# PANXIONG-CN/TEC-MoLLM

Measured on AMD Instinct MI355X. Metric: train samples/sec, higher is better.
Workload: dtype f32; 1 GPU; BASELINE configs[1]: B=8/GPU, L_in=48, L_out=12, N=2911, F=10 (d_emb=12), 3 GPT-2 blocks, full fwd+bwd+AdamW, fp32, GATv2 per_timestep, dropout on (p=0.1); global_batch=8, parallelism=dp1, data_feed=fixed, launch=eager

## Files before the change

include/tecmollm.h:

```cpp
#ifndef TECMOLLM_H
#define TECMOLLM_H

#include <stdint.h>

#ifdef __cplusplus
extern "C" {
#endif

#define TECM_OK 0
#define TECM_E_ARG (-1)
#define TECM_E_ALIGN (-2)
#define TECM_E_LAUNCH (-3)
#define TECM_E_LDS (-4)

#define TECM_ABI_VERSION 18
int tecm_abi_version(void);
const char* tecm_last_error(void);

typedef struct TecmWin {
  int32_t enabled;
  int32_t N;
  int32_t Lin, Lout;
  int32_t stride_t;
  int32_t taps;
  int32_t Cw;
  int32_t pad;
} TecmWin;

typedef struct TecmDrop {
  float p;
  int32_t _pad;
  uint64_t seed;
  int64_t ld;
  const uint64_t* seed_dev;
} TecmDrop;

enum { TECM_A_MK = 0, TECM_A_KM = 1 };
enum { TECM_B_NK = 0, TECM_B_KN = 1 };
enum { TECM_ACT_NONE = 0, TECM_ACT_GELU_ERF = 1, TECM_ACT_GELU_TANH = 2 };

#define TECM_IO_A_BF16 1
#define TECM_IO_B_BF16 2
#define TECM_IO_C_BF16 4
#define TECM_IO_PRE_BF16 8
typedef struct TecmGemm {
  int64_t M, N, K;
  const float* A; int64_t lda; int32_t a_layout; int32_t io_bf16; TecmWin a_win; TecmDrop a_drop;
  const float* B; int64_t ldb; int32_t b_layout; int32_t _p1; TecmWin b_win; TecmDrop b_drop;
  float* C; int64_t ldc; TecmWin c_win;
  float alpha; int32_t act;
  const float* bias;
  const float* rowbias; int64_t rb_ld; int32_t rb_div; int32_t rb_mod;
  float* preact; int64_t ldp;
  const float* dact_src; int64_t ldd;
  TecmDrop out_drop;
  const float* residual; int64_t ldr;
  int32_t accumulate;
  int32_t split_k;
  float* workspace;
} TecmGemm;
int tecm_gemm_f32(const TecmGemm* desc, void* stream);
int tecm_gemm_bf16(const TecmGemm* desc, void* stream);
int tecm_gemm_bf16x3(const TecmGemm* g, void* stream);
int tecm_gemm_bf16x6(const TecmGemm* g, void* stream);

int32_t tecm_gemm_tn_splits(int64_t M, int64_t N, int64_t K);
int tecm_p8_rows(int64_t M, int64_t N);

typedef struct TecmSpatial {
  int32_t B, L, N, Cin, Demb, H;
  int32_t graphs_with_edges;
  int32_t num_tiles, tile_nodes, win_max;
  const float* x;
  const float* tf; int64_t tf_sb, tf_sl, tf_sn, tf_sf;
  const float* node_tab; const float* tod_tab; const float* doy_tab; const float* year_tab;
  const float* season_tab;
  int32_t year_rows;
  int32_t tile_edges_max;
  const float* Wl; const float* bl; const float* Wr; const float* br;
  const float* att;
  const float* bias;
  const int32_t* rowptr;
  const int32_t* colidx;
  const int32_t* tile_lo; const int32_t* tile_hi;
  TecmDrop alpha_drop;
  float* out;
  int32_t* err_flag;
  int32_t flags;
  int32_t out_ld;
} TecmSpatial;
#define TECM_SPATIAL_EMBED_ONLY 1
#define TECM_SPATIAL_NO_RESIDUAL 2
#define TECM_BAD_TOD 1
#define TECM_BAD_DOY 2
#define TECM_BAD_YEAR 4
#define TECM_BAD_SEASON 8
int tecm_spatial_fwd(const TecmSpatial* d, void* stream);
int64_t tecm_spatial_fwd2_ws_floats(const TecmSpatial* d);
int tecm_spatial_fwd2(const TecmSpatial* d, float* ws, void* stream);

typedef struct TecmSpatialGrads {
  const float* dout;
  float* d_node_tab;
  float* d_tod_tab; float* d_doy_tab; float* d_year_tab; float* d_season_tab;
  float* partials; int64_t partial_ld;
  int32_t t_chunk; int32_t num_blocks;
  const int32_t* src_ptr; const int32_t* src_col; const int32_t* src_ptr_off;
} TecmSpatialGrads;
int tecm_spatial_bwd(const TecmSpatial* d, const TecmSpatialGrads* g, void* stream);
int tecm_spatial_bwd2_blocks(const TecmSpatial* d);
int tecm_spatial_bwd2(const TecmSpatial* d, const TecmSpatialGrads* g, float* ws, void* stream);
int tecm_spatial_bwd_blocks(const TecmSpatial* d);

#define TECM_GN_OUT_BF16 2
#define TECM_GN_DACT_BF16 4
#define TECM_GN_Y_BF16 1
#define TECM_GN_STATS_GIVEN 8
int tecm_gn_y16_supported(int32_t L, int32_t N, int32_t Cout);
int tecm_groupnorm_gelu_fwd(const void* y, const float* gamma, const float* beta, void* act,
                            float* stats, int32_t B, int32_t L, int32_t N, int32_t Cout, float eps,
                            int32_t io_bf16, int32_t act_stride, void* stream);
int tecm_groupnorm_gelu_bwd(const void* dact, int32_t dstride, const void* y, const float* gamma,
                            const float* beta, const float* stats, void* dy, float* dgb_partials,
                            int32_t* num_blocks, int32_t B, int32_t L, int32_t N, int32_t Cout,
                            int32_t io_bf16,
                            float* seq_sums ,
                            void* stream);

int tecm_layernorm_fwd(const float* x, int64_t ldx, const float* gamma, const float* beta, float* y,
                       int64_t ldy, void* y16, int64_t ldy16,
                       void* y16d ,
                       int64_t ldy16d, const TecmDrop* drop ,
                       int32_t y16d_seq_T, int32_t y16d_seq_N ,
                       float* stats , int64_t M, int32_t D, float eps, void* stream);
typedef struct TecmLnAdd {
  const void* dy2;
  int64_t ld;
  int32_t bf16, _pad;
  TecmDrop drop;
} TecmLnAdd;
typedef struct TecmLnDyMap {
  int32_t T, N;
  TecmDrop drop;
} TecmLnDyMap;
int tecm_layernorm_bwd(const float* dy, int64_t lddy, const float* x, int64_t ldx, const float* gamma,
                       const float* stats, const float* dres, float* dx, void* dx_masked, int32_t masked_bf16,
                       const TecmDrop* mask_drop, float* dgb_partials, int32_t* num_blocks, int64_t M, int32_t D,
                       const TecmLnAdd* add ,
                       int32_t dy_bf16 ,
                       const TecmLnDyMap* dymap , void* stream);

#define TECM_ATT_OUT_BF16 1
#define TECM_ATT_QKV_BF16 2
#define TECM_ATT_DCTX_BF16 4
int tecm_attention_fwd(const float* qkv, void* ctx, int32_t io_bf16, int32_t B, int32_t T, int32_t N, int32_t heads,
                       int32_t D, const TecmDrop* prob_drop, void* stream);
int tecm_attention_bwd(const float* qkv, const float* dctx, void* dqkv, int32_t io_bf16, int32_t B, int32_t T, int32_t N,
                       int32_t heads, int32_t D, const TecmDrop* prob_drop, void* stream);

int tecm_colsum(const float* in, int64_t ld, int64_t outer, int64_t inner, int32_t nseg, int32_t C,
                float* out, int64_t ldo, int32_t accumulate, float scale, const TecmDrop* in_drop,
                float* workspace , void* stream);
int tecm_colsum_twin(const float* in, int64_t ld, int64_t outer, int64_t inner, int32_t nseg, int32_t C,
                     float* out, int64_t ldo, int32_t accumulate, float scale, const TecmDrop* in_drop,
                     float* workspace, void* twin_bf16, int64_t ld_twin, void* stream);

int tecm_huber_fwd_bwd(const float* pred, const float* target, float* dpred, float* loss_out,
                       int64_t n, float delta, float grad_scale, float* workspace ,
                       void* stream);

int tecm_conv_weight_pack(const float* w, float* fwd_pack, float* bwd_pack, int32_t Cout, int32_t Cin,
                          int32_t k, void* stream);
int tecm_conv_weight_unpack(const float* dpack, float* dw, int32_t Cout, int32_t Cin, int32_t k,
                            void* stream);

typedef struct TecmConvDx {
  const void* dy;
  const void* wpack;
  float* dinp;
  int32_t B, Lc, N, Cout, ld_in, _pad;
} TecmConvDx;
int tecm_conv_dx_pack(const float* w3, const float* w5, const float* w7, void* wpack, int32_t Cout, int32_t Cin,
                      int32_t ld_in, void* stream);
int tecm_conv_dx_bf16(const TecmConvDx* p, void* stream);
typedef struct TecmConvFwd {
  const void* inp;
  const void* wpack;
  const float* bias;
  float* y;
  int32_t B, Lc, N, Cout, ld_in, y_bf16;
  float* stats;
  float eps;
  int32_t _pad;
} TecmConvFwd;
int tecm_conv_fwd_pack(const float* w3, const float* w5, const float* w7, void* wpack, int32_t Cout, int32_t Cin,
                       int32_t ld_in, void* stream);
int tecm_conv_fwd_bf16(const TecmConvFwd* p, void* stream);
int tecm_conv_fwd_pack_f32(const float* w3, const float* w5, const float* w7, float* wpack, int32_t Cout, int32_t Cin,
                           int32_t ld_in, void* stream);
int tecm_conv_fwd_f32(const TecmConvFwd* p, void* stream);
int tecm_conv_dx_pack_f32(const float* w3, const float* w5, const float* w7, float* wpack, int32_t Cout, int32_t Cin,
                          int32_t ld_in, void* stream);
int tecm_conv_dx_f32(const TecmConvDx* p, void* stream);
int tecm_conv_fwd_supported(int32_t Lc, int32_t Cout, int32_t ld_in, int32_t f32);
int tecm_conv_dx_supported(int32_t Lc, int32_t Cout, int32_t ld_in, int32_t f32);

typedef struct TecmConvDw {
  const void* inp;
  const void* dy;
  float* workspace;
  float* dw3;
  float* dw5;
  float* dw7;
  int32_t B, Lc, N, Cout, Cin, ld_in, num_blocks, _pad;
} TecmConvDw;
int tecm_huber_fwd_bwd_strided(const float* pred, const int64_t* pred_strides , const float* target,
                               const int64_t* target_strides , float* dpred, float* loss_out, int32_t B, int32_t H,
                               int32_t N, float delta, float grad_scale, float* workspace , void* stream);

int64_t tecm_conv_dw_workspace(int32_t Cout, int32_t ld_in, int32_t num_blocks);
int tecm_conv_dw_bf16(const TecmConvDw* p, void* stream);
int tecm_conv_dw_f32(const TecmConvDw* p, void* stream);

int tecm_cast_bf16(const float* src, int64_t ld_src, void* dst, int64_t ld_dst, int64_t rows, int32_t cols, void* stream);

int tecm_weight_bf16(const float* src, int64_t ld_src, void* same_bf16, int64_t ld_same, void* transposed_bf16, int64_t ld_tr,
                     int32_t rows, int32_t cols, void* stream);

int tecm_dropout_apply(const float* src, int64_t ld_src, void* dst, int64_t ld_dst, int32_t dst_bf16, void* dst2_bf16,
                       int64_t ld_dst2, int64_t rows, int32_t cols, const TecmDrop* drop, void* stream);

int tecm_transpose_scale(const float* src, int64_t lds, float* dst, int64_t ldd, int32_t rows,
                         int32_t cols, float scale, void* stream);

int tecm_lora_fold(const float* lora_B, int32_t n_out, int32_t r, float scale, void* w_kn, int64_t ld_kn, int32_t kn_bf16,
                   void* w_nk, int64_t ld_nk, int32_t nk_bf16, int32_t k_off, void* stream);

int tecm_pack_vectors(const float* const* srcs, const int32_t* lens, int32_t count, float* dst, void* stream);

#define TECM_NORM_BLOCKS 512
typedef struct {
  int64_t n;
  float* param; float* grad; float* exp_avg; float* exp_avg_sq;
  double* partials;
  float* total_norm_out;
  float lr, beta1, beta2, eps, weight_decay, max_norm, grad_scale;
  int32_t step;
  int32_t zero_grad;
  int32_t _pad;
} TecmAdamW;
int tecm_adamw_clip_step(const TecmAdamW* a, void* stream);
int tecm_checksum_tail(const float* param, int64_t n, float* tail, int32_t world, int32_t rank, double* ws, void* stream);
int tecm_checksum_verify(const float* tail, int32_t world, int32_t* err_word, int32_t bit, void* stream);
int tecm_seed_advance(uint64_t* word, uint64_t inc, void* stream);

#define TECM_METRIC_STATS 8
typedef struct {
  const float* pred; int64_t p_stride_s, p_stride_h, p_stride_i;
  const float* target; int64_t t_stride_s, t_stride_h, t_stride_i;
  int64_t S; int32_t H; int32_t _pad; int64_t I;
  double mean, scale;
  float clip_lo, clip_hi; int32_t clip;
  int32_t _pad2;
  double* stats;
} TecmMetrics;
int tecm_metrics_accumulate(const TecmMetrics* m, void* stream);

typedef struct {
  const float* X; const float* TF; const float* Y; const int64_t* starts;
  const int64_t* starts_host_check;
  int64_t T; int64_t row;
  int32_t N, L_in, L_out, F_t, B, _pad;
  float* x_out; float* tf_out; float* y_out;
} TecmWindowBatch;
int tecm_window_batch(const TecmWindowBatch* w, void* stream);

enum { TECM_BASELINE_MEAN = 0, TECM_BASELINE_LAST = 1, TECM_BASELINE_PERIODIC = 2 };
typedef struct {
  const float* X; const int64_t* starts;
  const int64_t* starts_host_check;
  int64_t T;
  int32_t N, C, channel, L_in, L_out, B, mode, period;
  float* out; int64_t o_stride_b, o_stride_h, o_stride_n;
} TecmWindowBaseline;
int tecm_window_baseline(const TecmWindowBaseline* w, void* stream);

typedef struct {
  const float* x; int64_t stride_t, stride_n;
  const int32_t* slot;
  int64_t T; int32_t N, n_slots;
  double* means; double* counts;
} TecmSlotMean;
int tecm_slot_mean(const TecmSlotMean* m, void* stream);

#ifdef __cplusplus
}
#endif
#endif
```

tec-mollm_amd/csrc/common.h:

```cpp
#pragma once
#include <hip/hip_runtime.h>
#include <stdint.h>
#include <stdio.h>
#include <stdarg.h>
#include <math.h>

#include "../../include/tecmollm.h"

#define TECM_WAVE 64

void tecm_set_error(const char* fmt, ...);

#define TECM_REQUIRE(cond, code, ...)            \
  do {                                           \
    if (!(cond)) {                               \
      tecm_set_error(__VA_ARGS__);               \
      return (code);                             \
    }                                            \
  } while (0)

#define TECM_CHECK_LAUNCH(name)                                                     \
  do {                                                                              \
    hipError_t e_ = hipGetLastError();                                              \
    if (e_ != hipSuccess) {                                                         \
      tecm_set_error("%s: launch failed: %s", (name), hipGetErrorString(e_));       \
      return TECM_E_LAUNCH;                                                         \
    }                                                                               \
  } while (0)

static inline bool tecm_aligned(const void* p, size_t a) { return (reinterpret_cast<uintptr_t>(p) % a) == 0; }

__host__ __device__ __forceinline__ uint32_t tecm_hash24(uint64_t seed, uint64_t idx) {
  uint32_t x = (uint32_t)idx + ((uint32_t)(idx >> 32) & 0xffffffu) * 0x9E3779u;
  x += (uint32_t)seed + (uint32_t)(seed >> 32) * 0x9E3779B1u;
  x ^= x >> 16;
  x *= 0x7feb352du;
  x ^= x >> 15;
  x *= 0x846ca68bu;
  x ^= x >> 16;
  return x >> 8;
}
__device__ __forceinline__ uint64_t tecm_seed_now(uint64_t seed, const uint64_t* seed_dev) {
  return seed_dev ? seed + *seed_dev : seed;
}
__host__ __device__ __forceinline__ uint32_t tecm_drop_thresh(float p) { return (uint32_t)(p * 16777216.0f); }
__device__ __forceinline__ float tecm_drop_mult(uint64_t seed, uint64_t idx, uint32_t thresh, float inv_keep) {
  return tecm_hash24(seed, idx) >= thresh ? inv_keep : 0.0f;
}

typedef __bf16 tecm_bf16x4 __attribute__((ext_vector_type(4)));
__device__ __forceinline__ void tecm_store_bf16x4(void* dst, float a, float b, float c, float d) {
  tecm_bf16x4 v;
  v[0] = (__bf16)a; v[1] = (__bf16)b; v[2] = (__bf16)c; v[3] = (__bf16)d;
  *reinterpret_cast<tecm_bf16x4*>(dst) = v;
}

__device__ __forceinline__ float gelu_erf(float x) { return 0.5f * x * (1.0f + erff(x * 0.70710678118654752440f)); }
__device__ __forceinline__ float dgelu_erf(float x) {
  const float cdf = 0.5f * (1.0f + erff(x * 0.70710678118654752440f));
  const float pdf = 0.39894228040143267794f * expf(-0.5f * x * x);
  return cdf + x * pdf;
}
__device__ __forceinline__ void gelu_erf_parts(float x, float& cdf, float& e) {
  const float z = fabsf(x) * 0.70710678118654752440f;
  const float t = __builtin_amdgcn_rcpf(1.0f + 0.3275911f * z);
  e = __builtin_amdgcn_exp2f(-0.72134752044448170368f * x * x);
  const float poly =
      t * (0.254829592f + t * (-0.284496736f + t * (1.421413741f + t * (-1.453152027f + t * 1.061405429f))));
  cdf = 0.5f * (1.0f + copysignf(1.0f - poly * e, x));
}
__device__ __forceinline__ float gelu_erf_fast(float x) {
  float cdf, e;
  gelu_erf_parts(x, cdf, e);
  return x * cdf;
}
__device__ __forceinline__ float dgelu_erf_fast(float x) {
  float cdf, e;
  gelu_erf_parts(x, cdf, e);
  return cdf + x * 0.39894228040143267794f * e;
}
__device__ __forceinline__ float fast_tanh(float u) {
  const float e = __builtin_amdgcn_exp2f(2.88539008177792681472f * u);
  return 1.0f - 2.0f * __builtin_amdgcn_rcpf(1.0f + e);
}
__device__ __forceinline__ void gelu_tanh_parts(float x, float x2, float& s, float& r) {
  float a = x * fmaf(x2, 0.10294324f, 2.3022082f);
  a = fminf(a, 100.0f);
  const float E = __builtin_amdgcn_exp2f(a);
  r = __builtin_amdgcn_rcpf(1.0f + E);
  s = E * r;
}
__device__ __forceinline__ float gelu_tanh(float x) {
  float s, r;
  gelu_tanh_parts(x, x * x, s, r);
  return x * s;
}
__device__ __forceinline__ float dgelu_tanh(float x) {
  const float x2 = x * x;
  float s, r;
  gelu_tanh_parts(x, x2, s, r);
  const float du2 = fmaf(x2, 0.21406445f, 1.5957691f);
  return fmaf(x * du2 * r, s, s);
}
__device__ __forceinline__ float apply_act(int act, float v) {
  return act == TECM_ACT_GELU_ERF ? gelu_erf(v) : (act == TECM_ACT_GELU_TANH ? gelu_tanh(v) : v);
}
__device__ __forceinline__ float apply_dact(int act, float v) {
  return act == TECM_ACT_GELU_ERF ? dgelu_erf(v) : (act == TECM_ACT_GELU_TANH ? dgelu_tanh(v) : 1.0f);
}

__device__ __forceinline__ float wave_sum(float v) {
#pragma unroll
  for (int o = 32; o > 0; o >>= 1) v += __shfl_xor(v, o, 64);
  return v;
}
__device__ __forceinline__ float wave_max(float v) {
#pragma unroll
  for (int o = 32; o > 0; o >>= 1) v = fmaxf(v, __shfl_xor(v, o, 64));
  return v;
}
__device__ __forceinline__ float group16_sum(float v) {
#pragma unroll
  for (int o = 8; o > 0; o >>= 1) v += __shfl_xor(v, o, 64);
  return v;
}

#define TECM_ROW_INVALID INT32_MIN
struct RowRef {
  int64_t srow;
  int32_t t0;
};

__device__ __forceinline__ RowRef make_rowref(const TecmWin& w, bool win, int64_t m, int64_t rows) {
  RowRef r;
  if (m >= rows) {
    r.srow = 0;
    r.t0 = TECM_ROW_INVALID;
    return r;
  }
  if (!win) {
    r.srow = m;
    r.t0 = 0;
    return r;
  }
  const int64_t q = m / w.N;
  const int32_t n = (int32_t)(m - q * w.N);
  const int64_t bq = q / w.Lout;
  const int32_t t_out = (int32_t)(q - bq * w.Lout);
  r.t0 = t_out * w.stride_t - w.pad;
  r.srow = (bq * w.Lin + r.t0) * (int64_t)w.N + n;
  return r;
}
```

tec-mollm_amd/csrc/gemm.hip:

```cpp
#include "gemm_bf16_impl.h"
int tecm_gemm_x3_dispatch(const TecmGemm& g, int products, hipStream_t st);

namespace {

template <int U>
__global__ __launch_bounds__(256) void splitk_reduce_kernel(const TecmGemm g, int splits) {
  __shared__ float red[4][64];
  const int64_t total = g.M * g.N;
  const int lane = threadIdx.x & 63, wave = threadIdx.x >> 6;
  const tecm_gemm::DropCtx odc = tecm_gemm::make_drop(g.out_drop);
  for (int64_t i0 = (int64_t)blockIdx.x * 64; i0 < total; i0 += (int64_t)gridDim.x * 64) {
    const int64_t i = i0 + lane;
    float v16[U];
#pragma unroll
    for (int u = 0; u < U; ++u) v16[u] = 0.f;
    if (i < total) {
      for (int s = wave; s < splits; s += 4 * U) {
#pragma unroll
        for (int u = 0; u < U; ++u) {
          const int sl = s + 4 * u;
          const float v = g.workspace[(int64_t)(sl < splits ? sl : splits - 1) * total + i];
          v16[u] += sl < splits ? v : 0.f;
        }
      }
    }
#pragma unroll
    for (int u = U / 2; u > 0; u >>= 1)
#pragma unroll
      for (int v = 0; v < u; ++v) v16[v] += v16[v + u];
    red[wave][lane] = v16[0];
    __syncthreads();
    if (wave == 0 && i < total) {
      const float v = (red[0][lane] + red[1][lane]) + (red[2][lane] + red[3][lane]);
      const int64_t m = i / g.N;
      tecm_gemm::epilogue_store(g, odc, m, (int32_t)(i - m * g.N), v);
    }
    __syncthreads();
  }
}

__global__ __launch_bounds__(256) void erf_post_kernel(float* __restrict__ C, int64_t ldc, const float* __restrict__ src,
                                                       int64_t lds, int64_t M, int32_t N, tecm_gemm::DropCtx odc) {
  const int64_t total = M * N;
  odc.seed = tecm_seed_now(odc.seed, odc.sdev);
  for (int64_t i = (int64_t)blockIdx.x * blockDim.x + threadIdx.x; i < total; i += (int64_t)gridDim.x * blockDim.x) {
    const int64_t m = i / N;
    const int32_t n = (int32_t)(i - m * N);
    float v = C[m * ldc + n];
    v = src ? v * dgelu_erf(src[m * lds + n]) : gelu_erf(v);
    if (odc.thresh) v *= tecm_drop_mult(odc.seed, (uint64_t)(m * odc.ld + n), odc.thresh, odc.inv);
    C[m * ldc + n] = v;
  }
}

int pick_vec(const float* p, int64_t ld, const TecmWin& w, bool inner_is_k, int64_t K) {
  int v = 4;
  while (v > 1) {
    bool ok = tecm_aligned(p, 4 * v) && (ld % v == 0);
    if (w.enabled) ok = ok && (w.Cw % v == 0);
    if (inner_is_k) ok = ok && (K % v == 0);
    if (ok) break;
    v >>= 1;
  }
  return v;
}

bool win_ok(const TecmWin& w) {
  return !w.enabled || (w.N > 0 && w.Lin > 0 && w.Lout > 0 && w.stride_t > 0 && w.taps > 0 && w.Cw > 0 && w.pad >= 0);
}

}

enum { MODE_F32 = 0, MODE_BF16 = 1, MODE_X3 = 2, MODE_X6 = 3 };
static int gemm_entry(const TecmGemm* d, void* stream, int mode);

extern "C" int tecm_gemm_f32(const TecmGemm* d, void* stream) { return gemm_entry(d, stream, MODE_F32); }

extern "C" int tecm_gemm_bf16(const TecmGemm* d, void* stream) { return gemm_entry(d, stream, MODE_BF16); }

extern "C" int tecm_gemm_bf16x3(const TecmGemm* d, void* stream) { return gemm_entry(d, stream, MODE_X3); }
extern "C" int tecm_gemm_bf16x6(const TecmGemm* d, void* stream) { return gemm_entry(d, stream, MODE_X6); }

static int gemm_entry(const TecmGemm* d, void* stream, int mode) {
  const bool bf16 = mode == MODE_BF16;
  TECM_REQUIRE(d != nullptr, TECM_E_ARG, "tecm_gemm_f32: null descriptor");
  const TecmGemm& g = *d;
  TECM_REQUIRE(g.M > 0 && g.N > 0 && g.K > 0, TECM_E_ARG, "tecm_gemm_f32: M,N,K must be positive (%lld,%lld,%lld)",
               (long long)g.M, (long long)g.N, (long long)g.K);
  TECM_REQUIRE(g.M < (1ll << 31) && g.K < (1ll << 30) && g.N < (1ll << 30), TECM_E_ARG,
               "tecm_gemm_f32: M/N/K too large for 32-bit row arithmetic");
  TECM_REQUIRE(g.A && g.B && g.C, TECM_E_ARG, "tecm_gemm_f32: null operand");
  TECM_REQUIRE(win_ok(g.a_win) && win_ok(g.b_win) && win_ok(g.c_win), TECM_E_ARG, "tecm_gemm_f32: bad window view");
  TECM_REQUIRE(!(g.a_win.enabled && g.a_layout != TECM_A_MK), TECM_E_ARG,
               "tecm_gemm_f32: a_win needs the MK layout (view rows are m)");
  TECM_REQUIRE(!(g.b_win.enabled && g.b_layout != TECM_B_KN), TECM_E_ARG,
               "tecm_gemm_f32: b_win needs the KN layout (view rows are the reduction index)");
  TECM_REQUIRE(!(g.a_win.enabled && (int64_t)g.a_win.taps * g.a_win.Cw != g.K), TECM_E_ARG,
               "tecm_gemm_f32: a_win taps*Cw != K");
  TECM_REQUIRE(!(g.b_win.enabled && (int64_t)g.b_win.taps * g.b_win.Cw != g.N), TECM_E_ARG,
               "tecm_gemm_f32: b_win taps*Cw != N");
  TECM_REQUIRE(!(g.c_win.enabled && (int64_t)g.c_win.taps * g.c_win.Cw != g.N), TECM_E_ARG,
               "tecm_gemm_f32: c_win taps*Cw != N");
  TECM_REQUIRE(!(g.rowbias && (g.rb_div <= 0 || g.rb_mod <= 0)), TECM_E_ARG, "tecm_gemm_f32: bad rowbias spec");
  TECM_REQUIRE(!(g.split_k > 1 && g.workspace == nullptr), TECM_E_ARG, "tecm_gemm_f32: split_k needs a workspace");
  TECM_REQUIRE(g.a_layout == TECM_A_MK || g.b_layout == TECM_B_KN, TECM_E_ARG,
               "tecm_gemm_f32: layout combination KM x NK is not built");
  hipStream_t st = (hipStream_t)stream;
  int avec = pick_vec(g.A, g.lda, g.a_win, g.a_layout == TECM_A_MK, g.K);
  int bvec = pick_vec(g.B, g.ldb, g.b_win, g.b_layout == TECM_B_NK, g.K);
  if (g.io_bf16 & TECM_IO_A_BF16) avec = 4;
  if (g.io_bf16 & TECM_IO_B_BF16) bvec = 4;
  const bool win = g.a_win.enabled || g.b_win.enabled;
  const bool drop = g.a_drop.p > 0.f || g.b_drop.p > 0.f;
  auto ok4 = [](const void* p, int64_t ld) { return p == nullptr || (tecm_aligned(p, 16) && ld % 4 == 0); };
  const bool c16 = (g.io_bf16 & TECM_IO_C_BF16) != 0;
  const bool p16 = (g.io_bf16 & TECM_IO_PRE_BF16) != 0;
  auto ok4h = [](const void* p, int64_t ld) { return p == nullptr || (tecm_aligned(p, 8) && ld % 4 == 0); };
  const bool vec4 = g.N % 4 == 0 && (c16 ? ok4h(g.C, g.ldc) : ok4(g.C, g.ldc)) && ok4(g.bias, 4) && ok4(g.rowbias, g.rb_ld) &&
                    (p16 ? ok4h(g.preact, g.ldp) && ok4h(g.dact_src, g.ldd) : ok4(g.preact, g.ldp) && ok4(g.dact_src, g.ldd)) &&
                    ok4(g.residual, g.ldr) &&
                    (!g.c_win.enabled || g.c_win.Cw % 4 == 0) &&
                    (g.split_k <= 1 || tecm_aligned(g.workspace, 16));
  if (c16) TECM_REQUIRE(vec4, TECM_E_ALIGN, "tecm_gemm_bf16: bf16 C needs 16-byte friendly epilogue operands");
  if (bf16)
    TECM_REQUIRE(avec == 4 && bvec == 4, TECM_E_ALIGN,
                 "tecm_gemm_bf16: operands must be 16-byte aligned with leading dims / K / Cw multiples of 4");
  if (mode == MODE_X3 || mode == MODE_X6) {
    TECM_REQUIRE(g.a_layout == TECM_A_MK && g.b_layout == TECM_B_NK && !win && !drop, TECM_E_ARG,
                 "tecm_gemm_bf16x3: serves the plain MK x NK contraction only (no operand windows / prologue dropout)");
    TECM_REQUIRE(avec == 4 && bvec == 4, TECM_E_ALIGN,
                 "tecm_gemm_bf16x3: operands must be 16-byte aligned with leading dims / K multiples of 4");
  }
  const int io = g.io_bf16 & (TECM_IO_A_BF16 | TECM_IO_B_BF16 | TECM_IO_C_BF16 | TECM_IO_PRE_BF16);
  TECM_REQUIRE(io == g.io_bf16, TECM_E_ARG, "tecm_gemm: unknown io_bf16 bits");
  if (io) {
    TECM_REQUIRE(bf16, TECM_E_ARG, "tecm_gemm: bf16 tensors in HBM are served by tecm_gemm_bf16 only");
    if (io & (TECM_IO_A_BF16 | TECM_IO_B_BF16))
      TECM_REQUIRE(!drop, TECM_E_ARG, "tecm_gemm_bf16: bf16 operands take no prologue dropout");
    if (io & TECM_IO_A_BF16) {
      TECM_REQUIRE(tecm_aligned(g.A, 16) && g.lda % 8 == 0, TECM_E_ALIGN, "tecm_gemm_bf16: bf16 A must be 16-byte friendly");
      TECM_REQUIRE((g.a_layout == TECM_A_MK ? g.K : g.M) % 8 == 0 && (!g.a_win.enabled || g.a_win.Cw % 8 == 0), TECM_E_ARG,
                   "tecm_gemm_bf16: bf16 A needs its contiguous extent (K for MK, M for KM) and a_win.Cw to be multiples of 8");
    }
    if (io & TECM_IO_B_BF16) {
      TECM_REQUIRE(tecm_aligned(g.B, 16) && g.ldb % 8 == 0, TECM_E_ALIGN, "tecm_gemm_bf16: bf16 B must be 16-byte friendly");
      TECM_REQUIRE((g.b_layout == TECM_B_NK ? g.K : g.N) % 8 == 0 && (!g.b_win.enabled || g.b_win.Cw % 8 == 0), TECM_E_ARG,
                   "tecm_gemm_bf16: bf16 B needs its contiguous extent (K for NK, N for KN) and b_win.Cw to be multiples of 8");
    }
    if (io & TECM_IO_PRE_BF16)
      TECM_REQUIRE(vec4 && (g.preact || g.dact_src) && g.split_k <= 1 && g.act != TECM_ACT_GELU_ERF && !g.c_win.enabled &&
                       !g.rowbias,
                   TECM_E_ARG, "tecm_gemm_bf16: a bf16 preact / dact_src needs the 16-byte friendly plain tanh-GELU epilogue");
    if (io & TECM_IO_C_BF16)
      TECM_REQUIRE(vec4 && !g.residual && !g.accumulate && !g.c_win.enabled && g.split_k <= 1 &&
                       g.act != TECM_ACT_GELU_ERF,
                   TECM_E_ARG, "tecm_gemm_bf16: bf16 C needs a 16-byte friendly plain epilogue");
  }
  TecmGemm gk = g;
  gk.io_bf16 = io | (vec4 ? TECM_P0_VEC4 : 0);
  const bool erf = g.act == TECM_ACT_GELU_ERF;
  if (erf) {
    TECM_REQUIRE(!g.residual && !g.accumulate && !g.c_win.enabled, TECM_E_ARG,
                 "tecm_gemm_f32: GELU_ERF cannot be combined with residual / accumulate / c_win");
    gk.act = TECM_ACT_NONE;
    gk.dact_src = nullptr;
    gk.out_drop.p = 0.f;
  }
  int splits;
  if (mode == MODE_X3 || mode == MODE_X6) {
    splits = tecm_gemm_x3_dispatch(gk, mode == MODE_X6 ? 6 : 3, st);
  } else if (bf16) {
    if (g.a_layout == TECM_A_MK && g.b_layout == TECM_B_NK)
      splits = tecm_gemm16_dispatch_mk_nk(gk, win, drop, st);
    else if (g.a_layout == TECM_A_MK)
      splits = tecm_gemm16_dispatch_mk_kn(gk, win, drop, st);
    else
      splits = tecm_gemm16_dispatch_km_kn(gk, win, drop, st);
  } else if (g.a_layout == TECM_A_MK && g.b_layout == TECM_B_NK)
    splits = tecm_gemm_dispatch_mk_nk(gk, avec, bvec, win, drop, st);
  else if (g.a_layout == TECM_A_MK)
    splits = tecm_gemm_dispatch_mk_kn(gk, avec, bvec, win, drop, st);
  else
    splits = tecm_gemm_dispatch_km_kn(gk, avec, bvec, win, drop, st);
  if (splits < 0) return splits;
  if (splits > 1) {
    const int64_t total = g.M * g.N;
    const int64_t want = (total + 63) / 64;
    const int blocks = (int)(want < 4096 ? want : 4096);
    if (splits > 32)
      hipLaunchKernelGGL(splitk_reduce_kernel<16>, dim3(blocks), dim3(256), 0, st, gk, splits);
    else if (splits > 16)
      hipLaunchKernelGGL(splitk_reduce_kernel<8>, dim3(blocks), dim3(256), 0, st, gk, splits);
    else
      hipLaunchKernelGGL(splitk_reduce_kernel<4>, dim3(blocks), dim3(256), 0, st, gk, splits);
    TECM_CHECK_LAUNCH("tecm_gemm_f32/splitk_reduce");
  }
  if (erf) {
    const int64_t want = (g.M * g.N + 255) / 256;
    hipLaunchKernelGGL(erf_post_kernel, dim3((unsigned)(want < 4096 ? want : 4096)), dim3(256), 0, st, g.C, g.ldc,
                       g.dact_src, g.ldd, g.M, (int32_t)g.N, tecm_gemm::make_drop_host(g.out_drop));
    TECM_CHECK_LAUNCH("tecm_gemm_f32/erf_post");
  }
  return TECM_OK;
}
```

tec-mollm_amd/csrc/gemm_impl.h:

```cpp
#pragma once
#include "common.h"
#ifndef TECM_BIG_THREADS
#define TECM_BIG_THREADS 512
#endif
#include <utility>
#ifndef TECM_ABLATE
#define TECM_ABLATE 0
#endif
#ifndef TECM_STAGE_Q
#define TECM_STAGE_Q 0
#endif

typedef float f32x16 __attribute__((ext_vector_type(16)));
typedef float f32x4 __attribute__((ext_vector_type(4)));

#define TECM_P0_VEC4 0x100

namespace tecm_gemm {

template <class F, int... Is>
__device__ __forceinline__ void static_for_impl(F&& f, std::integer_sequence<int, Is...>) {
  (f(std::integral_constant<int, Is>{}), ...);
}
template <int N, class F>
__device__ __forceinline__ void static_for(F&& f) {
  static_for_impl(f, std::make_integer_sequence<int, N>{});
}

constexpr int BM = 128;
constexpr int BK = 32;
constexpr int LDK = BK + 4;
constexpr int NTHREADS_MAX = 512;
__host__ __device__ constexpr int threads_for(int bn) { return bn >= 128 ? TECM_BIG_THREADS : 256; }

struct DropCtx {
  uint64_t seed;
  int64_t ld;
  uint32_t thresh;
  float inv;
  const uint64_t* sdev;
};
inline DropCtx make_drop_host(const TecmDrop& d) {
  DropCtx c;
  c.seed = d.seed;
  c.sdev = d.seed_dev;
  c.ld = d.ld;
  c.thresh = d.p > 0.f ? tecm_drop_thresh(d.p) : 0u;
  c.inv = d.p > 0.f ? 1.0f / (1.0f - d.p) : 1.0f;
  return c;
}
__device__ __forceinline__ DropCtx make_drop(const TecmDrop& d) {
  DropCtx c;
  c.seed = tecm_seed_now(d.seed, d.seed_dev);
  c.sdev = nullptr;
  c.ld = d.ld;
  c.thresh = d.p > 0.f ? tecm_drop_thresh(d.p) : 0u;
  c.inv = d.p > 0.f ? 1.0f / (1.0f - d.p) : 1.0f;
  return c;
}

template <int VEC>
__device__ __forceinline__ void gload(const float* __restrict__ p, const float* __restrict__ safe, bool ok,
                                      float (&out)[VEC]) {
  const float* q = ok ? p : safe;
  if constexpr (VEC == 4) {
    const float4 v = *reinterpret_cast<const float4*>(q);
    out[0] = v.x; out[1] = v.y; out[2] = v.z; out[3] = v.w;
  } else if constexpr (VEC == 2) {
    const float2 v = *reinterpret_cast<const float2*>(q);
    out[0] = v.x; out[1] = v.y;
  } else {
    out[0] = q[0];
  }
}

template <int VEC>
__device__ __forceinline__ void apply_drop(const DropCtx& dc, int64_t didx, float (&v)[VEC]) {
  if (dc.thresh) {
#pragma unroll
    for (int e = 0; e < VEC; ++e) v[e] *= tecm_drop_mult(dc.seed, (uint64_t)(didx + e), dc.thresh, dc.inv);
  }
}

template <int VEC>
__device__ __forceinline__ void lds_store(float* dst, const float (&v)[VEC]) {
  if constexpr (VEC == 4) {
    *reinterpret_cast<float4*>(dst) = make_float4(v[0], v[1], v[2], v[3]);
  } else if constexpr (VEC == 2) {
    *reinterpret_cast<float2*>(dst) = make_float2(v[0], v[1]);
  } else {
    dst[0] = v[0];
  }
}

struct WinRow {
  int64_t srow;
  int32_t t0;
};
__device__ __forceinline__ WinRow win_row(const TecmWin& w, int64_t m, int64_t rows) {
  WinRow r;
  if (m >= rows) {
    r.srow = 0;
    r.t0 = TECM_ROW_INVALID;
    return r;
  }
  const uint32_t mm = (uint32_t)m;
  const uint32_t q = mm / (uint32_t)w.N;
  const int32_t n = (int32_t)(mm - q * (uint32_t)w.N);
  const uint32_t bq = q / (uint32_t)w.Lout;
  const int32_t t_out = (int32_t)(q - bq * (uint32_t)w.Lout);
  r.t0 = t_out * w.stride_t - w.pad;
  r.srow = ((int64_t)bq * w.Lin + r.t0) * (int64_t)w.N + n;
  return r;
}

template <bool ROWK, int ROWS, int VEC, bool WIN, bool DROP, int NTHREADS>
struct Stager {
  static constexpr int R = ROWK ? BK : ROWS;
  static constexpr int CI = ROWK ? ROWS : BK;
  static constexpr int LD = ROWK ? ROWS + 4 : LDK;
  static constexpr int VPR = CI / VEC;
  static constexpr int NV = (R * VPR) / NTHREADS;
  static constexpr int RSTEP = NTHREADS / VPR;
  static_assert((R * VPR) % NTHREADS == 0 && NTHREADS % VPR == 0, "tile/thread mapping");

  struct Tile {
    float regs[NV][VEC];
    uint32_t okbits = 0;
    int64_t dsave[DROP ? NV : 1];
  };
  const float* ptr[NV];
  uint32_t rowok;
  bool inner_ok;
  int64_t didx[DROP ? NV : 1];
  WinRow wr[(WIN && !ROWK) ? NV : 1];
  int32_t rn[(WIN && ROWK) ? NV : 1], rt[(WIN && ROWK) ? NV : 1], rb[(WIN && ROWK) ? NV : 1];
  int32_t tap, c;
  int32_t kk;

  __device__ __forceinline__ void init(const float* __restrict__ P, const TecmWin& w, int64_t ld, int64_t row0,
                                       int64_t rows_total, int32_t kbeg, int64_t fixed0, int64_t fixed_lim,
                                       const DropCtx& dc) {
    const int cv = (threadIdx.x % VPR) * VEC;
    const int r0 = threadIdx.x / VPR;
    rowok = 0;
    inner_ok = true;
    tap = 0;
    c = 0;
    kk = kbeg + cv;
    const bool wen = WIN && w.enabled;
    if (!wen) {
      if constexpr (!ROWK) {
#pragma unroll
        for (int i = 0; i < NV; ++i) {
          int64_t row = row0 + r0 + i * RSTEP;
          if (row < rows_total) rowok |= 1u << i;
          else row = rows_total - 1;
          ptr[i] = P + row * ld + kbeg + cv;
          if constexpr (DROP) didx[i] = row * dc.ld + kbeg + cv;
        }
      } else {
        inner_ok = (fixed0 + cv) < fixed_lim;
        const int64_t inner = inner_ok ? fixed0 + cv : 0;
#pragma unroll
        for (int i = 0; i < NV; ++i) {
          const int64_t row = (int64_t)kbeg + r0 + i * RSTEP;
          ptr[i] = P + row * ld + inner;
          if constexpr (DROP) didx[i] = row * dc.ld + inner;
        }
      }
    } else if constexpr (WIN) {
      if constexpr (!ROWK) {
#pragma unroll
        for (int i = 0; i < NV; ++i) wr[i] = win_row(w, row0 + r0 + i * RSTEP, rows_total);
        tap = kk / w.Cw;
        c = kk - tap * w.Cw;
      } else {
        const int32_t inner = (int32_t)(fixed0 + cv);
        inner_ok = inner < fixed_lim;
        tap = inner / w.Cw;
        c = inner - tap * w.Cw;
#pragma unroll
        for (int i = 0; i < NV; ++i) {
          const uint32_t row = (uint32_t)(kbeg + r0 + i * RSTEP);
          const uint32_t q = row / (uint32_t)w.N;
          rn[i] = (int32_t)(row - q * (uint32_t)w.N);
          rb[i] = (int32_t)(q / (uint32_t)w.Lout);
          rt[i] = (int32_t)(q - (uint32_t)rb[i] * (uint32_t)w.Lout);
        }
      }
    }
  }

  __device__ __forceinline__ void load(Tile& tl, const float* __restrict__ P, const TecmWin& w, int64_t ld, int32_t k0,
                                       int32_t klim, const DropCtx& dc) {
    load_part<0, NV>(tl, P, w, ld, k0, klim, dc);
  }
  template <int IB, int IE>
  __device__ __forceinline__ void load_part(Tile& tl, const float* __restrict__ P, const TecmWin& w, int64_t ld, int32_t k0,
                                            int32_t klim, const DropCtx& dc) {
    if constexpr (IB >= IE) return;
    const int r0 = threadIdx.x / VPR;
    const bool wen = WIN && w.enabled;
    constexpr bool LAST = IE == NV;
    if (!wen) {
      if constexpr (!ROWK) {
        const bool kok = kk < klim;
#pragma unroll
        for (int i = IB; i < IE; ++i) {
          const bool ok = kok && ((rowok >> i) & 1u);
          gload<VEC>(ptr[i], P, ok, tl.regs[i]);
          tl.okbits = (tl.okbits & ~(1u << i)) | ((ok ? 1u : 0u) << i);
          if constexpr (DROP) { tl.dsave[i] = didx[i]; didx[i] += BK; }
          ptr[i] += BK;
        }
        if constexpr (LAST) kk += BK;
      } else {
#pragma unroll
        for (int i = IB; i < IE; ++i) {
          const bool ok = inner_ok && (k0 + r0 + i * RSTEP) < klim;
          gload<VEC>(ptr[i], P, ok, tl.regs[i]);
          tl.okbits = (tl.okbits & ~(1u << i)) | ((ok ? 1u : 0u) << i);
          if constexpr (DROP) { tl.dsave[i] = didx[i]; didx[i] += (int64_t)BK * dc.ld; }
          ptr[i] += (int64_t)BK * ld;
        }
      }
    } else if constexpr (WIN) {
      if constexpr (!ROWK) {
        const bool kok = kk < klim;
        const int64_t tapoff = (int64_t)tap * w.N;
#pragma unroll
        for (int i = IB; i < IE; ++i) {
          const int32_t t_in = wr[i].t0 + tap;
          const bool ok = kok && t_in >= 0 && t_in < w.Lin;
          const int64_t row = wr[i].srow + tapoff;
          gload<VEC>(P + row * ld + c, P, ok, tl.regs[i]);
          tl.okbits = (tl.okbits & ~(1u << i)) | ((ok ? 1u : 0u) << i);
          if constexpr (DROP) tl.dsave[i] = row * dc.ld + c;
        }
        if constexpr (LAST) {
          kk += BK;
          c += BK;
          while (c >= w.Cw) { c -= w.Cw; ++tap; }
        }
      } else {
#pragma unroll
        for (int i = IB; i < IE; ++i) {
          const int32_t t_in = rt[i] * w.stride_t - w.pad + tap;
          const bool ok = inner_ok && (k0 + r0 + i * RSTEP) < klim && t_in >= 0 && t_in < w.Lin;
          const int64_t row = ((int64_t)rb[i] * w.Lin + t_in) * (int64_t)w.N + rn[i];
          gload<VEC>(P + row * ld + c, P, ok, tl.regs[i]);
          tl.okbits = (tl.okbits & ~(1u << i)) | ((ok ? 1u : 0u) << i);
          if constexpr (DROP) tl.dsave[i] = row * dc.ld + c;
          rn[i] += BK;
          while (rn[i] >= w.N) {
            rn[i] -= w.N;
            if (++rt[i] >= w.Lout) { rt[i] = 0; ++rb[i]; }
          }
        }
      }
    }
  }

  __device__ __forceinline__ void load_steady(Tile& tl, int64_t ld, const DropCtx& dc) {
    tl.okbits = ~0u;
#pragma unroll
    for (int i = 0; i < NV; ++i) {
      gload<VEC>(ptr[i], ptr[i], true, tl.regs[i]);
      if constexpr (!ROWK) {
        if constexpr (DROP) { tl.dsave[i] = didx[i]; didx[i] += BK; }
        ptr[i] += BK;
      } else {
        if constexpr (DROP) { tl.dsave[i] = didx[i]; didx[i] += (int64_t)BK * dc.ld; }
        ptr[i] += (int64_t)BK * ld;
      }
    }
    if constexpr (!ROWK) kk += BK;
  }
  __device__ __forceinline__ void store_steady(const Tile& tl, float* lds, const DropCtx& dc) {
    const int cv = (threadIdx.x % VPR) * VEC;
    const int r0 = threadIdx.x / VPR;
#pragma unroll
    for (int i = 0; i < NV; ++i) {
      if constexpr (DROP) {
        float v[VEC];
#pragma unroll
        for (int e = 0; e < VEC; ++e) v[e] = tl.regs[i][e];
        apply_drop<VEC>(dc, tl.dsave[i], v);
        lds_store<VEC>(lds + (r0 + i * RSTEP) * LD + cv, v);
      } else {
        lds_store<VEC>(lds + (r0 + i * RSTEP) * LD + cv, tl.regs[i]);
      }
    }
  }

  __device__ __forceinline__ void store(const Tile& tl, float* lds, const DropCtx& dc) { store_part<0, NV>(tl, lds, dc); }
  template <int IB, int IE>
  __device__ __forceinline__ void store_part(const Tile& tl, float* lds, const DropCtx& dc) {
    if constexpr (IB >= IE) return;
    const int cv = (threadIdx.x % VPR) * VEC;
    const int r0 = threadIdx.x / VPR;
#pragma unroll
    for (int i = IB; i < IE; ++i) {
      float v[VEC];
      const bool ok = (tl.okbits >> i) & 1u;
#pragma unroll
      for (int e = 0; e < VEC; ++e) v[e] = ok ? tl.regs[i][e] : 0.f;
      if constexpr (DROP) apply_drop<VEC>(dc, tl.dsave[i], v);
      lds_store<VEC>(lds + (r0 + i * RSTEP) * LD + cv, v);
    }
  }
};

struct EpiRow {
  int64_t m;
  int64_t crow;
  int64_t drow;
  int32_t t0;
  const float* rb;
};
struct EpiCol {
  int32_t n;
  int32_t tap, c;
  float bias;
  bool ok;
};

__device__ __forceinline__ EpiRow epi_row(const TecmGemm& g, const DropCtx& odc, int64_t m) {
  EpiRow r;
  r.m = m;
  r.t0 = 0;
  if (g.c_win.enabled) {
    const WinRow w = win_row(g.c_win, m, g.M);
    r.crow = w.srow;
    r.t0 = w.t0;
    r.drow = 0;
  } else {
    r.crow = m * g.ldc;
    r.drow = m * odc.ld;
  }
  r.rb = g.rowbias ? g.rowbias + (int64_t)(((uint32_t)m / (uint32_t)g.rb_div) % (uint32_t)g.rb_mod) * g.rb_ld
                   : nullptr;
  return r;
}
__device__ __forceinline__ EpiCol epi_col(const TecmGemm& g, int64_t n) {
  EpiCol c;
  c.n = (int32_t)n;
  c.ok = n < g.N;
  c.bias = (g.bias && c.ok) ? g.bias[n] : 0.f;
  c.tap = 0;
  c.c = 0;
  if (g.c_win.enabled) {
    c.tap = c.n / g.c_win.Cw;
    c.c = c.n - c.tap * g.c_win.Cw;
  }
  return c;
}
__device__ __forceinline__ void epi_elem(const TecmGemm& g, const DropCtx& odc, const EpiRow& r, const EpiCol& c,
                                         float v) {
  const int32_t n = c.n;
  v = v * g.alpha + c.bias;
  if (r.rb) v += r.rb[n];
  if (g.preact) g.preact[r.m * g.ldp + n] = v;
  if (g.dact_src)
    v *= dgelu_tanh(g.dact_src[r.m * g.ldd + n]);
  else if (g.act)
    v = gelu_tanh(v);
  int64_t off, didx;
  if (g.c_win.enabled) {
    const int32_t t_in = r.t0 + c.tap;
    if (t_in < 0 || t_in >= g.c_win.Lin) return;
    const int64_t row = r.crow + (int64_t)c.tap * g.c_win.N;
    off = row * g.ldc + c.c;
    didx = row * odc.ld + c.c;
  } else {
    off = r.crow + n;
    didx = r.drow + n;
  }
  if (odc.thresh) v *= tecm_drop_mult(odc.seed, (uint64_t)didx, odc.thresh, odc.inv);
  if (g.residual) v += g.residual[r.m * g.ldr + n];
  if (g.accumulate) v += g.C[off];
  g.C[off] = v;
}
__device__ __forceinline__ void epilogue_store(const TecmGemm& g, const DropCtx& odc, int64_t m, int32_t n, float v) {
  const EpiRow r = epi_row(g, odc, m);
  const EpiCol c = epi_col(g, n);
  epi_elem(g, odc, r, c, v);
}

__device__ __forceinline__ void epi_vec4(const TecmGemm& g, const DropCtx& odc, const EpiRow& r, const EpiCol& c,
                                         const float4& bias4, float4 v) {
  const int32_t n = c.n;
  float o[4] = {v.x * g.alpha + bias4.x, v.y * g.alpha + bias4.y, v.z * g.alpha + bias4.z, v.w * g.alpha + bias4.w};
  if (r.rb) {
    const float4 t = *reinterpret_cast<const float4*>(r.rb + n);
    o[0] += t.x; o[1] += t.y; o[2] += t.z; o[3] += t.w;
  }
  const bool p16 = (g.io_bf16 & TECM_IO_PRE_BF16) != 0;
  if (g.preact) {
    if (p16) {
      tecm_bf16x4 h;
      h[0] = (__bf16)o[0]; h[1] = (__bf16)o[1]; h[2] = (__bf16)o[2]; h[3] = (__bf16)o[3];
      *reinterpret_cast<tecm_bf16x4*>(reinterpret_cast<__bf16*>(g.preact) + r.m * g.ldp + n) = h;
      o[0] = (float)h[0]; o[1] = (float)h[1]; o[2] = (float)h[2]; o[3] = (float)h[3];
    } else {
      *reinterpret_cast<float4*>(g.preact + r.m * g.ldp + n) = make_float4(o[0], o[1], o[2], o[3]);
    }
  }
  if (g.dact_src) {
    float4 t;
    if (p16) {
      const tecm_bf16x4 h = *reinterpret_cast<const tecm_bf16x4*>(reinterpret_cast<const __bf16*>(g.dact_src) + r.m * g.ldd + n);
      t = make_float4((float)h[0], (float)h[1], (float)h[2], (float)h[3]);
    } else {
      t = *reinterpret_cast<const float4*>(g.dact_src + r.m * g.ldd + n);
    }
    o[0] *= dgelu_tanh(t.x); o[1] *= dgelu_tanh(t.y);
    o[2] *= dgelu_tanh(t.z); o[3] *= dgelu_tanh(t.w);
  } else if (g.act) {
#pragma unroll
    for (int e = 0; e < 4; ++e) o[e] = gelu_tanh(o[e]);
  }
  int64_t off, didx;
  if (g.c_win.enabled) {
    const int32_t t_in = r.t0 + c.tap;
    if (t_in < 0 || t_in >= g.c_win.Lin) return;
    const int64_t row = r.crow + (int64_t)c.tap * g.c_win.N;
    off = row * g.ldc + c.c;
    didx = row * odc.ld + c.c;
  } else {
    off = r.crow + n;
    didx = r.drow + n;
  }
  if (odc.thresh) {
#pragma unroll
    for (int e = 0; e < 4; ++e) o[e] *= tecm_drop_mult(odc.seed, (uint64_t)(didx + e), odc.thresh, odc.inv);
  }
  if (g.residual) {
    const float4 t = *reinterpret_cast<const float4*>(g.residual + r.m * g.ldr + n);
    o[0] += t.x; o[1] += t.y; o[2] += t.z; o[3] += t.w;
  }
  if (g.accumulate) {
    const float4 t = *reinterpret_cast<const float4*>(g.C + off);
    o[0] += t.x; o[1] += t.y; o[2] += t.z; o[3] += t.w;
  }
  if (g.io_bf16 & TECM_IO_C_BF16) {
    typedef __bf16 bf16x4_t __attribute__((ext_vector_type(4)));
    bf16x4_t h;
    h[0] = (__bf16)o[0]; h[1] = (__bf16)o[1]; h[2] = (__bf16)o[2]; h[3] = (__bf16)o[3];
    *reinterpret_cast<bf16x4_t*>(reinterpret_cast<__bf16*>(g.C) + off) = h;
    return;
  }
  *reinterpret_cast<float4*>(g.C + off) = make_float4(o[0], o[1], o[2], o[3]);
}

#ifndef TECM_EPI_STAMP
#define TECM_EPI_STAMP(i) do { } while (0)
#endif
template <int NIT, int RPI, int MODE>
__device__ __forceinline__ void epi_fast_load(const TecmGemm& g, int lrow, int64_t mrow0, const EpiCol& ecol,
                                              float4 (&in)[NIT]) {
  const int32_t ncol = ecol.ok ? ecol.n : 0;
  if constexpr (MODE == 5) {
#pragma unroll
    for (int it = 0; it < NIT; ++it) {
      int64_t m = mrow0 + it * RPI + lrow;
      m = m < g.M ? m : g.M - 1;
      const uint32_t rr = ((uint32_t)m / (uint32_t)g.rb_div) % (uint32_t)g.rb_mod;
      in[it] = *reinterpret_cast<const float4*>(g.rowbias + (int64_t)rr * g.rb_ld + ncol);
    }
  }
  if constexpr (MODE >= 1 && MODE <= 3) {
    const float* src = MODE == 1 ? g.residual : (MODE == 2 ? g.dact_src : g.C);
    const int64_t ld = MODE == 1 ? g.ldr : (MODE == 2 ? g.ldd : g.ldc);
    const int32_t mb = (int32_t)mrow0 + lrow;
    const int64_t off0 = (int64_t)mb * ld + ncol, step = (int64_t)RPI * ld, off_last = (g.M - 1) * ld + ncol;
    if (MODE == 2 && (g.io_bf16 & TECM_IO_PRE_BF16)) {
#pragma unroll
      for (int it = 0; it < NIT; ++it) {
        const int64_t off = mb + it * RPI < (int32_t)g.M ? off0 + it * step : off_last;
        const float2 raw = *reinterpret_cast<const float2*>(reinterpret_cast<const __bf16*>(src) + off);
        in[it].x = raw.x;
        in[it].y = raw.y;
      }
      return;
    }
#pragma unroll
    for (int it = 0; it < NIT; ++it) {
      const int64_t off = mb + it * RPI < (int32_t)g.M ? off0 + it * step : off_last;
      in[it] = *reinterpret_cast<const float4*>(src + off);
    }
  }
}
enum { EPI_F_PRE = 1, EPI_F_P16 = 2, EPI_F_ACT = 4, EPI_F_DROP = 8, EPI_F_C16 = 16 };
template <int FEAT, int BIT>
__device__ __forceinline__ bool epi_feat(bool dynamic) {
  if constexpr (FEAT < 0) return dynamic;
  else return (FEAT & BIT) != 0;
}
template <int NIT, int RPI, int STG_LD, int MODE, bool NT, int FEAT = -1>
__device__ __forceinline__ void epi_fast_rows(const TecmGemm& g, const DropCtx& odc, const float* stg, int lrow, int lcol,
                                              int64_t mrow0, const EpiCol& ecol, const float4& bias4,
                                              const float4 (&in)[NIT]) {
  const int32_t n = ecol.n;
  const bool c16 = epi_feat<FEAT, EPI_F_C16>((g.io_bf16 & TECM_IO_C_BF16) != 0);
  const bool p16 = epi_feat<FEAT, EPI_F_P16>((g.io_bf16 & TECM_IO_PRE_BF16) != 0);
  const bool has_pre = epi_feat<FEAT, EPI_F_PRE>(g.preact != nullptr);
  const bool has_act = epi_feat<FEAT, EPI_F_ACT>(g.act != 0);
  const bool has_drop = epi_feat<FEAT, EPI_F_DROP>(odc.thresh != 0);
  constexpr int GRP = NIT < 4 ? NIT : 4;
  static_assert(NIT % GRP == 0, "row groups are read from the staging rows in whole batches");
  const int32_t mb = (int32_t)mrow0 + lrow;
  const int64_t offC0 = (int64_t)mb * g.ldc + n, stepC = (int64_t)RPI * g.ldc;
  const int64_t offP0 = (int64_t)mb * g.ldp + n, stepP = (int64_t)RPI * g.ldp;
  const int64_t idxD0 = (int64_t)mb * odc.ld + n, stepD = (int64_t)RPI * odc.ld;
  float4 vv[GRP];
#pragma unroll
  for (int it = 0; it < NIT; ++it) {
    if (it % GRP == 0) {
#pragma unroll
      for (int j = 0; j < GRP; ++j)
        vv[j] = *reinterpret_cast<const float4*>(&stg[((it + j) * RPI + lrow) * STG_LD + lcol]);
    }
    const int64_t m = mb + it * RPI;
    const float4 v = vv[it % GRP];
    const bool row_ok = mb + it * RPI < (int32_t)g.M && ecol.ok;
    if constexpr (MODE == 4) {
      if (row_ok) *reinterpret_cast<float4*>(g.workspace + ((int64_t)blockIdx.z * g.M + m) * g.N + n) = v;
      continue;
    }
    float o[4] = {v.x * g.alpha + bias4.x, v.y * g.alpha + bias4.y, v.z * g.alpha + bias4.z, v.w * g.alpha + bias4.w};
    if constexpr (MODE == 5) {
      o[0] += in[it].x; o[1] += in[it].y; o[2] += in[it].z; o[3] += in[it].w;
    }
    if (has_pre && p16) {
      tecm_bf16x4 hv;
      hv[0] = (__bf16)o[0]; hv[1] = (__bf16)o[1]; hv[2] = (__bf16)o[2]; hv[3] = (__bf16)o[3];
      if (row_ok) {
        tecm_bf16x4* dst = reinterpret_cast<tecm_bf16x4*>(reinterpret_cast<__bf16*>(g.preact) + (offP0 + it * stepP));
        if constexpr (NT) __builtin_nontemporal_store(hv, dst);
        else *dst = hv;
      }
      o[0] = (float)hv[0]; o[1] = (float)hv[1]; o[2] = (float)hv[2]; o[3] = (float)hv[3];
    } else if (has_pre && row_ok) {
      if constexpr (NT) {
        f32x4 nv = {o[0], o[1], o[2], o[3]};
        __builtin_nontemporal_store(nv, reinterpret_cast<f32x4*>(g.preact + (offP0 + it * stepP)));
      } else {
        *reinterpret_cast<float4*>(g.preact + (offP0 + it * stepP)) = make_float4(o[0], o[1], o[2], o[3]);
      }
    }
    if constexpr (MODE == 2) {
      float t0 = in[it].x, t1 = in[it].y, t2 = in[it].z, t3 = in[it].w;
      if (p16) {
        const uint32_t lo = __builtin_bit_cast(uint32_t, in[it].x), hi = __builtin_bit_cast(uint32_t, in[it].y);
        t0 = __builtin_bit_cast(float, lo << 16); t1 = __builtin_bit_cast(float, lo & 0xffff0000u);
        t2 = __builtin_bit_cast(float, hi << 16); t3 = __builtin_bit_cast(float, hi & 0xffff0000u);
      }
      o[0] *= dgelu_tanh(t0); o[1] *= dgelu_tanh(t1);
      o[2] *= dgelu_tanh(t2); o[3] *= dgelu_tanh(t3);
    } else {
      if (has_act) {
#pragma unroll
        for (int e = 0; e < 4; ++e) o[e] = gelu_tanh(o[e]);
      }
    }
    int64_t off = offC0 + it * stepC, didx = idxD0 + it * stepD;
    bool st_ok = row_ok;
    if constexpr (MODE == 6) {
      const WinRow w = win_row(g.c_win, m < g.M ? m : g.M - 1, g.M);
      const int32_t t_in = w.t0 + ecol.tap;
      const int64_t row = w.srow + (int64_t)ecol.tap * g.c_win.N;
      st_ok = row_ok && t_in >= 0 && t_in < g.c_win.Lin;
      off = row * g.ldc + ecol.c;
      didx = row * odc.ld + ecol.c;
    }
    if (has_drop) {
#pragma unroll
      for (int e = 0; e < 4; ++e) o[e] *= tecm_drop_mult(odc.seed, (uint64_t)(didx + e), odc.thresh, odc.inv);
    }
    if constexpr (MODE == 1 || MODE == 3) {
      o[0] += in[it].x; o[1] += in[it].y; o[2] += in[it].z; o[3] += in[it].w;
    }
    if (st_ok) {
      if constexpr (NT) {
        if (c16) {
          tecm_bf16x4 hv;
          hv[0] = (__bf16)o[0]; hv[1] = (__bf16)o[1]; hv[2] = (__bf16)o[2]; hv[3] = (__bf16)o[3];
          __builtin_nontemporal_store(hv, reinterpret_cast<tecm_bf16x4*>(reinterpret_cast<__bf16*>(g.C) + off));
        } else {
          f32x4 nv = {o[0], o[1], o[2], o[3]};
          __builtin_nontemporal_store(nv, reinterpret_cast<f32x4*>(g.C + off));
        }
      } else {
        if (c16) tecm_store_bf16x4(reinterpret_cast<__bf16*>(g.C) + off, o[0], o[1], o[2], o[3]);
        else *reinterpret_cast<float4*>(g.C + off) = make_float4(o[0], o[1], o[2], o[3]);
      }
    }
#ifdef TECM_EPI_SLEEP
    __builtin_amdgcn_s_sleep(TECM_EPI_SLEEP);
#endif
  }
}
template <int SLABS, int NIT, int RPI, int STG_LD, int MODE, bool NT, int FEAT = -1, typename StageFn>
__device__ __forceinline__ void epi_fast_block(const TecmGemm& g, const DropCtx& odc, const float* stg, int lrow, int lcol,
                                               int64_t mrow0, const EpiCol& ecol, const float4& bias4, StageFn&& stage) {
  float4 in[2][NIT];
  epi_fast_load<NIT, RPI, MODE>(g, lrow, mrow0, ecol, in[0]);
  static_for<SLABS>([&](auto sc) {
    constexpr int sl = decltype(sc)::value;
    TECM_EPI_STAMP(3 * sl);
    stage(sc);
    TECM_EPI_STAMP(3 * sl + 1);
    if constexpr (sl + 1 < SLABS)
      epi_fast_load<NIT, RPI, MODE>(g, lrow, mrow0 + (int64_t)(sl + 1) * NIT * RPI, ecol, in[(sl + 1) & 1]);
    epi_fast_rows<NIT, RPI, STG_LD, MODE, NT, FEAT>(g, odc, stg, lrow, lcol, mrow0 + (int64_t)sl * NIT * RPI, ecol, bias4, in[sl & 1]);
    TECM_EPI_STAMP(3 * sl + 2);
  });
}
__device__ __forceinline__ int epi_fast_mode(const TecmGemm& g) {
  if (!(g.io_bf16 & TECM_P0_VEC4)) return -1;
  if (gridDim.z > 1) return 4;
  const int streams = (g.residual ? 1 : 0) + (g.dact_src ? 1 : 0) + (g.accumulate ? 1 : 0);
  if (g.c_win.enabled)
    return (streams == 0 && !g.rowbias && !g.preact && !(g.io_bf16 & (TECM_IO_C_BF16 | TECM_IO_PRE_BF16))) ? 6 : -1;
  if (g.rowbias) return streams == 0 ? 5 : -1;
  if (streams > 1) return -1;
  return g.residual ? 1 : (g.dact_src ? 2 : (g.accumulate ? 3 : 0));
}
template <int SLABS, int NIT, int RPI, int STG_LD, bool NT = false, bool SPECIAL = false, typename StageFn>
__device__ __forceinline__ void epi_fast_dispatch(int mode, const TecmGemm& g, const DropCtx& odc, const float* stg, int lrow,
                                                  int lcol, int64_t mrow0, const EpiCol& ecol, const float4& bias4,
                                                  StageFn&& stage) {
  if constexpr (SPECIAL) {
    const int feat = (g.preact ? EPI_F_PRE : 0) | ((g.io_bf16 & TECM_IO_PRE_BF16) ? EPI_F_P16 : 0) | (g.act ? EPI_F_ACT : 0) |
                     (odc.thresh ? EPI_F_DROP : 0) | ((g.io_bf16 & TECM_IO_C_BF16) ? EPI_F_C16 : 0);
    if (mode == 0 && feat == EPI_F_C16)
      return epi_fast_block<SLABS, NIT, RPI, STG_LD, 0, NT, EPI_F_C16>(g, odc, stg, lrow, lcol, mrow0, ecol, bias4, stage);
    if (mode == 0 && feat == (EPI_F_PRE | EPI_F_P16 | EPI_F_ACT | EPI_F_C16))
      return epi_fast_block<SLABS, NIT, RPI, STG_LD, 0, NT, EPI_F_PRE | EPI_F_P16 | EPI_F_ACT | EPI_F_C16>(g, odc, stg, lrow, lcol, mrow0,
                                                                                                    ecol, bias4, stage);
    if (mode == 1 && feat == EPI_F_DROP)
      return epi_fast_block<SLABS, NIT, RPI, STG_LD, 1, NT, EPI_F_DROP>(g, odc, stg, lrow, lcol, mrow0, ecol, bias4, stage);
    if (mode == 2 && (feat & ~EPI_F_ACT) == (EPI_F_P16 | EPI_F_C16))
      return epi_fast_block<SLABS, NIT, RPI, STG_LD, 2, NT, EPI_F_P16 | EPI_F_C16>(g, odc, stg, lrow, lcol, mrow0, ecol, bias4, stage);
  }
  if (mode == 0) epi_fast_block<SLABS, NIT, RPI, STG_LD, 0, NT>(g, odc, stg, lrow, lcol, mrow0, ecol, bias4, stage);
  else if (mode == 1) epi_fast_block<SLABS, NIT, RPI, STG_LD, 1, NT>(g, odc, stg, lrow, lcol, mrow0, ecol, bias4, stage);
  else if (mode == 2) epi_fast_block<SLABS, NIT, RPI, STG_LD, 2, NT>(g, odc, stg, lrow, lcol, mrow0, ecol, bias4, stage);
  else if (mode == 3) epi_fast_block<SLABS, NIT, RPI, STG_LD, 3, NT>(g, odc, stg, lrow, lcol, mrow0, ecol, bias4, stage);
  else if (mode == 5) epi_fast_block<SLABS, NIT, RPI, STG_LD, 5, NT>(g, odc, stg, lrow, lcol, mrow0, ecol, bias4, stage);
  else if (mode == 6) epi_fast_block<SLABS, NIT, RPI, STG_LD, 6, NT>(g, odc, stg, lrow, lcol, mrow0, ecol, bias4, stage);
  else epi_fast_block<SLABS, NIT, RPI, STG_LD, 4, NT>(g, odc, stg, lrow, lcol, mrow0, ecol, bias4, stage);
}

template <int MT, int NT, int WTM, int WTN, int STG_LD>
__device__ __forceinline__ void block_epilogue(const TecmGemm& g, f32x16 (&acc)[MT][NT], float* smem, int wave, int lane,
                                               int wm, int wn, int64_t m0, int64_t n0) {
  const int r = lane & 31, h = lane >> 5;
  const DropCtx odc = make_drop(g.out_drop);
  const bool split = gridDim.z > 1;
  float* stg = smem + wave * (WTM * STG_LD);
  auto stage_all = [&](auto) {
    static_for<MT>([&](auto ic) {
      constexpr int i = decltype(ic)::value;
      static_for<16>([&](auto ec) {
        constexpr int e = decltype(ec)::value;
        static_for<NT>([&](auto jc) {
          constexpr int jn = decltype(jc)::value;
          stg[(i * 32 + (e & 3) + 8 * (e >> 2) + 4 * h) * STG_LD + jn * 32 + r] = acc[i][jn][e];
        });
      });
    });
  };
  if (g.io_bf16 & TECM_P0_VEC4) {
    constexpr int LPR = WTN / 4;
    constexpr int RPI = 64 / LPR;
    const int lcol = (lane % LPR) * 4, lrow = lane / LPR;
    const EpiCol ecol = epi_col(g, n0 + wn * WTN + lcol);
    float4 bias4 = make_float4(0.f, 0.f, 0.f, 0.f);
    if (g.bias) bias4 = *reinterpret_cast<const float4*>(g.bias + (ecol.ok ? ecol.n : 0));
    const int fmode = epi_fast_mode(g);
    if (fmode >= 0) {
      epi_fast_dispatch<1, WTM / RPI, RPI, STG_LD>(fmode, g, odc, stg, lrow, lcol, m0 + wm * WTM, ecol, bias4, stage_all);
      return;
    }
    stage_all(0);
    __syncthreads();
#pragma unroll 1
    for (int it = 0; it < WTM / RPI; ++it) {
      const int rl = it * RPI + lrow;
      const int64_t m = m0 + wm * WTM + rl;
      if (m < g.M && ecol.ok) {
        const float4 v = *reinterpret_cast<const float4*>(&stg[rl * STG_LD + lcol]);
        if (split) {
          *reinterpret_cast<float4*>(g.workspace + ((int64_t)blockIdx.z * g.M + m) * g.N + ecol.n) = v;
        } else {
          const EpiRow er = epi_row(g, odc, m);
          epi_vec4(g, odc, er, ecol, bias4, v);
        }
      }
    }
  } else {
    stage_all(0);
    __syncthreads();
    constexpr int RPI = 64 / WTN;
    const int lcol = lane % WTN, lrow = lane / WTN;
    const EpiCol ecol = epi_col(g, n0 + wn * WTN + lcol);
#pragma unroll 1
    for (int it = 0; it < WTM / RPI; ++it) {
      const int rl = it * RPI + lrow;
      const int64_t m = m0 + wm * WTM + rl;
      if (m < g.M && ecol.ok) {
        const float v = stg[rl * STG_LD + lcol];
        if (split) {
          g.workspace[((int64_t)blockIdx.z * g.M + m) * g.N + ecol.n] = v;
        } else {
          const EpiRow er = epi_row(g, odc, m);
          epi_elem(g, odc, er, ecol, v);
        }
      }
    }
  }
}

template <int ALAY, int BLAY, int AVEC, int BVEC, int BN, bool WIN, bool DROP, int BMT = BM>
__global__ __launch_bounds__(threads_for(BN), (AVEC == 4 && BVEC == 4) ? (threads_for(BN) == 512 ? (BMT > 128 ? 2 : 4) : 2) : 1) void gemm_kernel(const TecmGemm g,
                                                                                           int tiles_m, int tiles_n,
                                                                                           int k_chunk) {
  constexpr int NTHREADS = threads_for(BN);
  constexpr int NWAVES = NTHREADS / 64;
  constexpr int WN = BN >= 128 ? (NWAVES == 8 ? (BMT > 128 ? 2 : 4) : 2) : (BN == 64 ? 2 : 1);
  constexpr int WM = NWAVES / WN;
  constexpr int WTM = BMT / WM;
  static_assert(WTM >= 32 && WTM % 32 == 0, "wave tile");
  constexpr int WTN = BN / WN;
  constexpr int MT = WTM / 32;
  constexpr int NT = WTN / 32;
  using AStager = Stager<ALAY == TECM_A_KM, BMT, AVEC, WIN, DROP, NTHREADS>;
  using BStager = Stager<BLAY == TECM_B_KN, BN, BVEC, WIN, DROP, NTHREADS>;
  constexpr int A_FLOATS = AStager::R * AStager::LD;
  constexpr int B_FLOATS = BStager::R * BStager::LD;
  constexpr int TILE_FLOATS = A_FLOATS + B_FLOATS;
  constexpr int STG_LD = WTN + 4;
  constexpr int STG_FLOATS = NWAVES * WTM * STG_LD;
  constexpr int SMEM_FLOATS = 2 * TILE_FLOATS > STG_FLOATS ? 2 * TILE_FLOATS : STG_FLOATS;
  __shared__ __attribute__((aligned(16))) float smem[SMEM_FLOATS];

  const int nwg = tiles_m * tiles_n;
  const int id = blockIdx.x;
  const int xcd = id & 7, local = id >> 3;
  const int q8 = nwg >> 3, r8 = nwg & 7;
  const int wg = (xcd < r8 ? xcd * (q8 + 1) : r8 * (q8 + 1) + (xcd - r8) * q8) + local;
  const int GROUP_M = g._p1 > 0 ? g._p1 : (tiles_n <= 8 ? 2 : 8);
  const int per_group = GROUP_M * tiles_n;
  const int group = wg / per_group;
  const int first_m = group * GROUP_M;
  const int gsz = min(tiles_m - first_m, GROUP_M);
  const int in_group = wg - group * per_group;
  const int tm = first_m + in_group % gsz, tn = in_group / gsz;
  const int64_t m0 = (int64_t)tm * BMT;
  const int64_t n0 = (int64_t)tn * BN;
  const int32_t kbeg = blockIdx.z * k_chunk;
  const int32_t kend = min((int32_t)g.K, kbeg + k_chunk);

  const int lane = threadIdx.x & 63, wave = threadIdx.x >> 6;
  const int wm = wave / WN, wn = wave % WN;
  const int r = lane & 31, h = lane >> 5;

  const DropCtx adc = make_drop(g.a_drop), bdc = make_drop(g.b_drop);

  AStager sa;
  BStager sb;
  typename AStager::Tile ta;
  typename BStager::Tile tb;
  sa.init(g.A, g.a_win, g.lda, m0, g.M, kbeg, m0, g.M, adc);
  sb.init(g.B, g.b_win, g.ldb, n0, g.N, kbeg, n0, g.N, bdc);

  f32x16 acc[MT][NT];
#pragma unroll
  for (int i = 0; i < MT; ++i)
#pragma unroll
    for (int j = 0; j < NT; ++j)
#pragma unroll
      for (int e = 0; e < 16; ++e) acc[i][j][e] = 0.f;

  auto read_frags = [&](const float* As, const float* Bs, auto qc, float (&af)[MT][4], float (&bf)[NT][4]) {
    constexpr int q = decltype(qc)::value;
#pragma unroll
    for (int i = 0; i < MT; ++i) {
      const int row = wm * WTM + i * 32 + r;
      if constexpr (ALAY == TECM_A_MK) {
        const float4 v = *reinterpret_cast<const float4*>(&As[row * LDK + 8 * q + 4 * h]);
        af[i][0] = v.x; af[i][1] = v.y; af[i][2] = v.z; af[i][3] = v.w;
      } else {
#pragma unroll
        for (int j = 0; j < 4; ++j) af[i][j] = As[(8 * q + 4 * h + j) * AStager::LD + row];
      }
    }
#pragma unroll
    for (int i = 0; i < NT; ++i) {
      const int col = wn * WTN + i * 32 + r;
      if constexpr (BLAY == TECM_B_NK) {
        const float4 v = *reinterpret_cast<const float4*>(&Bs[col * LDK + 8 * q + 4 * h]);
        bf[i][0] = v.x; bf[i][1] = v.y; bf[i][2] = v.z; bf[i][3] = v.w;
      } else {
#pragma unroll
        for (int j = 0; j < 4; ++j) bf[i][j] = Bs[(8 * q + 4 * h + j) * BStager::LD + col];
      }
    }
  };
  auto do_mfma = [&](const float (&af)[MT][4], const float (&bf)[NT][4]) {
#pragma unroll
    for (int j = 0; j < 4; ++j)
#pragma unroll
      for (int i = 0; i < MT; ++i)
#pragma unroll
        for (int jn = 0; jn < NT; ++jn)
          acc[i][jn] = __builtin_amdgcn_mfma_f32_32x32x2f32(af[i][j], bf[jn][j], acc[i][jn], 0, 0, 0);
  };

  {
    typename AStager::Tile ta0;
    typename BStager::Tile tb0;
    sa.load(ta0, g.A, g.a_win, g.lda, kbeg, kend, adc);
    sb.load(tb0, g.B, g.b_win, g.ldb, kbeg, kend, bdc);
    if (kbeg + BK < kend) {
      sa.load(ta, g.A, g.a_win, g.lda, kbeg + BK, kend, adc);
      sb.load(tb, g.B, g.b_win, g.ldb, kbeg + BK, kend, bdc);
    }
    sa.store(ta0, smem, adc);
    sb.store(tb0, smem + A_FLOATS, bdc);
  }
  __syncthreads();

  float fa[2][MT][4], fb[2][NT][4];
  constexpr int ANV = AStager::NV, BNV = BStager::NV;
  auto tile_body = [&](const float* Ac, const float* Bc, float* An, int32_t k0, auto fullc) {
    constexpr bool FULL = decltype(fullc)::value;
    read_frags(Ac, Bc, std::integral_constant<int, 0>{}, fa[0], fb[0]);
    static_for<4>([&](auto qc) {
      constexpr int q = decltype(qc)::value;
      if constexpr (q < 3 && !(TECM_ABLATE >= 2 && FULL)) read_frags(Ac, Bc, std::integral_constant<int, q + 1>{}, fa[(q + 1) & 1], fb[(q + 1) & 1]);
      do_mfma(fa[q & 1], fb[q & 1]);
      if constexpr (q == TECM_STAGE_Q && !((TECM_ABLATE == 1 || TECM_ABLATE == 2) && FULL)) {
        if (FULL || k0 + BK < kend) {
          if constexpr (TECM_ABLATE == 3 && FULL) {
#pragma unroll
            for (int i = 0; i < ANV; ++i) asm volatile("" ::"v"(ta.regs[i][0]), "v"(ta.regs[i][1]), "v"(ta.regs[i][2]), "v"(ta.regs[i][3]));
#pragma unroll
            for (int i = 0; i < BNV; ++i) asm volatile("" ::"v"(tb.regs[i][0]), "v"(tb.regs[i][1]), "v"(tb.regs[i][2]), "v"(tb.regs[i][3]));
          } else if constexpr (FULL && !WIN) {
            sa.store_steady(ta, An, adc);
            sb.store_steady(tb, An + A_FLOATS, bdc);
          } else {
            sa.store(ta, An, adc);
            sb.store(tb, An + A_FLOATS, bdc);
          }
        }
        if constexpr (FULL && !WIN && TECM_ABLATE != 4) {
          sa.load_steady(ta, g.lda, adc);
          sb.load_steady(tb, g.ldb, bdc);
        } else if ((FULL && TECM_ABLATE != 4) || (!FULL && k0 + 2 * BK < kend)) {
          sa.load(ta, g.A, g.a_win, g.lda, k0 + 2 * BK, kend, adc);
          sb.load(tb, g.B, g.b_win, g.ldb, k0 + 2 * BK, kend, bdc);
        }
      }
      if constexpr (FULL && !WIN && !DROP && AVEC == 4 && BVEC == 4) {
        constexpr int NMFMA = MT * NT * 4;
        constexpr int NREAD = MT * (ALAY == TECM_A_MK ? 1 : 4) + NT * (BLAY == TECM_B_NK ? 1 : 4);
        constexpr int HALF = NMFMA / 2;
        constexpr int SPS = (ANV + BNV + HALF - 1) / HALF;
#pragma unroll
        for (int m = 0; m < NMFMA; ++m) {
          __builtin_amdgcn_sched_group_barrier(0x008, 1, 0);
          if constexpr (q < 3) {
            if (m < NREAD) __builtin_amdgcn_sched_group_barrier(0x100, 1, 0);
          }
          if constexpr (q == TECM_STAGE_Q) {
            if (m < HALF) __builtin_amdgcn_sched_group_barrier(0x200, SPS, 0);
            else __builtin_amdgcn_sched_group_barrier(0x020, SPS, 0);
          }
        }
      }
    });
  };

  int cur = 0;
  int32_t k0 = kbeg;
  for (; k0 + 3 * BK <= kend; k0 += BK) {
    tile_body(smem + cur * TILE_FLOATS, smem + cur * TILE_FLOATS + A_FLOATS, smem + (cur ^ 1) * TILE_FLOATS, k0,
              std::true_type{});
    __syncthreads();
    cur ^= 1;
  }
  for (; k0 < kend; k0 += BK) {
    tile_body(smem + cur * TILE_FLOATS, smem + cur * TILE_FLOATS + A_FLOATS, smem + (cur ^ 1) * TILE_FLOATS, k0,
              std::false_type{});
    __syncthreads();
    cur ^= 1;
  }

#ifdef TECM_ABLATE_NOEPI
  float keep = 0.f;
#pragma unroll
  for (int i = 0; i < MT; ++i)
#pragma unroll
    for (int j = 0; j < NT; ++j)
#pragma unroll
      for (int e = 0; e < 16; ++e) keep += acc[i][j][e];
  if (keep == 12345.678f) g.C[0] = keep;
#else
  block_epilogue<MT, NT, WTM, WTN, STG_LD>(g, acc, smem, wave, lane, wm, wn, m0, n0);
#endif
}

template <int ALAY, int BLAY, int AVEC, int BVEC, int BN, bool WIN, bool DROP, int BMT = BM>
int launch(const TecmGemm& g, hipStream_t st) {
  const int tiles_m = (int)((g.M + BMT - 1) / BMT);
  const int tiles_n = (int)((g.N + BN - 1) / BN);
  int splits = g.split_k > 1 ? g.split_k : 1;
  int k_chunk = (int)(((g.K + splits - 1) / splits + BK - 1) / BK) * BK;
  splits = (int)((g.K + k_chunk - 1) / k_chunk);
  dim3 grid((unsigned)(tiles_m * tiles_n), 1, (unsigned)splits);
  hipLaunchKernelGGL((gemm_kernel<ALAY, BLAY, AVEC, BVEC, BN, WIN, DROP, BMT>), grid, dim3(threads_for(BN)), 0, st, g, tiles_m,
                     tiles_n, k_chunk);
  TECM_CHECK_LAUNCH("tecm_gemm_f32");
  return splits;
}

template <int ALAY, int BLAY, int BN>
int dispatch(const TecmGemm& g, int avec, int bvec, bool win, bool drop, hipStream_t st) {
  if (avec == 4 && bvec == 4) {
    if (!win && !drop) return launch<ALAY, BLAY, 4, 4, BN, false, false>(g, st);
    if (win && !drop) return launch<ALAY, BLAY, 4, 4, BN, true, false>(g, st);
    if (!win && drop) return launch<ALAY, BLAY, 4, 4, BN, false, true>(g, st);
    return launch<ALAY, BLAY, 4, 4, BN, true, true>(g, st);
  }
  if constexpr (ALAY == TECM_A_MK) {
    if (avec >= 2) return launch<ALAY, BLAY, 2, 1, BN, true, true>(g, st);
  } else {
    if (avec == 4 && bvec >= 2) return launch<ALAY, BLAY, 4, 2, BN, true, true>(g, st);
  }
  return launch<ALAY, BLAY, 1, 1, BN, true, true>(g, st);
}

template <int ALAY, int BLAY, int BN>
int dispatch_m64(const TecmGemm& g, bool win, bool drop, hipStream_t st) {
  if (!win && !drop) return launch<ALAY, BLAY, 4, 4, BN, false, false, 64>(g, st);
  if (win && !drop) return launch<ALAY, BLAY, 4, 4, BN, true, false, 64>(g, st);
  if (!win && drop) return launch<ALAY, BLAY, 4, 4, BN, false, true, 64>(g, st);
  return launch<ALAY, BLAY, 4, 4, BN, true, true, 64>(g, st);
}

}

int tecm_gemm_dispatch_mk_nk(const TecmGemm& g, int avec, int bvec, bool win, bool drop, hipStream_t st);
int tecm_gemm_dispatch_mk_kn(const TecmGemm& g, int avec, int bvec, bool win, bool drop, hipStream_t st);
int tecm_gemm_dispatch_km_kn(const TecmGemm& g, int avec, int bvec, bool win, bool drop, hipStream_t st);
```

tec-mollm_amd/tecmollm/functions.py:

```python
from __future__ import annotations

import os
from dataclasses import dataclass
import weakref
from typing import List, Optional

import torch

from . import devcheck, ops
from ._lib import TecmSpatial, TecmSpatialGrads, check, lib, stream_ptr
from .graph import GraphMeta
from .ops import (A_KM, A_MK, ACT_GELU_ERF, ACT_GELU_TANH, B_KN, B_NK, colsum, drop, gemm, pick_split_k, win)

PRE16 = os.environ.get("TECM_PRE16", "1")[:1] != "0"
GRAD16 = os.environ.get("TECM_GRAD16", "1")[:1] != "0"
QKV16 = os.environ.get("TECM_QKV16", "1")[:1] != "0"

import ctypes as C

CP = 24
C_FEAT = 22
LORA_R = 32
LORA_SCALE = 2.0
GPT_HEADS = 12

SITE_GAT, SITE_EMBD, SITE_POST, SITE_HEAD = 0, 1, 100, 101


def site_lora(i):
    return 10 + 4 * i


def site_attn(i):
    return 11 + 4 * i


def site_res1(i):
    return 12 + 4 * i


def site_res2(i):
    return 13 + 4 * i


@dataclass
class DropPlan:
    training: bool
    p: float
    base_seed: int
    bf16: bool = False
    fuse_head: bool = False
    recompute: int = 0
    keep: bool = True

    def spec(self, site: int, ld: int):
        if not self.training or self.p <= 0.0:
            return None
        return drop(self.p, ops.splitmix64(self.base_seed * 1000003 + site), ld)


def _lib_error(msg: str):
    from ._lib import TecmError
    return TecmError(msg)


def _empty(*shape, like: torch.Tensor) -> torch.Tensor:
    return torch.empty(*shape, device=like.device, dtype=torch.float32)


class SpatialFn(torch.autograd.Function):

    @staticmethod
    def forward(ctx, x, tf, node_tab, tod_tab, doy_tab, year_tab, season_tab, Wl, bl, Wr, br, att, bias,
                meta: GraphMeta, heads: int, graphs_with_edges: int, plan: DropPlan):
        B, L, N, Cin = x.shape
        Demb = node_tab.shape[1]
        x = x.contiguous()
        out = _empty(B, L, N, CP, like=x)
        d = SpatialFn._desc(x, tf, node_tab, tod_tab, doy_tab, year_tab, season_tab, Wl, bl, Wr, br, att, bias, meta,
                            heads, graphs_with_edges, plan, B, L, N, Cin, Demb)
        d.out = out.data_ptr()
        errs = devcheck.error_word(x.device)
        errs.poll()
        nws = lib().tecm_spatial_fwd2_ws_floats(C.byref(d)) if os.environ.get("TECM_SPATIAL_V2", "1")[:1] != "0" else 0
        if nws > 0:
            ws = torch.empty(nws, device=x.device, dtype=torch.float32)
            check(lib().tecm_spatial_fwd2(C.byref(d), ws.data_ptr(), stream_ptr()), "tecm_spatial_fwd2")
        else:
            check(lib().tecm_spatial_fwd(C.byref(d), stream_ptr()), "tecm_spatial_fwd")
        errs.post()
        ctx.save_for_backward(x, tf, node_tab, tod_tab, doy_tab, year_tab, season_tab, Wl, bl, Wr, br, att, bias)
        ctx.meta, ctx.heads, ctx.R, ctx.plan = meta, heads, graphs_with_edges, plan
        return out

    @staticmethod
    def _desc(x, tf, node_tab, tod_tab, doy_tab, year_tab, season_tab, Wl, bl, Wr, br, att, bias, meta, heads, R,
              plan, B, L, N, Cin, Demb) -> TecmSpatial:
        d = TecmSpatial()
        d.B, d.L, d.N, d.Cin, d.Demb, d.H = B, L, N, Cin, Demb, heads
        d.graphs_with_edges = min(int(R), B * L)
        d.num_tiles, d.tile_nodes, d.win_max = meta.num_tiles, meta.tile_nodes, meta.win_max
        d.tile_edges_max = meta.tile_edges_max
        d.x = x.data_ptr()
        if tf is not None:
            d.tf = tf.data_ptr()
            d.tf_sb, d.tf_sl, d.tf_sn, d.tf_sf = tf.stride()
        for name, t in (("node_tab", node_tab), ("tod_tab", tod_tab), ("doy_tab", doy_tab), ("year_tab", year_tab),
                        ("season_tab", season_tab), ("Wl", Wl), ("bl", bl), ("Wr", Wr), ("br", br), ("att", att),
                        ("bias", bias)):
            if t is not None:
                setattr(d, name, t.data_ptr())
        d.year_rows = year_tab.shape[0] if year_tab is not None else 0
        d.rowptr, d.colidx = meta.rowptr.data_ptr(), meta.colidx.data_ptr()
        d.tile_lo, d.tile_hi = meta.tile_lo.data_ptr(), meta.tile_hi.data_ptr()
        sp = plan.spec(SITE_GAT, meta.max_deg + 1)
        if sp is not None:
            d.alpha_drop = sp
        d.err_flag = devcheck.error_word(x.device).ptr()
        d.flags, d.out_ld = 0, CP
        return d

    @staticmethod
    def backward(ctx, dout):
        (x, tf, node_tab, tod_tab, doy_tab, year_tab, season_tab, Wl, bl, Wr, br, att, bias) = ctx.saved_tensors
        meta = ctx.meta
        B, L, N, Cin = x.shape
        Demb = node_tab.shape[1]
        dout = dout.contiguous()
        d = SpatialFn._desc(x, tf, node_tab, tod_tab, doy_tab, year_tab, season_tab, Wl, bl, Wr, br, att, bias, meta,
                            ctx.heads, ctx.R, ctx.plan, B, L, N, Cin, Demb)
        v2 = os.environ.get("TECM_SPATIAL_V2", "1")[:1] != "0" and os.environ.get("TECM_SPATIAL_BWD2", "1")[:1] != "0"
        nb2 = lib().tecm_spatial_bwd2_blocks(C.byref(d)) if v2 else 0
        nblocks = nb2 if nb2 > 0 else lib().tecm_spatial_bwd_blocks(C.byref(d))
        if nblocks <= 0:
            check(nblocks, "tecm_spatial_bwd_blocks")
        Cc = C_FEAT
        pld = 2 * Cc * Cc + 4 * Cc
        partials = _empty(nblocks, pld, like=x)
        tabs = (node_tab, tod_tab, doy_tab, year_tab, season_tab)
        zbuf = torch.zeros(sum(t.numel() for t in tabs), device=x.device, dtype=torch.float32)
        offs = [0]
        for t in tabs:
            offs.append(offs[-1] + t.numel())
        d_node, d_tod, d_doy, d_year, d_season = (zbuf[a:b].view_as(t) for t, a, b in zip(tabs, offs[:-1], offs[1:]))
        g = TecmSpatialGrads()
        g.dout = dout.data_ptr()
        g.d_node_tab, g.d_tod_tab, g.d_doy_tab = d_node.data_ptr(), d_tod.data_ptr(), d_doy.data_ptr()
        g.d_year_tab, g.d_season_tab = d_year.data_ptr(), d_season.data_ptr()
        g.partials, g.partial_ld = partials.data_ptr(), pld
        g.t_chunk, g.num_blocks = 0, nblocks
        g.src_ptr, g.src_col = meta.src_ptr.data_ptr(), meta.src_col.data_ptr()
        g.src_ptr_off = meta.src_ptr_off.data_ptr()
        if nb2 > 0:
            ws = torch.empty(lib().tecm_spatial_fwd2_ws_floats(C.byref(d)), device=x.device, dtype=torch.float32)
            check(lib().tecm_spatial_bwd2(C.byref(d), C.byref(g), ws.data_ptr(), stream_ptr()), "tecm_spatial_bwd2")
        else:
            check(lib().tecm_spatial_bwd(C.byref(d), C.byref(g), stream_ptr()), "tecm_spatial_bwd")
        s = colsum(partials, pld, nblocks, 1, 1, pld)[0]
        o = 0
        dWl = s[o:o + Cc * Cc].view(Cc, Cc); o += Cc * Cc
        dbl = s[o:o + Cc]; o += Cc
        dWr = s[o:o + Cc * Cc].view(Cc, Cc); o += Cc * Cc
        dbr = s[o:o + Cc]; o += Cc
        datt = s[o:o + Cc].view_as(att)
        dbias = colsum(dout, CP, B * L * N, 1, 1, CP)[0, :Cc]
        return (None, None, d_node, d_tod, d_doy, d_year, d_season, dWl, dbl, dWr, dbr, datt, dbias,
                None, None, None, None)


class EmbedFn(torch.autograd.Function):

    @staticmethod
    def forward(ctx, x, tf, node_tab, tod_tab, doy_tab, year_tab, season_tab):
        B, L, N, Cin = x.shape
        Demb = node_tab.shape[1]
        x = x.contiguous()
        out = _empty(B, L, N, Cin + Demb, like=x)
        d = EmbedFn._desc(x, tf, node_tab, tod_tab, doy_tab, year_tab, season_tab, B, L, N, Cin, Demb)
        d.out = out.data_ptr()
        errs = devcheck.error_word(x.device)
        errs.poll()
        check(lib().tecm_spatial_fwd(C.byref(d), stream_ptr()), "tecm_spatial_fwd(embed only)")
        errs.post()
        ctx.save_for_backward(x, tf, node_tab, tod_tab, doy_tab, year_tab, season_tab)
        return out

    @staticmethod
    def _desc(x, tf, node_tab, tod_tab, doy_tab, year_tab, season_tab, B, L, N, Cin, Demb) -> TecmSpatial:
        d = TecmSpatial()
        d.B, d.L, d.N, d.Cin, d.Demb, d.H = B, L, N, Cin, Demb, 2
        d.graphs_with_edges, d.num_tiles, d.tile_nodes, d.win_max, d.tile_edges_max = 0, N, 1, 1, 0
        d.x = x.data_ptr()
        d.tf = tf.data_ptr()
        d.tf_sb, d.tf_sl, d.tf_sn, d.tf_sf = tf.stride()
        for name, t in (("node_tab", node_tab), ("tod_tab", tod_tab), ("doy_tab", doy_tab), ("year_tab", year_tab),
                        ("season_tab", season_tab)):
            setattr(d, name, t.data_ptr())
        for name in ("Wl", "bl", "Wr", "br", "att", "bias", "rowptr", "colidx", "tile_lo", "tile_hi"):
            setattr(d, name, node_tab.data_ptr())
        d.year_rows = year_tab.shape[0]
        d.err_flag = devcheck.error_word(x.device).ptr()
        d.flags, d.out_ld = 1, Cin + Demb
        return d

    @staticmethod
    def backward(ctx, dout):
        x, tf, node_tab, tod_tab, doy_tab, year_tab, season_tab = ctx.saved_tensors
        B, L, N, Cin = x.shape
        Demb = node_tab.shape[1]
        dout = dout.contiguous()
        d = EmbedFn._desc(x, tf, node_tab, tod_tab, doy_tab, year_tab, season_tab, B, L, N, Cin, Demb)
        grads = [torch.zeros_like(t) for t in (node_tab, tod_tab, doy_tab, year_tab, season_tab)]
        g = TecmSpatialGrads()
        g.dout = dout.data_ptr()
        g.d_node_tab, g.d_tod_tab, g.d_doy_tab, g.d_year_tab, g.d_season_tab = (t.data_ptr() for t in grads)
        check(lib().tecm_spatial_bwd(C.byref(d), C.byref(g), stream_ptr()), "tecm_spatial_bwd(embed only)")
        dx = dout[..., :Cin] if ctx.needs_input_grad[0] else None
        return (dx, None, *grads)


class GatFn(torch.autograd.Function):

    @staticmethod
    def forward(ctx, x, Wl, bl, Wr, br, att, bias, meta: GraphMeta, heads: int, graphs_with_edges: int, plan: DropPlan):
        G, N, Cc = x.shape
        x = x.contiguous()
        out = _empty(G, 1, N, CP, like=x)
        d = GatFn._desc(x, Wl, bl, Wr, br, att, bias, meta, heads, graphs_with_edges, plan)
        d.out = out.data_ptr()
        check(lib().tecm_spatial_fwd(C.byref(d), stream_ptr()), "tecm_spatial_fwd(GAT only)")
        ctx.save_for_backward(x, Wl, bl, Wr, br, att, bias)
        ctx.meta, ctx.heads, ctx.R, ctx.plan = meta, heads, graphs_with_edges, plan
        return out.view(G, N, CP)[..., :C_FEAT]

    @staticmethod
    def _desc(x, Wl, bl, Wr, br, att, bias, meta, heads, R, plan) -> TecmSpatial:
        G, N, Cc = x.shape
        d = SpatialFn._desc(x, None, None, None, None, None, None, Wl, bl, Wr, br, att, bias, meta, heads, R, plan,
                            G, 1, N, Cc, 0)
        d.flags = 2
        return d

    @staticmethod
    def backward(ctx, dout):
        x, Wl, bl, Wr, br, att, bias = ctx.saved_tensors
        G, N, Cc = x.shape
        if ctx.needs_input_grad[0]:
            raise _lib_error("SpatialEncoder.forward: the input needs no gradient in the MI355X path (x must not require grad)")
        dpad = torch.zeros(G, 1, N, CP, device=x.device, dtype=torch.float32)
        dpad[..., :Cc] = dout.reshape(G, 1, N, Cc)
        d = GatFn._desc(x, Wl, bl, Wr, br, att, bias, ctx.meta, ctx.heads, ctx.R, ctx.plan)
        nblocks = lib().tecm_spatial_bwd_blocks(C.byref(d))
        if nblocks <= 0:
            check(nblocks, "tecm_spatial_bwd_blocks")
        pld = 2 * Cc * Cc + 4 * Cc
        partials = _empty(nblocks, pld, like=x)
        g = TecmSpatialGrads()
        g.dout, g.partials, g.partial_ld, g.num_blocks = dpad.data_ptr(), partials.data_ptr(), pld, nblocks
        meta = ctx.meta
        g.src_ptr, g.src_col, g.src_ptr_off = meta.src_ptr.data_ptr(), meta.src_col.data_ptr(), meta.src_ptr_off.data_ptr()
        check(lib().tecm_spatial_bwd(C.byref(d), C.byref(g), stream_ptr()), "tecm_spatial_bwd(GAT only)")
        s = colsum(partials, pld, nblocks, 1, 1, pld)[0]
        o = 0
        dWl = s[o:o + Cc * Cc].view(Cc, Cc); o += Cc * Cc
        dbl = s[o:o + Cc]; o += Cc
        dWr = s[o:o + Cc * Cc].view(Cc, Cc); o += Cc * Cc
        dbr = s[o:o + Cc]; o += Cc
        datt = s[o:o + Cc].view_as(att)
        dbias = colsum(dpad, CP, G * N, 1, 1, CP)[0, :Cc]
        return (None, dWl, dbl, dWr, dbr, datt, dbias, None, None, None, None)


def conv_block_acts16(Lc: int, N: int, Cout: int) -> bool:
    return Cout >= 64 and ops.gn_reg_ok(Lc, N, Cout)


def conv_block_y16(Lc: int, N: int, Cout: int, ld_in: int) -> bool:
    CT = 3 * Cout
    return (conv_block_acts16(Lc, N, Cout) and ld_in % 8 == 0 and ops.conv_fwd_seq_ok(Lc, Cout, ld_in, f32=False)
            and ops.gn_y16_ok(Lc, N, Cout) and ops.uses_bf16(CT, Cout, Cout, CT, b_layout=B_KN))


def conv_storage_policy(N: int):
    def policy(L: int, Cout: int, Cin: int):
        ld_in = CP if Cin == C_FEAT else Cin
        return conv_block_acts16(L, N, Cout), conv_block_y16(L, N, Cout, ld_in)
    return policy


class ConvBlockFn(torch.autograd.Function):

    @staticmethod
    def forward(ctx, inp, inp16, cin: int, stride: int, need_dinp: bool, bf16: bool, recompute: bool,
                w3, b3, g3, be3, w5, b5, g5, be5, w7, b7, g7, be7, wf, bf):
        B, Lc, N, ld_in = inp.shape
        Cout = w3.shape[0]
        CT = 3 * Cout
        M = B * Lc * N
        ws = (w3, w5, w7)
        bs = (b3, b5, b7)
        r16 = int(bf16) == ops.PREC_BF16 and conv_block_acts16(Lc, N, Cout)
        adt = torch.bfloat16 if r16 else torch.float32
        side16 = r16
        packs = []
        seq_in = inp16 if (side16 and inp16 is not None) else (inp if int(bf16) == ops.PREC_FP32 else None)
        fwd_seq = seq_in is not None and ops.conv_fwd_seq_ok(Lc, Cout, ld_in, f32=seq_in.dtype == torch.float32)
        y16 = r16 and fwd_seq and seq_in.dtype == torch.bfloat16 and conv_block_y16(Lc, N, Cout, ld_in)
        y = torch.empty(B, Lc, N, CT, device=inp.device, dtype=torch.bfloat16 if y16 else torch.float32)
        bgb = ops.pack_vectors([b3, b5, b7, g3, g5, g7, be3, be5, be7])
        bias3, gamma, beta = bgb[:CT], bgb[CT:2 * CT], bgb[2 * CT:]
        stats = _empty(B * N, 3, 2, like=inp)
        st_given = y16 and ops.conv_fwd_stats_ok(Lc)
        if fwd_seq:
            ConvBlockFn._conv_seq(seq_in, (w3, w5, w7), bias3, y, stats if st_given else None, B, Lc, N, Cout, cin, ld_in)
        dx_gemm = need_dinp and not ConvBlockFn._dx_seq(bf16, r16, Lc, Cout, ld_in)
        fps = []
        a_in = inp16 if (inp16 is not None and side16 and ld_in % 8 == 0) else inp
        for j, (w, b) in enumerate(zip(ws, bs)):
            k = w.shape[2]
            if fwd_seq and not dx_gemm:
                packs.append(w.new_empty(0))
                continue
            wp = w if ld_in == cin else torch.nn.functional.pad(w, (0, 0, 0, ld_in - cin))
            fp, bp = ops.conv_weight_pack(wp.contiguous(), want_bwd=True)
            packs.append(bp)
            if fwd_seq:
                continue
            fps.append(fp)
            ConvBlockFn._conv_win(j, a_in, fp, b, y, M, B, Lc, N, Cout, ld_in, bf16)
        Lo = (Lc - 1) // stride + 1
        compact = stride > 1 and ops.gn_reg_ok(Lc, N, Cout) and int(bf16) in (ops.PREC_FP32, ops.PREC_BF16)
        La = Lo if compact else Lc
        act = torch.empty(B, La, N, CT, device=inp.device, dtype=adt)
        ConvBlockFn._norm(y, gamma, beta, act, stats, B, Lc, N, Cout, stride if compact else 1, st_given)
        out = _empty(B, Lo, N, Cout, like=inp)
        wf2 = wf.view(Cout, CT)
        out16 = None
        awin = None if compact else win(N, Lc, Lo, stride, 1, CT, 0)
        wfT16 = None
        if int(bf16) == ops.PREC_BF16 and compact and act.dtype == torch.bfloat16 and Cout % 8 == 0:
            wf2, wfT16 = ops.weight_bf16(wf2, same=True, transposed=True)
        ctx.wfT16 = wfT16
        if side16:
            out16 = torch.empty(B, Lo, N, Cout, device=inp.device, dtype=torch.bfloat16)
            gemm(B * Lo * N, Cout, CT, act, CT, wf2, CT, out16, Cout, a_win=awin, bias=bf, preact=(out, Cout), bf16=bf16)
            ctx.mark_non_differentiable(out16)
        else:
            gemm(B * Lo * N, Cout, CT, act, CT, wf2, CT, out, Cout, a_win=awin, bias=bf, bf16=bf16)
        ctx.recompute = bool(recompute)
        if recompute:
            ctx.save_for_backward(inp, gamma, beta, wf, *packs)
            ctx.rebuild = (seq_in if fwd_seq else None, a_in, fps, tuple(b.detach() for b in bs), bias3, y.dtype,
                           act.shape, adt, st_given)
            del y, act, stats
        else:
            ctx.save_for_backward(inp, y, act, stats, gamma, beta, wf, *packs)
        ctx.w357 = (w3.detach(), w5.detach(), w7.detach())
        ctx.inp16 = inp16 if (side16 and inp16 is not None and ld_in % 8 == 0) else None
        ctx.dims = (B, Lc, N, ld_in, cin, Cout, stride, Lo, need_dinp, bf16)
        ctx.compact = compact
        return out, out16

    @staticmethod
    def _conv_seq(seq_in, w357, bias3, y, stats, B, Lc, N, Cout, cin, ld_in):
        ops.conv_fwd(seq_in.detach(), w357[0].detach(), w357[1].detach(), w357[2].detach(), bias3, y, B, Lc, N, Cout, cin,
                     ld_in, stats=stats)

    @staticmethod
    def _conv_win(j, a_in, fp, b, y, M, B, Lc, N, Cout, ld_in, bf16):
        k = 3 + 2 * j
        gemm(M, Cout, k * ld_in, a_in, ld_in, fp, k * ld_in, y, 3 * Cout, c_off=j * Cout,
             a_win=win(N, Lc, Lc, 1, k, ld_in, (k - 1) // 2), bias=b, bf16=bf16)

    @staticmethod
    def _norm(y, gamma, beta, act, stats, B, Lc, N, Cout, act_stride, st_given):
        ops.groupnorm_gelu_fwd(y, gamma, beta, act, stats, B, Lc, N, Cout, act_stride=act_stride, stats_given=st_given)

    @staticmethod
    def _rebuild(ctx, gamma, beta):
        B, Lc, N, ld_in, cin, Cout, stride, Lo, need_dinp, bf16 = ctx.dims
        seq_in, a_in, fps, bs, bias3, ydt, ashape, adt, st_given = ctx.rebuild
        y = torch.empty(B, Lc, N, 3 * Cout, device=gamma.device, dtype=ydt)
        stats = _empty(B * N, 3, 2, like=gamma)
        if seq_in is not None:
            ConvBlockFn._conv_seq(seq_in, ctx.w357, bias3, y, stats if st_given else None, B, Lc, N, Cout, cin, ld_in)
        else:
            for j, (fp, b) in enumerate(zip(fps, bs)):
                ConvBlockFn._conv_win(j, a_in, fp, b, y, B * Lc * N, B, Lc, N, Cout, ld_in, bf16)
        act = torch.empty(ashape, device=gamma.device, dtype=adt)
        ConvBlockFn._norm(y, gamma, beta, act, stats, B, Lc, N, Cout, stride if ctx.compact else 1, st_given)
        return y, act, stats

    @staticmethod
    def _dx_seq(bf16, dy16: bool, Lc: int, Cout: int, ld_in: int) -> bool:
        return int(bf16) in (ops.PREC_FP32, ops.PREC_BF16) and (dy16 or int(bf16) == ops.PREC_FP32) \
            and ops.conv_dx_seq_ok(Lc, Cout, ld_in, f32=not dy16)

    @staticmethod
    def backward(ctx, dout, _dout16=None):
        if ctx.recompute:
            inp, gamma, beta, wf, bp3, bp5, bp7 = ctx.saved_tensors
            y, act, stats = ConvBlockFn._rebuild(ctx, gamma, beta)
        else:
            inp, y, act, stats, gamma, beta, wf, bp3, bp5, bp7 = ctx.saved_tensors
        B, Lc, N, ld_in, cin, Cout, stride, Lo, need_dinp, bf16 = ctx.dims
        CT = 3 * Cout
        M = B * Lc * N
        Mo = B * Lo * N
        dout = dout.contiguous()
        wf2 = wf.view(Cout, CT)
        if int(bf16) == ops.PREC_BF16 and act.dtype == torch.bfloat16 and ctx.compact and ops.tn_ok(Cout, CT, Mo) and Cout % 8 == 0:
            dout_g = torch.empty(Mo, Cout, device=dout.device, dtype=torch.bfloat16)
            dbf = colsum(dout, Cout, Mo, 1, 1, Cout, twin=dout_g)[0]
        else:
            dout_g = dout
            dbf = colsum(dout, Cout, Mo, 1, 1, Cout)[0]
        dwf = _empty(Cout, CT, like=inp)
        gemm(Cout, CT, Mo, dout_g, Cout, act, CT, dwf, CT, a_layout=A_KM, b_layout=B_KN,
             b_win=None if ctx.compact else win(N, Lc, Lo, stride, 1, CT, 0),
             split_k=pick_split_k(Cout, CT, Mo, prec=bf16), bf16=bf16)
        d16 = act.dtype == torch.bfloat16 and ops.uses_bf16(CT, Cout, Cout, CT, b_layout=B_KN)
        dact = torch.empty(B, Lo, N, CT, device=inp.device, dtype=torch.bfloat16 if d16 else torch.float32)
        if ctx.wfT16 is not None and dout_g.dtype == torch.bfloat16 and d16:
            gemm(Mo, CT, Cout, dout_g, Cout, ctx.wfT16, Cout, dact, CT, bf16=bf16)
        else:
            gemm(Mo, CT, Cout, dout_g, Cout, wf2, CT, dact, CT, b_layout=B_KN, bf16=bf16)
        dy = torch.empty(B, Lc, N, CT, device=inp.device, dtype=act.dtype)
        dgamma, dbeta, dbconv = ops.groupnorm_gelu_bwd(dact, stride, y, gamma, beta, stats, dy, B, Lc, N, Cout)
        dinp = _empty(B, Lc, N, ld_in, like=inp) if need_dinp else None
        dx_seq = need_dinp and ConvBlockFn._dx_seq(bf16, dy.dtype == torch.bfloat16, Lc, Cout, ld_in)
        if dx_seq:
            ops.conv_dx(dy, ctx.w357[0], ctx.w357[1], ctx.w357[2], dinp, B, Lc, N, Cout, cin, ld_in)
        grads = []
        dw_in = ctx.inp16 if dy.dtype == torch.bfloat16 else (inp if int(bf16) == ops.PREC_FP32 else None)
        dw_seq = dw_in is not None and ops.conv_dw_seq_ok(Lc, Cout, ld_in)
        dws = ops.conv_dw(dw_in, dy, B, Lc, N, Cout, cin, ld_in) if dw_seq else None
        for j, (k, bp) in enumerate(((3, bp3), (5, bp5), (7, bp7))):
            K = k * ld_in
            db = dbconv[j * Cout:(j + 1) * Cout]
            if dw_seq:
                if need_dinp and not dx_seq:
                    gemm(M, ld_in, k * Cout, dy, CT, bp, ld_in, dinp, ld_in, b_layout=B_KN, a_off=j * Cout,
                         a_win=win(N, Lc, Lc, 1, k, Cout, (k - 1) // 2), accumulate=(j > 0), bf16=bf16)
                grads += [dws[j], db, dgamma[j * Cout:(j + 1) * Cout], dbeta[j * Cout:(j + 1) * Cout]]
                continue
            dpack = _empty(Cout, K, like=inp)
            b_src = ctx.inp16 if (ctx.inp16 is not None and dy.dtype == torch.bfloat16
                                  and os.environ.get("TECM_DW_B16", "1")[:1] != "0") else inp
            gemm(Cout, K, M, dy, CT, b_src, ld_in, dpack, K, a_layout=A_KM, b_layout=B_KN, a_off=j * Cout,
                 b_win=win(N, Lc, Lc, 1, k, ld_in, (k - 1) // 2), split_k=pick_split_k(Cout, K, M, prec=bf16), bf16=bf16)
            dw = ops.conv_weight_unpack(dpack, Cout, ld_in, k)
            if ld_in != cin:
                dw = dw[:, :cin, :].contiguous()
            if need_dinp and not dx_seq:
                gemm(M, ld_in, k * Cout, dy, CT, bp, ld_in, dinp, ld_in, b_layout=B_KN, a_off=j * Cout,
                     a_win=win(N, Lc, Lc, 1, k, Cout, (k - 1) // 2), accumulate=(j > 0), bf16=bf16)
            grads += [dw, db, dgamma[j * Cout:(j + 1) * Cout], dbeta[j * Cout:(j + 1) * Cout]]
        return (dinp, None, None, None, None, None, None, *grads, dwf.view_as(wf), dbf)


class PatchEmbedFn(torch.autograd.Function):

    @staticmethod
    def forward(ctx, conv, conv16, Wp, bp, wpe, patch_len: int, plan: DropPlan):
        B, Lc, N, D = conv.shape
        P = Lc // patch_len
        d_llm = Wp.shape[0]
        M = B * P * N
        K = patch_len * D
        h0 = _empty(B, P, N, d_llm, like=conv)
        w = win(N, Lc, P, patch_len, patch_len, D, 0)
        dspec = plan.spec(SITE_EMBD, d_llm) if wpe is not None else None
        a_in = conv16 if (conv16 is not None and int(plan.bf16) == ops.PREC_BF16 and D % 8 == 0) else conv
        ctx.WpT16 = None
        Wf = Wp
        if a_in.dtype == torch.bfloat16 and D % 64 == 0 and P * patch_len == Lc and M >= 256 and d_llm >= 128:
            Wf, ctx.WpT16 = ops.weight_bf16(Wp, same=True, transposed=True)
        gemm(M, d_llm, K, a_in, D, Wf, K, h0, d_llm, a_win=w, bias=bp,
             rowbias=(wpe, wpe.shape[1], N, P) if wpe is not None else None, out_drop=dspec, bf16=plan.bf16)
        ctx.save_for_backward(a_in, Wp, wpe if wpe is not None else Wp)
        ctx.meta = (B, Lc, N, D, P, d_llm, patch_len, wpe is not None, dspec)
        ctx.plan = plan
        return h0

    @staticmethod
    def backward(ctx, dh0):
        conv, Wp, wpe = ctx.saved_tensors
        B, Lc, N, D, P, d_llm, patch_len, has_wpe, dspec = ctx.meta
        plan = ctx.plan
        M = B * P * N
        K = patch_len * D
        dh0 = dh0.contiguous()
        w = win(N, Lc, P, patch_len, patch_len, D, 0)
        t16 = int(plan.bf16) == ops.PREC_BF16 and conv.dtype == torch.bfloat16 and \
            ops.tn_ok(d_llm, K, M) and d_llm % 8 == 0
        dh16 = None
        cdrop = None
        if t16:
            dh16 = torch.empty(M, d_llm, device=dh0.device, dtype=torch.bfloat16)
            cdrop = dspec
        elif dspec is not None:
            dh0 = ops.dropout_apply(dh0, M, d_llm, dspec)
        dwpe = None
        if has_wpe:
            dwpe = torch.zeros_like(wpe)
            colsum(dh0, d_llm, B, N, P, d_llm, out=dwpe, in_drop=cdrop, twin=dh16)
            dbp = colsum(dwpe, d_llm, P, 1, 1, d_llm)[0]
        else:
            dbp = colsum(dh0, d_llm, M, 1, 1, d_llm, in_drop=cdrop, twin=dh16)[0]
        dWp = _empty(d_llm, K, like=conv)
        dg = dh16 if dh16 is not None else dh0
        gemm(d_llm, K, M, dg, d_llm, conv, D, dWp, K, a_layout=A_KM, b_layout=B_KN, b_win=w,
             split_k=pick_split_k(d_llm, K, M, prec=plan.bf16), bf16=plan.bf16)
        dconv = _empty(B, Lc, N, D, like=conv)
        if P * patch_len != Lc:
            dconv.zero_()
        if dh16 is not None and K % 8 == 0:
            WpT16 = ctx.WpT16 if ctx.WpT16 is not None else ops.weight_bf16(Wp, same=False, transposed=True)[1]
            gemm(M, K, d_llm, dh16, d_llm, WpT16, d_llm, dconv, D, c_win=w, bf16=plan.bf16)
        else:
            gemm(M, K, d_llm, dg, d_llm, Wp, K, dconv, D, b_layout=B_KN, c_win=w, bf16=plan.bf16)
        return dconv, None, dWp, dbp, dwpe, None, None


_NK_CACHE: dict = {}
_KEXT_GEN: dict = {}


def _frozen_copy(W: torch.Tensor, kind: str) -> Optional[torch.Tensor]:
    if W.requires_grad:
        return None
    key = (id(W), kind)
    hit = _NK_CACHE.get(key)
    if hit is not None and hit[0]() is W and hit[1] == W._version and hit[2] == W.data_ptr():
        return hit[3]
    if len(_NK_CACHE) > 256:
        for k in [k for k, v in _NK_CACHE.items() if v[0]() is None]:
            del _NK_CACHE[k]
    Wd = W.detach()
    if kind == "nk32":
        out = Wd.t().contiguous()
    elif kind == "nk16":
        out = Wd.t().contiguous().bfloat16()
    elif kind == "kn16":
        out = Wd.contiguous().bfloat16()
    elif kind in ("kext_kn32", "kext_kn16", "kext_nk32", "kext_nk16"):
        K, N = Wd.shape
        dt = torch.bfloat16 if kind.endswith("16") else torch.float32
        if "_kn" in kind:
            out = torch.zeros(K + LORA_R, N, device=W.device, dtype=dt)
            out[:K].copy_(Wd)
        else:
            out = torch.zeros(N, K + LORA_R, device=W.device, dtype=dt)
            out[:, :K].copy_(Wd.t())
    else:
        raise ValueError(kind)
    _NK_CACHE[key] = (weakref.ref(W), W._version, W.data_ptr(), out)
    return out


def invalidate_frozen_copies() -> None:
    _NK_CACHE.clear()


def _frozen_nk(W: torch.Tensor) -> Optional[torch.Tensor]:
    return _frozen_copy(W, "nk32")


def _fwd_weight(W: torch.Tensor, K: int, N: int, prec=0):
    wt = _frozen_copy(W, "nk16" if int(prec) == ops.PREC_BF16 else "nk32")
    return (wt, K, B_NK) if wt is not None else (W, N, B_KN)


def _bwd_weight(W: torch.Tensor, prec=0) -> torch.Tensor:
    if int(prec) == ops.PREC_BF16:
        w16 = _frozen_copy(W, "kn16")
        if w16 is not None:
            return w16
    return W


class GPT2StackFn(torch.autograd.Function):
    PER_LAYER = 14
    FROZEN_SLOTS = {2: "attn.c_attn.base_layer.weight", 3: "attn.c_attn.base_layer.bias", 6: "attn.c_proj.weight",
                    7: "attn.c_proj.bias", 10: "mlp.c_fc.weight", 11: "mlp.c_fc.bias", 12: "mlp.c_proj.weight",
                    13: "mlp.c_proj.bias"}

    @staticmethod
    def forward(ctx, h0, n_layers: int, plan: DropPlan, *params):
        for i in range(n_layers):
            for slot, name in GPT2StackFn.FROZEN_SLOTS.items():
                if params[i * GPT2StackFn.PER_LAYER + slot].requires_grad:
                    raise _lib_error(f"h.{i}.{name} has requires_grad=True: the MI355X path computes gradients for the "
                                     "LoRA, LayerNorm and wpe parameters only (the reference's freeze rule, "
                                     "modules.py:195-203); freeze the GPT-2 base weights")
        B, T, N, D = h0.shape
        M = B * T * N
        h = h0.contiguous()
        level = plan.recompute if plan.keep else 0
        saved: List[torch.Tensor] = []
        ctx_lAT: List[Optional[torch.Tensor]] = []
        ctx_gen: List[int] = []
        ctx_wk: list = []
        for i in range(n_layers):
            lp = params[i * GPT2StackFn.PER_LAYER:(i + 1) * GPT2StackFn.PER_LAYER]
            h3, acts, wk = GPT2StackFn._block_fwd(h, i, lp, plan, B, T, N, keep=plan.keep and level == 0)
            ctx_lAT.append(wk[3])
            ctx_gen.append(wk[4])
            if acts is not None:
                u_s, ud_s, st1, qkv, h2, st2, a = acts
                saved += [h, u_s, ud_s, st1, wk[0], qkv, h2, st2, a]
                del acts, u_s, ud_s, st1, qkv, h2, st2, a
            elif plan.keep:
                saved.append(h)
                ctx_wk.append(wk)
            h = h3
        lnfw, lnfb = params[n_layers * GPT2StackFn.PER_LAYER:]
        stf = _empty(M, 2, like=h)
        ctx.fused = bool(plan.fuse_head) and int(plan.bf16) == ops.PREC_BF16 and D % 8 == 0
        if ctx.fused:
            out = torch.empty(B, N, T * D, device=h.device, dtype=torch.bfloat16)
            pspec = plan.spec(SITE_POST, D)
            ops.layernorm_fwd(h, D, lnfw, lnfb, None, D, stf, M, D, y16d=out, ldy16d=D,
                              drop16d=pspec if pspec is not None else ops.NO_DROP, seq_major=(T, N))
        else:
            out = _empty(B, T, N, D, like=h)
            ops.layernorm_fwd(h, D, lnfw, lnfb, out, D, stf, M, D)
        ctx.save_for_backward(h, stf, *saved, *params)
        ctx.lAT16 = ctx_lAT
        ctx.kext_gen = ctx_gen
        ctx.wk = ctx_wk
        ctx.level = level
        ctx.meta = (B, T, N, D, n_layers, plan, len(saved))
        return out

    @staticmethod
    def _block_fwd(h, i: int, lp, plan: DropPlan, B: int, T: int, N: int, wk=None, out: bool = True, keep: bool = True):
        (ln1w, ln1b, Wqkv, bqkv, lA, lB, Wo, bo, ln2w, ln2b, Wfc, bfc, Wpr, bpr) = lp
        D = h.shape[-1]
        M = B * T * N
        KE = D + LORA_R
        F3, F4 = Wqkv.shape[1], Wfc.shape[1]
        b16 = int(plan.bf16) == ops.PREC_BF16
        wcatT = _frozen_copy(Wqkv, "kext_nk16" if b16 else "kext_nk32") if wk is None else wk[1]
        Wo_f, ldo_f, lay_o = _fwd_weight(Wo, D, D, plan.bf16)
        Wfc_f, ldfc_f, lay_fc = _fwd_weight(Wfc, D, F4, plan.bf16)
        Wpr_f, ldpr_f, lay_pr = _fwd_weight(Wpr, F4, D, plan.bf16)
        a16 = b16 and all(w is not None and w.dtype == torch.bfloat16 for w in (wcatT, Wo_f, Wfc_f, Wpr_f))
        st1 = _empty(M, 2, like=h)
        lspec = plan.spec(site_lora(i), KE)
        lA16 = lAT16 = None
        if a16:
            u = None
            u16 = torch.empty(M, KE, device=h.device, dtype=torch.bfloat16)
            u16d = torch.empty(M, D, device=h.device, dtype=torch.bfloat16) if lspec is not None else None
            ops.layernorm_fwd(h, D, ln1w, ln1b, None, KE, st1, M, D, y16=u16, ldy16=KE, y16d=u16d, ldy16d=D, drop16d=lspec)
            a_lora, ld_lora = (u16d, D) if u16d is not None else (u16, KE)
            lA16, lAT16 = ops.weight_bf16(lA, same=True, transposed=True) if wk is None else wk[2:4]
            gemm(M, LORA_R, D, a_lora, ld_lora, lA16, D, u16, KE, c_off=D, bf16=plan.bf16)
            del a_lora
        else:
            u = _empty(M, KE, like=h)
            u16 = u16d = None
            ops.layernorm_fwd(h, D, ln1w, ln1b, u, KE, st1, M, D)
            gemm(M, LORA_R, D, u, KE, lA, D, u, KE, c_off=D, a_drop=lspec, bf16=plan.bf16)
        if not keep:
            u16d = None
        if wk is None:
            wcat = _frozen_copy(Wqkv, "kext_kn16" if b16 else "kext_kn32")
            ops.lora_fold(lB.detach(), LORA_SCALE, wcat, wcatT, D)
            _KEXT_GEN[wcat.data_ptr()] = _KEXT_GEN.get(wcat.data_ptr(), 0) + 1
            wk = (wcat, wcatT, lA16, lAT16, _KEXT_GEN[wcat.data_ptr()])
        qkv = torch.empty(M, F3, device=h.device, dtype=torch.bfloat16 if (a16 and QKV16) else torch.float32)
        gemm(M, F3, KE, u16 if a16 else u, KE, wcatT, KE, qkv, F3, b_layout=B_NK, bias=bqkv, bf16=plan.bf16)
        if not keep:
            u = u16 = None
        cx = torch.empty(M, D, device=h.device, dtype=torch.bfloat16 if a16 else torch.float32)
        aspec = plan.spec(site_attn(i), 1)
        ops.attention_fwd(qkv, cx, B, T, N, GPT_HEADS, D, aspec)
        if not keep:
            qkv = None
        h2 = _empty(M, D, like=h)
        gemm(M, D, D, cx, D, Wo_f, ldo_f, h2, D, b_layout=lay_o, bias=bo, out_drop=plan.spec(site_res1(i), D),
             residual=(h, D), bf16=plan.bf16)
        if not keep:
            cx = None
        st2 = _empty(M, 2, like=h)
        if a16:
            u2 = torch.empty(M, D, device=h.device, dtype=torch.bfloat16)
            ops.layernorm_fwd(h2, D, ln2w, ln2b, None, D, st2, M, D, y16=u2, ldy16=D)
        else:
            u2 = _empty(M, D, like=h)
            ops.layernorm_fwd(h2, D, ln2w, ln2b, u2, D, st2, M, D)
        f16 = b16 and Wfc_f.dtype == torch.bfloat16 and Wpr_f.dtype == torch.bfloat16
        a = torch.empty(M, F4, device=h.device, dtype=torch.bfloat16 if f16 and PRE16 else torch.float32)
        f = torch.empty(M, F4, device=h.device, dtype=torch.bfloat16 if f16 else torch.float32)
        gemm(M, F4, D, u2, D, Wfc_f, ldfc_f, f, F4, b_layout=lay_fc, bias=bfc, preact=(a, F4), act=ACT_GELU_TANH,
             bf16=plan.bf16)
        if not keep:
            u2 = a = None
        h3 = None
        if out:
            h3 = _empty(M, D, like=h)
            gemm(M, D, F4, f, F4, Wpr_f, ldpr_f, h3, D, b_layout=lay_pr, bias=bpr, out_drop=plan.spec(site_res2(i), D),
                 residual=(h2, D), bf16=plan.bf16)
        del cx, u2, f
        if not keep:
            return h3, None, wk
        u_s, ud_s = (u16, (u16d if u16d is not None else h.new_empty(0))) if a16 else (u, h.new_empty(0))
        return h3, (u_s, ud_s, st1, qkv, h2, st2, a), wk

    @staticmethod
    def backward(ctx, dout):
        B, T, N, D, n_layers, plan, nsaved = ctx.meta
        tens = ctx.saved_tensors
        h_last, stf = tens[0], tens[1]
        saved = tens[2:2 + nsaved]
        params = tens[2 + nsaved:]
        M = B * T * N
        KE = D + LORA_R
        dout = dout.contiguous()
        lnfw = params[n_layers * GPT2StackFn.PER_LAYER]
        dh = _empty(M, D, like=dout)
        b16 = int(plan.bf16) == ops.PREC_BF16

        def masked_buf(sp_, W):
            if sp_ is None:
                return None
            w16 = b16 and _bwd_weight(W, plan.bf16).dtype == torch.bfloat16
            return torch.empty(M, D, device=dout.device, dtype=torch.bfloat16 if w16 else torch.float32)

        sp = plan.spec(site_res2(n_layers - 1), D)
        last_Wpr = params[(n_layers - 1) * GPT2StackFn.PER_LAYER + 12]
        dhm = masked_buf(sp, last_Wpr) if sp is not None else dh
        nig = ctx.needs_input_grad
        base_f = 3 + n_layers * GPT2StackFn.PER_LAYER
        dlnfw, dlnfb = ops.layernorm_bwd(dout, D, h_last, D, lnfw, stf, None, dh, M, D,
                                         dx_masked=dhm if sp is not None else None, mask_drop=sp,
                                         need_dgb=nig[base_f] or nig[base_f + 1],
                                         dy_seq_major=(T, N, plan.spec(SITE_POST, D)) if ctx.fused else None)
        pgrads: List[Optional[torch.Tensor]] = [None] * (n_layers * GPT2StackFn.PER_LAYER)
        for i in reversed(range(n_layers)):
            (ln1w, ln1b, Wqkv, bqkv, lA, lB, Wo, bo, ln2w, ln2b, Wfc, bfc, Wpr,
             bpr) = params[i * GPT2StackFn.PER_LAYER:(i + 1) * GPT2StackFn.PER_LAYER]
            if ctx.level == 0:
                h, u, ud, st1, wcat, qkv, h2, st2, a = saved[i * 9:(i + 1) * 9]
            else:
                h, wcat = saved[i], ctx.wk[i][0]
            if _KEXT_GEN.get(wcat.data_ptr()) != ctx.kext_gen[i]:
                raise _lib_error(f"GPT-2 block {i}: the K-extended c_attn operand [W ; 2 B^T] was rewritten by a later forward "
                                "of the same frozen base weight before this backward ran (shared cache buffer); run each "
                                "forward's backward before the next forward of that layer")
            if ctx.level:
                _, acts, _ = GPT2StackFn._block_fwd(h, i, params[i * GPT2StackFn.PER_LAYER:(i + 1) * GPT2StackFn.PER_LAYER],
                                                    plan, B, T, N, wk=ctx.wk[i], out=False)
                u, ud, st1, qkv, h2, st2, a = acts
                del acts
            F3, F4 = Wqkv.shape[1], Wfc.shape[1]
            Wpr_b, Wfc_b = _bwd_weight(Wpr, plan.bf16), _bwd_weight(Wfc, plan.bf16)
            da16 = Wpr_b.dtype == torch.bfloat16 and Wfc_b.dtype == torch.bfloat16
            da = torch.empty(M, F4, device=dh.device, dtype=torch.bfloat16 if da16 else torch.float32)
            gemm(M, F4, D, dhm, D, Wpr_b, D, da, F4, act=ACT_GELU_TANH, dact_src=(a, F4), bf16=plan.bf16)
            g16 = b16 and da16 and GRAD16
            du2 = torch.empty(M, D, device=dh.device, dtype=torch.bfloat16 if g16 else torch.float32)
            gemm(M, D, F4, da, F4, Wfc_b, F4, du2, D, bf16=plan.bf16)
            del da
            dh2 = _empty(M, D, like=dh)
            sp = plan.spec(site_res1(i), D)
            dh2m = masked_buf(sp, Wo) if sp is not None else dh2
            pb = 3 + i * GPT2StackFn.PER_LAYER
            dg2, db2 = ops.layernorm_bwd(du2, D, h2, D, ln2w, st2, dh, dh2, M, D,
                                         dx_masked=dh2m if sp is not None else None, mask_drop=sp,
                                         need_dgb=nig[pb + 8] or nig[pb + 9])
            Wo_b = _bwd_weight(Wo, plan.bf16)
            c16 = g16 and Wo_b.dtype == torch.bfloat16 and dh2m.dtype == torch.bfloat16 and qkv.dtype == torch.bfloat16
            dcx = torch.empty(M, D, device=dh.device, dtype=torch.bfloat16) if c16 else \
                (du2 if du2.dtype == torch.float32 else _empty(M, D, like=dh))
            gemm(M, D, D, dh2m, D, Wo_b, D, dcx, D, bf16=plan.bf16)
            q16 = b16 and wcat.dtype == torch.bfloat16
            dqkv = torch.empty(M, F3, device=dh.device, dtype=torch.bfloat16 if q16 else torch.float32)
            ops.attention_bwd(qkv, dcx, dqkv, B, T, N, GPT_HEADS, D, plan.spec(site_attn(i), 1))
            u16g = g16 and q16 and u.dtype == torch.bfloat16
            du = torch.empty(M, KE, device=dh.device, dtype=torch.bfloat16 if u16g else torch.float32)
            gemm(M, KE, F3, dqkv, F3, wcat, F3, du, KE, bf16=plan.bf16)
            lspec = plan.spec(site_lora(i), KE)
            dlB = _empty(F3, LORA_R, like=dh)
            gemm(F3, LORA_R, M, dqkv, F3, u, KE, dlB, LORA_R, a_layout=A_KM, b_layout=B_KN, b_off=D,
                 alpha=LORA_SCALE, split_k=pick_split_k(F3, LORA_R, M, prec=plan.bf16), bf16=plan.bf16)
            dlA = _empty(LORA_R, D, like=dh)
            if u.dtype == torch.bfloat16:
                b_in, ldb_in = (ud, D) if ud.numel() else (u, KE)
                gemm(LORA_R, D, M, du, KE, b_in, ldb_in, dlA, D, a_layout=A_KM, b_layout=B_KN, a_off=D,
                     split_k=pick_split_k(LORA_R, D, M, prec=plan.bf16), bf16=plan.bf16)
            else:
                gemm(LORA_R, D, M, du, KE, u, KE, dlA, D, a_layout=A_KM, b_layout=B_KN, a_off=D, b_drop=lspec,
                     split_k=pick_split_k(LORA_R, D, M, prec=plan.bf16), bf16=plan.bf16)
            dzA = torch.empty(M, D, device=dh.device, dtype=torch.bfloat16 if (b16 and GRAD16) else torch.float32)
            if ctx.lAT16[i] is not None and dzA.dtype == torch.bfloat16 and du.dtype == torch.bfloat16:
                gemm(M, D, LORA_R, du, KE, ctx.lAT16[i], LORA_R, dzA, D, a_off=D, bf16=plan.bf16)
            else:
                gemm(M, D, LORA_R, du, KE, lA, D, dzA, D, b_layout=B_KN, a_off=D, bf16=plan.bf16)
            dhn = _empty(M, D, like=dh)
            sp = plan.spec(site_res2(i - 1), D) if i > 0 else None
            dhm = masked_buf(sp, params[(i - 1) * GPT2StackFn.PER_LAYER + 12]) if sp is not None else dhn
            dg1, db1 = ops.layernorm_bwd(du, KE, h, D, ln1w, st1, dh2, dhn, M, D,
                                         dx_masked=dhm if sp is not None else None, mask_drop=sp,
                                         need_dgb=nig[pb + 0] or nig[pb + 1],
                                         add=(dzA, D, lspec))
            dh = dhn
            base = i * GPT2StackFn.PER_LAYER
            pgrads[base + 0], pgrads[base + 1] = dg1, db1
            pgrads[base + 4], pgrads[base + 5] = dlA, dlB
            pgrads[base + 8], pgrads[base + 9] = dg2, db2
            if ctx.level:
                del u, ud, st1, qkv, h2, st2, a, du2, dh2, dh2m, dcx, dqkv, du, dzA
        pg = [g if ctx.needs_input_grad[3 + j] else None for j, g in enumerate(pgrads)]
        return (dh.view(B, T, N, D), None, None, *pg, dlnfw, dlnfb)


class HeadFn(torch.autograd.Function):

    @staticmethod
    def forward(ctx, hid, W1, b1, W2, b2, plan: DropPlan):
        ctx.fused = hid.dim() == 3 and hid.dtype == torch.bfloat16
        if ctx.fused:
            return HeadFn._forward_fused(ctx, hid, W1, b1, W2, b2, plan)
        B, T, N, D = hid.shape
        S = B * N
        Hd, K1 = W1.shape
        Lo = W2.shape[0]
        w = win(N, T, 1, T, T, D, 0)
        pspec = plan.spec(SITE_POST, D)
        hspec = plan.spec(SITE_HEAD, Hd)
        pre = _empty(S, Hd, like=hid)
        h1 = _empty(S, Hd, like=hid)
        hid = hid.contiguous()
        h16 = int(plan.bf16) == ops.PREC_BF16 and D % 8 == 0 and ops.uses_bf16(Hd, K1, D, K1) and \
            ops.uses_bf16(K1, S, Hd, D, a_layout=A_KM, b_layout=B_KN)
        hd = ops.dropout_apply(hid, B * T * N, D, pspec, out_bf16=h16) if pspec is not None else hid
        gemm(S, Hd, K1, hd, D, W1, K1, h1, Hd, a_win=w, bias=b1, preact=(pre, Hd), act=ACT_GELU_ERF,
             out_drop=hspec, bf16=plan.bf16)
        pred = _empty(B, N, Lo, like=hid)
        gemm(S, Lo, Hd, h1, Hd, W2, Hd, pred, Lo, bias=b2, bf16=plan.bf16)
        ctx.save_for_backward(hd, W1, W2, pre, h1)
        ctx.meta = (B, T, N, D, Hd, K1, Lo, w, pspec, hspec)
        ctx.plan = plan
        return pred

    @staticmethod
    def _forward_fused(ctx, hid, W1, b1, W2, b2, plan: DropPlan):
        B, N, K1 = hid.shape
        S = B * N
        Hd = W1.shape[0]
        Lo = W2.shape[0]
        hspec = plan.spec(SITE_HEAD, Hd)
        W1_16, W1T16 = ops.weight_bf16(W1, same=True, transposed=True)
        pre = _empty(S, Hd, like=hid)
        h1 = _empty(S, Hd, like=hid)
        gemm(S, Hd, K1, hid, K1, W1_16, K1, h1, Hd, bias=b1, preact=(pre, Hd), act=ACT_GELU_ERF, out_drop=hspec, bf16=plan.bf16)
        pred = _empty(B, N, Lo, like=hid)
        gemm(S, Lo, Hd, h1, Hd, W2, Hd, pred, Lo, bias=b2, bf16=plan.bf16)
        ctx.save_for_backward(hid, W1, W2, pre, h1)
        ctx.W1T16 = W1T16
        ctx.meta = (B, N, K1, Hd, Lo, hspec)
        ctx.plan = plan
        return pred

    @staticmethod
    def _backward_fused(ctx, dpred):
        hid, W1, W2, pre, h1 = ctx.saved_tensors
        B, N, K1, Hd, Lo, hspec = ctx.meta
        plan = ctx.plan
        S = B * N
        dpred = dpred.contiguous()
        db2 = colsum(dpred, Lo, S, 1, 1, Lo)[0]
        dW2 = _empty(Lo, Hd, like=hid)
        gemm(Lo, Hd, S, dpred, Lo, h1, Hd, dW2, Hd, a_layout=A_KM, b_layout=B_KN, split_k=pick_split_k(Lo, Hd, S, prec=plan.bf16), bf16=plan.bf16)
        dpre = _empty(S, Hd, like=hid)
        gemm(S, Hd, Lo, dpred, Lo, W2, Hd, dpre, Hd, b_layout=B_KN, act=ACT_GELU_ERF, dact_src=(pre, Hd),
             out_drop=hspec, bf16=plan.bf16)
        dp = torch.empty(S, Hd, device=hid.device, dtype=torch.bfloat16)
        db1 = colsum(dpre, Hd, S, 1, 1, Hd, twin=dp)[0]
        dW1 = _empty(Hd, K1, like=hid)
        gemm(Hd, K1, S, dp, Hd, hid, K1, dW1, K1, a_layout=A_KM, b_layout=B_KN,
             split_k=pick_split_k(Hd, K1, S, prec=plan.bf16), bf16=plan.bf16)
        dhid = torch.empty(B, N, K1, device=hid.device, dtype=torch.bfloat16)
        gemm(S, K1, Hd, dp, Hd, ctx.W1T16, Hd, dhid, K1, bf16=plan.bf16)
        return dhid, dW1, db1, dW2, db2, None

    @staticmethod
    def backward(ctx, dpred):
        if ctx.fused:
            return HeadFn._backward_fused(ctx, dpred)
        hid, W1, W2, pre, h1 = ctx.saved_tensors
        B, T, N, D, Hd, K1, Lo, w, pspec, hspec = ctx.meta
        plan = ctx.plan
        S = B * N
        dpred = dpred.contiguous()
        db2 = colsum(dpred, Lo, S, 1, 1, Lo)[0]
        dW2 = _empty(Lo, Hd, like=hid)
        gemm(Lo, Hd, S, dpred, Lo, h1, Hd, dW2, Hd, a_layout=A_KM, b_layout=B_KN, split_k=pick_split_k(Lo, Hd, S, prec=plan.bf16), bf16=plan.bf16)
        dpre = _empty(S, Hd, like=hid)
        gemm(S, Hd, Lo, dpred, Lo, W2, Hd, dpre, Hd, b_layout=B_KN, act=ACT_GELU_ERF, dact_src=(pre, Hd),
             out_drop=hspec, bf16=plan.bf16)
        dW1 = _empty(Hd, K1, like=hid)
        if int(plan.bf16) == ops.PREC_BF16 and hid.dtype == torch.bfloat16 and ops.tn_ok(Hd, K1, S) and Hd % 8 == 0:
            dp = torch.empty(S, Hd, device=hid.device, dtype=torch.bfloat16)
            db1 = colsum(dpre, Hd, S, 1, 1, Hd, twin=dp)[0]
        else:
            dp = dpre
            db1 = colsum(dpre, Hd, S, 1, 1, Hd)[0]
        gemm(Hd, K1, S, dp, Hd, hid, D, dW1, K1, a_layout=A_KM, b_layout=B_KN, b_win=w,
             split_k=pick_split_k(Hd, K1, S, prec=plan.bf16), bf16=plan.bf16)
        dhid = _empty(B, T, N, D, like=hid)
        if dp.dtype == torch.bfloat16 and K1 % 8 == 0:
            W1T16 = ops.weight_bf16(W1, same=False, transposed=True)[1]
            gemm(S, K1, Hd, dp, Hd, W1T16, Hd, dhid, D, c_win=w, out_drop=pspec, bf16=plan.bf16)
        else:
            gemm(S, K1, Hd, dp, Hd, W1, K1, dhid, D, b_layout=B_KN, c_win=w, out_drop=pspec, bf16=plan.bf16)
        return dhid, dW1, db1, dW2, db2, None


class HuberFn(torch.autograd.Function):

    @staticmethod
    def forward(ctx, pred, target, delta: float):
        if pred.dim() == 4 and pred.shape[3] == 1 and pred.shape == target.shape:
            loss, dpred = ops.huber_fwd_bwd_strided(pred, target, delta, 1.0, want_grad=True)
        else:
            loss, dpred = ops.huber_fwd_bwd(pred.contiguous(), target.contiguous(), delta, 1.0, want_grad=True)
            dpred = dpred.view(pred.shape)
        ctx.save_for_backward(dpred)
        return loss[0]

    @staticmethod
    def backward(ctx, gloss):
        (dpred,) = ctx.saved_tensors
        return dpred * gloss, None, None
```

tec-mollm_amd/tecmollm/ops.py:

```python
from __future__ import annotations

import os
import ctypes as C
from typing import Optional, Tuple

import torch

from . import _lib
from ._lib import TecmDrop, TecmGemm, TecmWin, check, lib, ptr, stream_ptr

A_MK, A_KM = 0, 1
B_NK, B_KN = 0, 1
ACT_NONE, ACT_GELU_ERF, ACT_GELU_TANH = 0, 1, 2

_MASK64 = (1 << 64) - 1


def splitmix64(x: int) -> int:
    x = (x + 0x9E3779B97F4A7C15) & _MASK64
    z = x
    z = ((z ^ (z >> 30)) * 0xBF58476D1CE4E5B9) & _MASK64
    z = ((z ^ (z >> 27)) * 0x94D049BB133111EB) & _MASK64
    return z ^ (z >> 31)


def win(N: int, Lin: int, Lout: int, stride_t: int, taps: int, Cw: int, pad: int) -> TecmWin:
    return TecmWin(1, N, Lin, Lout, stride_t, taps, Cw, pad)


NO_WIN = TecmWin(0, 0, 0, 0, 0, 0, 0, 0)


SEED_WORD: Optional[torch.Tensor] = None


def drop(p: float, seed: int, ld: int) -> TecmDrop:
    return TecmDrop(float(p), 0, seed & _MASK64, int(ld), SEED_WORD.data_ptr() if SEED_WORD is not None else None)


NO_DROP = TecmDrop(0.0, 0, 0, 0, None)


def _off(t: torch.Tensor, col_off: int = 0) -> int:
    return t.data_ptr() + t.element_size() * col_off


def gemm(M: int, N: int, K: int, A: torch.Tensor, lda: int, B: torch.Tensor, ldb: int, Cout: torch.Tensor, ldc: int,
         *, a_layout: int = A_MK, b_layout: int = B_NK, a_off: int = 0, b_off: int = 0, c_off: int = 0,
         a_win: Optional[TecmWin] = None, b_win: Optional[TecmWin] = None, c_win: Optional[TecmWin] = None,
         a_drop: Optional[TecmDrop] = None, b_drop: Optional[TecmDrop] = None, out_drop: Optional[TecmDrop] = None,
         alpha: float = 1.0, act: int = ACT_NONE, bias: Optional[torch.Tensor] = None,
         rowbias: Optional[Tuple[torch.Tensor, int, int, int]] = None,
         preact: Optional[Tuple[torch.Tensor, int]] = None, dact_src: Optional[Tuple[torch.Tensor, int]] = None,
         residual: Optional[Tuple[torch.Tensor, int]] = None, accumulate: bool = False, split_k: int = 1,
         bf16: bool = False) -> None:
    g = TecmGemm()
    g.M, g.N, g.K = M, N, K
    io = (IO_A_BF16 if A.dtype == torch.bfloat16 else 0) | (IO_B_BF16 if B.dtype == torch.bfloat16 else 0) | \
         (IO_C_BF16 if Cout.dtype == torch.bfloat16 else 0)
    pre_dt = {t[0].dtype for t in (preact, dact_src) if t is not None}
    if len(pre_dt) > 1:
        raise ValueError("gemm: preact and dact_src must share a dtype")
    if pre_dt == {torch.bfloat16}:
        io |= IO_PRE_BF16
    if io:
        if int(bf16) != PREC_BF16:
            raise _lib.TecmError("bf16 tensors are accepted by the bf16 GEMM only")
        g.io_bf16 = io
    g.A, g.lda, g.a_layout = _off(A, a_off), lda, a_layout
    g.B, g.ldb, g.b_layout = _off(B, b_off), ldb, b_layout
    g.C, g.ldc = _off(Cout, c_off), ldc
    g.a_win = a_win or NO_WIN
    g.b_win = b_win or NO_WIN
    g.c_win = c_win or NO_WIN
    g.a_drop = a_drop or NO_DROP
    g.b_drop = b_drop or NO_DROP
    g.out_drop = out_drop or NO_DROP
    g.alpha, g.act = alpha, act
    g.bias = ptr(bias)
    if rowbias is not None:
        rb, rb_ld, rb_div, rb_mod = rowbias
        g.rowbias, g.rb_ld, g.rb_div, g.rb_mod = rb.data_ptr(), rb_ld, rb_div, rb_mod
    if preact is not None:
        g.preact, g.ldp = preact[0].data_ptr(), preact[1]
    if dact_src is not None:
        g.dact_src, g.ldd = dact_src[0].data_ptr(), dact_src[1]
    if residual is not None:
        g.residual, g.ldr = residual[0].data_ptr(), residual[1]
    g.accumulate = 1 if accumulate else 0
    g._p1 = GROUP_M
    ws = None
    if split_k > 1:
        ws = torch.empty(split_k * M * N, device=Cout.device, dtype=torch.float32)
        g.split_k, g.workspace = split_k, ws.data_ptr()
    else:
        g.split_k = 1
    mode = int(bf16)
    use16 = mode == PREC_BF16 and (io != 0 or _bf16_ok(g))
    use3 = mode in (PREC_BF16X3, PREC_BF16X6) and _x3_ok(g)
    fn, what = ((lib().tecm_gemm_bf16x6, "tecm_gemm_bf16x6") if (use3 and mode == PREC_BF16X6) else
                (lib().tecm_gemm_bf16x3, "tecm_gemm_bf16x3") if use3 else
                (lib().tecm_gemm_bf16, "tecm_gemm_bf16") if use16 else (lib().tecm_gemm_f32, "tecm_gemm_f32"))
    if _timing is None:
        check(fn(C.byref(g), stream_ptr()), what)
        return
    e0, e1 = torch.cuda.Event(enable_timing=True), torch.cuda.Event(enable_timing=True)
    e0.record()
    check(fn(C.byref(g), stream_ptr()), what)
    e1.record()
    name = ("gemm_x3_kernel<3,16>" if mode == PREC_BF16X6 else "gemm_x3_kernel<2,32>") if use3 else _kernel_name(g, use16)
    if _timing_detail:
        name += (f" M={M} N={N} K={K} win={g.a_win.enabled}{g.b_win.enabled}{g.c_win.enabled}"
                 f" drop={int(g.a_drop.p > 0)}{int(g.b_drop.p > 0)}{int(g.out_drop.p > 0)} split={g.split_k}"
                 f" act={g.act} acc={g.accumulate} dact={int(dact_src is not None)} res={int(residual is not None)}"
                 f" pre={int(preact is not None)}")
    ea, eb, ec = A.element_size(), B.element_size(), Cout.element_size()
    nbytes = (min(A.numel(), M * K) if g.a_win.enabled else M * K) * ea + (min(B.numel(), N * K) if g.b_win.enabled else N * K) * eb
    nbytes += M * N * ec * (2 if accumulate else 1)
    for t in (preact, dact_src, residual):
        if t is not None:
            nbytes += M * N * t[0].element_size()
    _timing.append((name, 2.0 * M * N * K, e0, e1, float(nbytes)))


PREC_FP32, PREC_BF16, PREC_BF16X3, PREC_BF16X6 = 0, 1, 2, 3
IO_A_BF16, IO_B_BF16, IO_C_BF16, IO_PRE_BF16 = 1, 2, 4, 8
GROUP_M = int(os.environ.get("TECM_GROUP_M", "0"))
BF16_MIN_N = 64


def uses_bf16(N: int, K: int, lda: int, ldb: int, a_layout: int = A_MK, b_layout: int = B_NK, cw_a: int = 4,
              cw_b: int = 4) -> bool:
    if N < BF16_MIN_N or lda % 4 or ldb % 4 or cw_a % 4 or cw_b % 4:
        return False
    if a_layout == A_MK and K % 4:
        return False
    return True


def uses_x3(N: int, K: int, lda: int, ldb: int, a_layout: int = A_MK, b_layout: int = B_NK, a_win: bool = False,
            b_win: bool = False, a_drop: bool = False, b_drop: bool = False) -> bool:
    if a_layout != A_MK or b_layout != B_NK or a_win or b_win or a_drop or b_drop:
        return False
    return N >= BF16_MIN_N and lda % 4 == 0 and ldb % 4 == 0 and K % 4 == 0


def _x3_ok(g: TecmGemm) -> bool:
    if not uses_x3(g.N, g.K, g.lda, g.ldb, g.a_layout, g.b_layout, bool(g.a_win.enabled), bool(g.b_win.enabled),
                   g.a_drop.p > 0, g.b_drop.p > 0):
        return False
    return g.A % 16 == 0 and g.B % 16 == 0


def _bf16_ok(g: TecmGemm) -> bool:
    if not uses_bf16(g.N, g.K, g.lda, g.ldb, g.a_layout, g.b_layout, g.a_win.Cw if g.a_win.enabled else 4,
                     g.b_win.Cw if g.b_win.enabled else 4):
        return False
    return g.A % 16 == 0 and g.B % 16 == 0


_timing = None
_timing_detail = False


def _vec(p: int, ld: int, w: TecmWin, inner_is_k: bool, K: int) -> int:
    v = 4
    while v > 1:
        ok = p % (4 * v) == 0 and ld % v == 0
        if w.enabled:
            ok = ok and w.Cw % v == 0
        if inner_is_k:
            ok = ok and K % v == 0
        if ok:
            break
        v >>= 1
    return v


def _kernel_name(g: TecmGemm, use16: bool = False) -> str:
    if use16:
        win16 = "true" if (g.a_win.enabled or g.b_win.enabled) else "false"
        drp16 = "true" if (g.a_drop.p > 0 or g.b_drop.p > 0) else "false"
        if (g.io_bf16 & (IO_A_BF16 | IO_B_BF16)) and not (g.a_layout == A_MK and g.b_layout == B_NK and win16 == "false"):
            win16 = "true"
        both16 = (g.io_bf16 & IO_A_BF16) and (g.io_bf16 & IO_B_BF16)
        streams = (1 if g.residual else 0) + (1 if g.dact_src else 0) + (1 if g.accumulate else 0)
        if g.c_win.enabled:
            fast_epi = streams == 0 and not g.rowbias and not g.preact and not (g.io_bf16 & (IO_C_BF16 | IO_PRE_BF16))
        else:
            fast_epi = streams == 0 if g.rowbias else streams <= 1
        p8 = os.environ.get("TECM_BF16_P8", "")[:1]

        def p8_takes(a_rows: int) -> bool:
            return (fast_epi and not os.environ.get("TECM_BF16_DMA", "") and p8 != "0" and g.K >= 128 and g.K % 32 == 0
                    and g.M >= 256 and g.N >= 128 and (p8 == "1" or g.N >= 768 or not 1 <= g.N % 256 <= 128)
                    and (a_rows * g.lda + 64) * 2 < 2 ** 32 and (g.N * g.ldb + 64) * 2 < 2 ** 32)
        if (both16 and g.a_layout == A_MK and g.b_layout == B_NK and g.a_win.enabled and not g.b_win.enabled and drp16 == "false"
                and g.a_win.pad == 0 and g.a_win.Cw % 64 == 0 and g.split_k <= 1 and g.M >= 256 and g.N >= 128
                and os.environ.get("TECM_BF16_DMA", "")[:1] != "0"):
            w = g.a_win
            if ((w.Lout - 1) * w.stride_t + w.taps <= w.Lin and g.M % (w.Lout * w.N) == 0
                    and p8_takes(g.M // (w.Lout * w.N) * w.Lin * w.N)):
                return f"gemm_bf16_p8_kernel<{lib().tecm_p8_rows(g.M, g.N)}>"
            return "gemm_bf16_dma_kernel"
        sel = os.environ.get("TECM_BF16_DMA", "")[:1]
        if (both16 and g.a_layout == A_MK and g.b_layout == B_NK and not g.a_win.enabled and not g.b_win.enabled
                and g.split_k <= 1 and g.N % 4 == 0 and g.K % 32 == 0 and g.K >= 32 and g.M >= 256
                and (g.N >= 128 or g.N == 32) and sel != "0"):
            k32, n_small = g.K < 64, g.N < 128
            can16 = not g.c_win.enabled and not g.rowbias and streams <= 1
            if p8_takes(g.M):
                return f"gemm_bf16_p8_kernel<{lib().tecm_p8_rows(g.M, g.N)}>"
            narrow = n_small or (sel == "2" if (sel and not k32) else 1 <= g.N % 256 <= 128)
            if narrow:
                return "gemm_bf16_dma2_kernel"
            ring = sel == "4"
            can16 = not g.c_win.enabled and not g.rowbias and \
                (1 if g.residual else 0) + (1 if g.dact_src else 0) + (1 if g.accumulate else 0) <= 1
            if can16 and sel in ("6", "7"):
                return "gemm_bf16_dma6_kernel<256,128,2,2>" if sel == "6" else "gemm_bf16_dma6_kernel<128,256,1,4>"
            want16 = sel in ("5", "8") if (sel and not k32) else True
            if can16 and want16:
                tn_ = (g.N + 255) // 256
                cost = lambda bm: ((((g.M + bm - 1) // bm) * tn_ + 255) // 256) * bm
                tall = True if sel == "8" else (False if (sel == "5" or os.environ.get("TECM_BF16_TALL", "")[:1] == "0")
                                                else cost(288) * 100 < cost(256) * 95)
                return "gemm_bf16_dma5w_kernel" if tall else "gemm_bf16_dma5_kernel"
            return "gemm_bf16_dma4_kernel" if ring else ("gemm_bf16_dma3_kernel" if sel == "3" else "gemm_bf16_dma_kernel")
        if (both16 and g.a_layout == A_KM and g.b_layout == B_KN and g.split_k >= 2 and not g.a_win.enabled
                and (not g.b_win.enabled or g.b_win.pad == 0) and os.environ.get("TECM_BF16_TN", "")[:1] != "0"
                and lib().tecm_gemm_tn_splits(g.M, g.N, g.K) > 0):
            return "gemm_bf16_tn_kernel"
        return f"gemm_bf16_kernel<{g.a_layout},{g.b_layout},{win16},{drp16}>"
    av = _vec(g.A, g.lda, g.a_win, g.a_layout == A_MK, g.K)
    bv = _vec(g.B, g.ldb, g.b_win, g.b_layout == B_NK, g.K)
    if av == 4 and bv == 4:
        pair = (4, 4)
    elif g.a_layout == A_MK:
        pair = (2, 1) if av >= 2 else (1, 1)
    else:
        pair = (4, 2) if (av == 4 and bv >= 2) else (1, 1)
    bn = 32 if g.N <= 32 else (64 if g.N <= 64 else 128)
    m64 = ",64" if (g.a_layout == A_KM and g.M <= 64 and bn > 32 and pair == (4, 4)) else ",128"
    if pair == (4, 4):
        win = bool(g.a_win.enabled or g.b_win.enabled)
        drp = bool(g.a_drop.p > 0 or g.b_drop.p > 0)
    else:
        win = drp = True
    flags = f",{'true' if win else 'false'},{'true' if drp else 'false'}"
    return f"gemm_kernel<{g.a_layout},{g.b_layout},{pair[0]},{pair[1]},{bn}{flags}{m64}>"


def enable_gemm_timing(detail: bool = False) -> list:
    global _timing, _timing_detail
    _timing = []
    _timing_detail = detail
    return _timing


def disable_gemm_timing() -> None:
    global _timing
    _timing = None


def summarize_gemm_timing(records: list) -> dict:
    torch.cuda.synchronize()
    agg: dict = {}
    for rec in records:
        name, flops, e0, e1 = rec[:4]
        a = agg.setdefault(name, {"ms": 0.0, "flops": 0.0, "n": 0, "bytes": 0.0})
        a["ms"] += e0.elapsed_time(e1)
        a["flops"] += flops
        a["bytes"] += rec[4] if len(rec) > 4 else 0.0
        a["n"] += 1
    return agg


def tn_ok(Mo: int, No: int, K: int) -> bool:
    return os.environ.get("TECM_BF16_TN", "")[:1] != "0" and lib().tecm_gemm_tn_splits(Mo, No, K) >= 2


def pick_split_k(Mo: int, No: int, K: int, target_blocks: int = 512, min_chunk: int = 512,
                 max_splits: int = 256, prec: int = 0) -> int:
    if int(prec) == PREC_BF16:
        tn = lib().tecm_gemm_tn_splits(Mo, No, K)
        if tn >= 2:
            return int(tn)
    if int(prec) == PREC_BF16 and No >= BF16_MIN_N:
        tiles = ((Mo + 255) // 256) * ((No + 127) // 128)
        s = max(1, 256 // max(tiles, 1))
        return int(min(s, max(1, K // min_chunk), max_splits))
    tiles = ((Mo + 127) // 128) * ((No + 127) // 128 if No > 64 else 1)
    s = max(1, target_blocks // max(tiles, 1))
    s = min(s, max(1, K // min_chunk), max_splits)
    return int(s)


def layernorm_fwd(x: torch.Tensor, ldx: int, gamma: torch.Tensor, beta: torch.Tensor, y: Optional[torch.Tensor], ldy: int,
                  stats: torch.Tensor, M: int, D: int, eps: float = 1e-5, y_off: int = 0,
                  y16: Optional[torch.Tensor] = None, ldy16: int = 0, y16d: Optional[torch.Tensor] = None, ldy16d: int = 0,
                  drop16d: Optional[TecmDrop] = None, seq_major: Optional[Tuple[int, int]] = None) -> None:
    for t, what in ((y16, "y16"), (y16d, "y16d")):
        if t is not None and t.dtype != torch.bfloat16:
            raise _lib.TecmError(f"layernorm_fwd: {what} must be a bfloat16 tensor")
    if y16d is not None and drop16d is None:
        raise _lib.TecmError("layernorm_fwd: y16d needs its dropout spec")
    sT, sN = seq_major if seq_major is not None else (0, 0)
    check(lib().tecm_layernorm_fwd(x.data_ptr(), ldx, gamma.data_ptr(), beta.data_ptr(),
                                   None if y is None else _off(y, y_off), ldy, ptr(y16), ldy16, ptr(y16d), ldy16d,
                                   C.byref(drop16d) if drop16d is not None else None, sT, sN,
                                   stats.data_ptr(), M, D, eps, stream_ptr()), "tecm_layernorm_fwd")


def _ln_add(add) -> Optional["_lib.TecmLnAdd"]:
    if add is None:
        return None
    dy2, ld, dspec = add
    if dy2.dtype not in (torch.float32, torch.bfloat16):
        raise _lib.TecmError("layernorm_bwd: dy2 is fp32 or bf16")
    return _lib.TecmLnAdd(dy2=dy2.data_ptr(), ld=ld, bf16=1 if dy2.dtype == torch.bfloat16 else 0,
                          drop=dspec if dspec is not None else NO_DROP)


def layernorm_bwd_blocks(M: int, D: int) -> int:
    nb = C.c_int32(0)
    check(lib().tecm_layernorm_bwd(None, 0, None, 0, None, None, None, None, None, 0, None, None, C.byref(nb), M, D,
                                   None, 0, None, None), "tecm_layernorm_bwd(query)")
    return nb.value


def layernorm_bwd(dy: torch.Tensor, lddy: int, x: torch.Tensor, ldx: int, gamma: torch.Tensor, stats: torch.Tensor,
                  dres: Optional[torch.Tensor], dx: torch.Tensor, M: int, D: int,
                  dx_masked: Optional[torch.Tensor] = None,
                  mask_drop: Optional[TecmDrop] = None, need_dgb: bool = True, add=None, dy_seq_major=None):
    m16 = 1 if (dx_masked is not None and dx_masked.dtype == torch.bfloat16) else 0
    ad = _ln_add(add)
    dy16 = 1 if dy.dtype == torch.bfloat16 else 0
    nb = layernorm_bwd_blocks(M, D)
    partials = torch.empty(nb, 2 * D, device=dx.device, dtype=torch.float32)
    nbc = C.c_int32(0)
    od = mask_drop if mask_drop is not None else NO_DROP
    dm = None
    if dy_seq_major is not None:
        mT, mN, mdrop = dy_seq_major
        dm = _lib.TecmLnDyMap(T=mT, N=mN, drop=mdrop if mdrop is not None else NO_DROP)
    check(lib().tecm_layernorm_bwd(dy.data_ptr(), lddy, x.data_ptr(), ldx, gamma.data_ptr(), stats.data_ptr(),
                                   ptr(dres), dx.data_ptr(), ptr(dx_masked), m16, C.byref(od), partials.data_ptr(),
                                   C.byref(nbc), M, D, C.byref(ad) if ad is not None else None, dy16,
                                   C.byref(dm) if dm is not None else None, stream_ptr()),
          "tecm_layernorm_bwd")
    if not need_dgb:
        return None, None
    dgb = colsum(partials, 2 * D, nb, 1, 1, 2 * D)
    return dgb[0, :D], dgb[0, D:]


GN_Y_BF16, GN_OUT_BF16, GN_DACT_BF16 = 1, 2, 4


def gn_reg_ok(L: int, N: int, Cout: int) -> bool:
    quads = L * (3 * Cout // 4)
    if L * N * 3 * Cout >= 1 << 31:
        return False
    return any(quads % (64 * wps) == 0 and quads // (64 * wps) <= 9 for wps in (4, 8))


def _gn_io(y: torch.Tensor, out: torch.Tensor) -> int:
    if y.dtype == torch.bfloat16:
        if out.dtype != torch.bfloat16:
            raise _lib.TecmError("groupnorm_gelu: a bf16 y comes with bf16 act / dact / dy")
        return GN_Y_BF16 | GN_OUT_BF16
    if y.dtype != torch.float32:
        raise _lib.TecmError("groupnorm_gelu: y is fp32 or bf16")
    return GN_OUT_BF16 if out.dtype == torch.bfloat16 else 0


def gn_y16_ok(L: int, N: int, Cout: int) -> bool:
    return os.environ.get("TECM_Y16", "1")[:1] != "0" and lib().tecm_gn_y16_supported(L, N, Cout) == 1


GN_STATS_GIVEN = 8


def groupnorm_gelu_fwd(y: torch.Tensor, gamma: torch.Tensor, beta: torch.Tensor, act: torch.Tensor,
                       stats: torch.Tensor, B: int, L: int, N: int, Cout: int, eps: float = 1e-5, act_stride: int = 1,
                       stats_given: bool = False) -> None:
    La = (L + act_stride - 1) // act_stride
    if act.numel() != B * La * N * 3 * Cout:
        raise _lib.TecmError(f"groupnorm_gelu_fwd: act must hold (B, {La}, N, 3*Cout) values for act_stride {act_stride}")
    io = _gn_io(y, act)
    if stats_given:
        if io != (GN_Y_BF16 | GN_OUT_BF16):
            raise _lib.TecmError("groupnorm_gelu_fwd: given statistics go with a bf16 y and a bf16 act")
        io |= GN_STATS_GIVEN
    check(lib().tecm_groupnorm_gelu_fwd(y.data_ptr(), gamma.data_ptr(), beta.data_ptr(), act.data_ptr(),
                                        stats.data_ptr(), B, L, N, Cout, eps, io, act_stride, stream_ptr()),
          "tecm_groupnorm_gelu_fwd")


def groupnorm_gelu_bwd(dact: torch.Tensor, dstride: int, y: torch.Tensor, gamma: torch.Tensor, beta: torch.Tensor,
                       stats: torch.Tensor, dy: torch.Tensor, B: int, L: int, N: int,
                       Cout: int) -> Tuple[torch.Tensor, torch.Tensor, torch.Tensor]:
    nb = C.c_int32(0)
    check(lib().tecm_groupnorm_gelu_bwd(None, dstride, None, None, None, None, None, None, C.byref(nb), B, L, N, Cout,
                                        0, None, None), "tecm_groupnorm_gelu_bwd(query)")
    CT = 3 * Cout
    partials = torch.empty(nb.value, 3 * CT, device=dy.device, dtype=torch.float32)
    io = _gn_io(y, dy)
    if dact.dtype == torch.bfloat16:
        if not io:
            raise _lib.TecmError("groupnorm_gelu_bwd: a bf16 dact comes with a bf16 dy")
        io |= GN_DACT_BF16
    elif io & GN_Y_BF16:
        raise _lib.TecmError("groupnorm_gelu_bwd: a bf16 y comes with a bf16 dact")
    sums = torch.empty(B * N * 6, device=dy.device, dtype=torch.float32) if (io & GN_Y_BF16) else None
    check(lib().tecm_groupnorm_gelu_bwd(dact.data_ptr(), dstride, y.data_ptr(), gamma.data_ptr(), beta.data_ptr(),
                                        stats.data_ptr(), dy.data_ptr(), partials.data_ptr(), C.byref(nb), B, L, N,
                                        Cout, io, ptr(sums), stream_ptr()), "tecm_groupnorm_gelu_bwd")
    dgb = colsum(partials, 3 * CT, nb.value, 1, 1, 3 * CT)
    return dgb[0, :CT], dgb[0, CT:2 * CT], dgb[0, 2 * CT:]


ATT_OUT_BF16, ATT_QKV_BF16, ATT_DCTX_BF16 = 1, 2, 4


def attention_fwd(qkv: torch.Tensor, ctx: torch.Tensor, B: int, T: int, N: int, heads: int, D: int,
                  prob_drop: Optional[TecmDrop] = None) -> None:
    pd = prob_drop if prob_drop is not None else NO_DROP
    io = (ATT_OUT_BF16 if ctx.dtype == torch.bfloat16 else 0) | (ATT_QKV_BF16 if qkv.dtype == torch.bfloat16 else 0)
    check(lib().tecm_attention_fwd(qkv.data_ptr(), ctx.data_ptr(), io, B, T, N, heads, D, C.byref(pd), stream_ptr()),
          "tecm_attention_fwd")


def attention_bwd(qkv: torch.Tensor, dctx: torch.Tensor, dqkv: torch.Tensor, B: int, T: int, N: int, heads: int,
                  D: int, prob_drop: Optional[TecmDrop] = None) -> None:
    pd = prob_drop if prob_drop is not None else NO_DROP
    io = (ATT_OUT_BF16 if dqkv.dtype == torch.bfloat16 else 0) | (ATT_QKV_BF16 if qkv.dtype == torch.bfloat16 else 0) | \
        (ATT_DCTX_BF16 if dctx.dtype == torch.bfloat16 else 0)
    check(lib().tecm_attention_bwd(qkv.data_ptr(), dctx.data_ptr(), dqkv.data_ptr(), io, B, T, N, heads, D, C.byref(pd),
                                   stream_ptr()), "tecm_attention_bwd")


def colsum(inp: torch.Tensor, ld: int, outer: int, inner: int, nseg: int, Cn: int, *, in_off: int = 0,
           scale: float = 1.0, in_drop: Optional[TecmDrop] = None, out: Optional[torch.Tensor] = None,
           accumulate: bool = False, twin: Optional[torch.Tensor] = None) -> torch.Tensor:
    if out is None:
        out = torch.empty(nseg, Cn, device=inp.device, dtype=torch.float32)
    ws = torch.empty(1024 * nseg * Cn, device=inp.device, dtype=torch.float32)
    idr = in_drop if in_drop is not None else NO_DROP
    if twin is not None and not (Cn % 4 == 0 and Cn <= 1024 and ld % 4 == 0):
        if in_drop is not None or ld != Cn or in_off:
            raise _lib.TecmError("colsum: a bf16 twin of a masked or strided input needs Cn % 4 == 0 and Cn <= 1024")
        cast_bf16(inp, Cn, twin, Cn, outer * nseg * inner, Cn)
        twin = None
    if twin is not None:
        if twin.dtype != torch.bfloat16 or twin.numel() != outer * nseg * inner * Cn:
            raise _lib.TecmError("colsum: twin must be a contiguous bf16 tensor of the input's rows x Cn")
        check(lib().tecm_colsum_twin(_off(inp, in_off), ld, outer, inner, nseg, Cn, out.data_ptr(), Cn, 1 if accumulate else 0,
                                     scale, C.byref(idr), ws.data_ptr(), twin.data_ptr(), Cn, stream_ptr()), "tecm_colsum_twin")
        return out
    check(lib().tecm_colsum(_off(inp, in_off), ld, outer, inner, nseg, Cn, out.data_ptr(), Cn, 1 if accumulate else 0,
                            scale, C.byref(idr), ws.data_ptr(), stream_ptr()), "tecm_colsum")
    return out


def cast_bf16(src: torch.Tensor, lds: int, dst: torch.Tensor, ldd: int, rows: int, cols: int, src_off: int = 0,
              dst_off: int = 0) -> None:
    check(lib().tecm_cast_bf16(src.data_ptr() + 4 * src_off, lds, dst.data_ptr() + 2 * dst_off, ldd, rows, cols,
                               stream_ptr()), "tecm_cast_bf16")


def dropout_apply(src: torch.Tensor, rows: int, cols: int, spec: TecmDrop, ld: Optional[int] = None,
                  out_bf16: bool = False, twin_bf16: bool = False):
    dst = torch.empty_like(src, dtype=torch.bfloat16 if out_bf16 else torch.float32)
    twin = torch.empty_like(src, dtype=torch.bfloat16) if twin_bf16 else None
    ld = cols if ld is None else ld
    check(lib().tecm_dropout_apply(src.data_ptr(), ld, dst.data_ptr(), ld, 1 if out_bf16 else 0, ptr(twin), ld, rows, cols,
                                   C.byref(spec), stream_ptr()), "tecm_dropout_apply")
    return (dst, twin) if twin_bf16 else dst


def weight_bf16(W: torch.Tensor, same: bool = True, transposed: bool = False):
    R, Cc = W.shape
    s = torch.empty(R, Cc, device=W.device, dtype=torch.bfloat16) if same else None
    t = torch.empty(Cc, R, device=W.device, dtype=torch.bfloat16) if transposed else None
    check(lib().tecm_weight_bf16(W.data_ptr(), Cc, ptr(s), Cc, ptr(t), R, R, Cc, stream_ptr()), "tecm_weight_bf16")
    return s, t


def bf16_twin(src: torch.Tensor, rows: int, cols: int) -> torch.Tensor:
    dst = torch.empty(src.shape, device=src.device, dtype=torch.bfloat16)
    cast_bf16(src, cols, dst, cols, rows, cols)
    return dst


def huber_fwd_bwd(pred: torch.Tensor, target: torch.Tensor, delta: float = 1.0, grad_scale: float = 1.0,
                  want_grad: bool = True) -> Tuple[torch.Tensor, Optional[torch.Tensor]]:
    n = pred.numel()
    loss = torch.empty(1, device=pred.device, dtype=torch.float32)
    dpred = torch.empty_like(pred) if want_grad else None
    ws = torch.empty(1024, device=pred.device, dtype=torch.float32)
    check(lib().tecm_huber_fwd_bwd(pred.data_ptr(), target.data_ptr(), ptr(dpred), loss.data_ptr(), n, delta,
                                   grad_scale, ws.data_ptr(), stream_ptr()), "tecm_huber_fwd_bwd")
    return loss, dpred


def huber_fwd_bwd_strided(pred: torch.Tensor, target: torch.Tensor, delta: float = 1.0, grad_scale: float = 1.0,
                          want_grad: bool = True) -> Tuple[torch.Tensor, Optional[torch.Tensor]]:
    if pred.shape != target.shape or pred.dim() != 4 or pred.shape[3] != 1:
        raise _lib.TecmError("huber_fwd_bwd_strided: pred and target are (B, L_out, N, 1) tensors of one shape")
    _lib.require_gpu_tensor(pred, "pred")
    _lib.require_gpu_tensor(target, "target")
    B, H, N, _ = pred.shape
    loss = torch.empty(1, device=pred.device, dtype=torch.float32)
    dpred = torch.empty_strided(pred.shape, pred.stride(), device=pred.device, dtype=torch.float32) if want_grad else None
    if want_grad and max(st * (sz - 1) for st, sz in zip(pred.stride(), pred.shape)) + 1 > pred.numel():
        raise _lib.TecmError("huber_fwd_bwd_strided: pred must be a dense (permuted) tensor")
    ws = torch.empty(1024, device=pred.device, dtype=torch.float32)
    ps = (C.c_int64 * 3)(*pred.stride()[:3])
    tst = (C.c_int64 * 3)(*target.stride()[:3])
    check(lib().tecm_huber_fwd_bwd_strided(pred.data_ptr(), ps, target.data_ptr(), tst, ptr(dpred), loss.data_ptr(), B, H, N,
                                           delta, grad_scale, ws.data_ptr(), stream_ptr()), "tecm_huber_fwd_bwd_strided")
    return loss, dpred


def lora_fold(lB: torch.Tensor, scale: float, w_kn: Optional[torch.Tensor], w_nk: Optional[torch.Tensor], k_off: int) -> None:
    n, r = lB.shape
    for w, shape in ((w_kn, (k_off + r, n)), (w_nk, (n, k_off + r))):
        if w is not None and (tuple(w.shape) != shape or not w.is_contiguous() or w.dtype not in (torch.float32, torch.bfloat16)):
            raise _lib.TecmError(f"lora_fold: operand must be a contiguous {shape} fp32 / bf16 tensor")
    check(lib().tecm_lora_fold(lB.data_ptr(), n, r, float(scale), ptr(w_kn), n, int(w_kn is not None and w_kn.dtype == torch.bfloat16),
                               ptr(w_nk), k_off + r, int(w_nk is not None and w_nk.dtype == torch.bfloat16), k_off,
                               stream_ptr()), "tecm_lora_fold")


def pack_vectors(vecs, out: Optional[torch.Tensor] = None) -> torch.Tensor:
    vecs = [v.detach() for v in vecs]
    if any(v.dtype != torch.float32 or not v.is_contiguous() or v.dim() != 1 for v in vecs) or not 1 <= len(vecs) <= 12:
        raise _lib.TecmError("pack_vectors: 1..12 contiguous fp32 vectors")
    total = sum(v.numel() for v in vecs)
    if out is None:
        out = torch.empty(total, device=vecs[0].device, dtype=torch.float32)
    srcs = (C.c_void_p * len(vecs))(*[v.data_ptr() for v in vecs])
    lens = (C.c_int32 * len(vecs))(*[v.numel() for v in vecs])
    check(lib().tecm_pack_vectors(srcs, lens, len(vecs), out.data_ptr(), stream_ptr()), "tecm_pack_vectors")
    return out


def conv_weight_pack(w: torch.Tensor, want_bwd: bool = True) -> Tuple[torch.Tensor, Optional[torch.Tensor]]:
    Cout, Cin, k = w.shape
    fwd = torch.empty(Cout, k * Cin, device=w.device, dtype=torch.float32)
    bwd = torch.empty(k * Cout, Cin, device=w.device, dtype=torch.float32) if want_bwd else None
    check(lib().tecm_conv_weight_pack(w.data_ptr(), fwd.data_ptr(), ptr(bwd), Cout, Cin, k, stream_ptr()),
          "tecm_conv_weight_pack")
    return fwd, bwd


def conv_weight_unpack(dpack: torch.Tensor, Cout: int, Cin: int, k: int) -> torch.Tensor:
    dw = torch.empty(Cout, Cin, k, device=dpack.device, dtype=torch.float32)
    check(lib().tecm_conv_weight_unpack(dpack.data_ptr(), dw.data_ptr(), Cout, Cin, k, stream_ptr()),
          "tecm_conv_weight_unpack")
    return dw


def conv_dx_seq_ok(Lc: int, Cout: int, ld_in: int, f32: bool = False) -> bool:
    return (os.environ.get("TECM_CONV_SEQ", "1")[:1] != "0"
            and lib().tecm_conv_dx_supported(Lc, Cout, ld_in, 1 if f32 else 0) == 1)


def conv_dx(dy: torch.Tensor, w3: torch.Tensor, w5: torch.Tensor, w7: torch.Tensor, dinp: torch.Tensor, B: int,
            Lc: int, N: int, Cout: int, cin: int, ld_in: int) -> None:
    if dinp.dtype != torch.float32 or dy.dtype not in (torch.bfloat16, torch.float32):
        raise _lib.TecmError("conv_dx: dy is bf16 or fp32, dinp fp32")
    f32 = dy.dtype == torch.float32
    nci = (ld_in + 31) // 32
    wpack = torch.empty(15 * Cout * nci * 32, device=dy.device, dtype=dy.dtype)
    pack, run, what = ((lib().tecm_conv_dx_pack_f32, lib().tecm_conv_dx_f32, "tecm_conv_dx_f32") if f32 else
                       (lib().tecm_conv_dx_pack, lib().tecm_conv_dx_bf16, "tecm_conv_dx_bf16"))
    check(pack(w3.data_ptr(), w5.data_ptr(), w7.data_ptr(), wpack.data_ptr(), Cout, cin, ld_in, stream_ptr()), what + "/pack")
    d = _lib.TecmConvDx(dy=dy.data_ptr(), wpack=wpack.data_ptr(), dinp=dinp.data_ptr(), B=B, Lc=Lc, N=N, Cout=Cout,
                        ld_in=ld_in)
    if _timing is None:
        check(run(C.byref(d), stream_ptr()), what)
        return
    e0, e1 = torch.cuda.Event(enable_timing=True), torch.cuda.Event(enable_timing=True)
    e0.record()
    check(run(C.byref(d), stream_ptr()), what)
    e1.record()
    name = ("conv_dx_seq_f32_kernel" if f32 else "conv_dx_seq_kernel") + \
        (f" M={B * Lc * N} N={ld_in} K={15 * Cout}" if _timing_detail else "")
    _timing.append((name, 2.0 * B * Lc * N * ld_in * 15 * Cout, e0, e1))


conv_dx_bf16 = conv_dx


def conv_dw_seq_ok(Lc: int, Cout: int, ld_in: int) -> bool:
    return (Lc % 4 == 0 and Lc > 0 and Cout in (64, 128) and ld_in in (24, 64)
            and os.environ.get("TECM_CONV_DW_SEQ", "1")[:1] != "0")


_cu_count = {}


def conv_dw(inp: torch.Tensor, dy: torch.Tensor, B: int, Lc: int, N: int, Cout: int, cin: int, ld_in: int):
    if inp.dtype != dy.dtype or dy.dtype not in (torch.bfloat16, torch.float32):
        raise _lib.TecmError("conv_dw: inp and dy are both bf16 or both fp32 tensors")
    f32 = dy.dtype == torch.float32
    run, what = (lib().tecm_conv_dw_f32, "tecm_conv_dw_f32") if f32 else (lib().tecm_conv_dw_bf16, "tecm_conv_dw_bf16")
    dev = dy.device
    nb = _cu_count.get(dev.index)
    if nb is None:
        nb = _cu_count[dev.index] = int(os.environ.get("TECM_CONV_DW_BLOCKS", 0)) or \
            torch.cuda.get_device_properties(dev).multi_processor_count
    nws = lib().tecm_conv_dw_workspace(Cout, ld_in, nb)
    if nws <= 0:
        raise _lib.TecmError(f"conv_dw: no kernel for Cout={Cout}, ld_in={ld_in}")
    ws = torch.empty(nws, device=dev, dtype=torch.float32)
    dws = [torch.empty(Cout, cin, k, device=dev, dtype=torch.float32) for k in (3, 5, 7)]
    d = _lib.TecmConvDw(inp=inp.data_ptr(), dy=dy.data_ptr(), workspace=ws.data_ptr(), dw3=dws[0].data_ptr(),
                        dw5=dws[1].data_ptr(), dw7=dws[2].data_ptr(), B=B, Lc=Lc, N=N, Cout=Cout, Cin=cin, ld_in=ld_in,
                        num_blocks=nb)
    if _timing is None:
        check(run(C.byref(d), stream_ptr()), what)
        return dws
    e0, e1 = torch.cuda.Event(enable_timing=True), torch.cuda.Event(enable_timing=True)
    e0.record()
    check(run(C.byref(d), stream_ptr()), what)
    e1.record()
    name = ("conv_dw_seq_f32_kernel" if f32 else "conv_dw_seq_kernel") + (f" M={15 * ld_in} N={Cout} K={B * Lc * N}" if _timing_detail else "")
    _timing.append((name, 2.0 * B * Lc * N * ld_in * 15 * Cout, e0, e1))
    return dws


def conv_fwd_seq_ok(Lc: int, Cout: int, ld_in: int, f32: bool = False) -> bool:
    return (os.environ.get("TECM_CONV_SEQ", "1")[:1] != "0" and os.environ.get("TECM_CONV_FWD_SEQ", "1")[:1] != "0"
            and lib().tecm_conv_fwd_supported(Lc, Cout, ld_in, 1 if f32 else 0) == 1)


def conv_fwd_stats_ok(Lc: int) -> bool:
    return Lc <= 48 and os.environ.get("TECM_CONV_STATS", "1")[:1] != "0"


def conv_fwd(inp: torch.Tensor, w3: torch.Tensor, w5: torch.Tensor, w7: torch.Tensor, bias: torch.Tensor,
             y: torch.Tensor, B: int, Lc: int, N: int, Cout: int, cin: int, ld_in: int,
             stats: Optional[torch.Tensor] = None, eps: float = 1e-5) -> None:
    if inp.dtype not in (torch.bfloat16, torch.float32) or y.dtype not in (torch.bfloat16, torch.float32) or \
            (y.dtype == torch.bfloat16 and inp.dtype != torch.bfloat16):
        raise _lib.TecmError("conv_fwd: inp is bf16 or fp32, y fp32 (or bf16 next to a bf16 inp)")
    f32 = inp.dtype == torch.float32
    if f32:
        nval = sum(((3 + 2 * j) * ld_in // 8) * (Cout // 32) for j in range(3)) * 256
        pack, run, what = lib().tecm_conv_fwd_pack_f32, lib().tecm_conv_fwd_f32, "tecm_conv_fwd_f32"
    else:
        nval = sum((((3 + 2 * j) * ld_in + 15) // 16) * (Cout // 32) for j in range(3)) * 512
        pack, run, what = lib().tecm_conv_fwd_pack, lib().tecm_conv_fwd_bf16, "tecm_conv_fwd_bf16"
    wpack = torch.empty(nval, device=y.device, dtype=inp.dtype)
    check(pack(w3.data_ptr(), w5.data_ptr(), w7.data_ptr(), wpack.data_ptr(), Cout, cin, ld_in, stream_ptr()), what + "/pack")
    d = _lib.TecmConvFwd(inp=inp.data_ptr(), wpack=wpack.data_ptr(), bias=bias.data_ptr(), y=y.data_ptr(), B=B, Lc=Lc,
                         N=N, Cout=Cout, ld_in=ld_in, y_bf16=1 if y.dtype == torch.bfloat16 else 0,
                         stats=ptr(stats), eps=eps)
    if _timing is None:
        check(run(C.byref(d), stream_ptr()), what)
        return
    e0, e1 = torch.cuda.Event(enable_timing=True), torch.cuda.Event(enable_timing=True)
    e0.record()
    check(run(C.byref(d), stream_ptr()), what)
    e1.record()
    name = ("conv_fwd_seq_f32_kernel" if f32 else "conv_fwd_seq_kernel") + \
        (f" M={B * Lc * N} N={3 * Cout} K={5 * ld_in}(avg)" if _timing_detail else "")
    _timing.append((name, 2.0 * B * Lc * N * Cout * 15 * ld_in, e0, e1))


conv_fwd_bf16 = conv_fwd


def transpose_scale(src: torch.Tensor, lds: int, dst: torch.Tensor, ldd: int, rows: int, cols: int, scale: float,
                    dst_off: int = 0) -> None:
    check(lib().tecm_transpose_scale(src.data_ptr(), lds, _off(dst, dst_off), ldd, rows, cols, scale, stream_ptr()),
          "tecm_transpose_scale")
```

Measured before the change: 126.9 samples/s.

## Add segmented windowed A loads, edge-tile wave split-K, and stored GELU derivative

Result: no change. 127.6 samples/s, median of 6 (+0.5%).

```diff
diff --git a/include/tecmollm.h b/include/tecmollm.h
--- a/include/tecmollm.h
+++ b/include/tecmollm.h
@@ -37,7 +37,8 @@
 
 enum { TECM_A_MK = 0, TECM_A_KM = 1 };
 enum { TECM_B_NK = 0, TECM_B_KN = 1 };
-enum { TECM_ACT_NONE = 0, TECM_ACT_GELU_ERF = 1, TECM_ACT_GELU_TANH = 2 };
+enum { TECM_ACT_NONE = 0, TECM_ACT_GELU_ERF = 1, TECM_ACT_GELU_TANH = 2,
+       TECM_ACT_GELU_TANH_D = 3 };
 
 #define TECM_IO_A_BF16 1
 #define TECM_IO_B_BF16 2
diff --git a/tec-mollm_amd/csrc/common.h b/tec-mollm_amd/csrc/common.h
--- a/tec-mollm_amd/csrc/common.h
+++ b/tec-mollm_amd/csrc/common.h
@@ -95,12 +95,17 @@
   gelu_tanh_parts(x, x * x, s, r);
   return x * s;
 }
-__device__ __forceinline__ float dgelu_tanh(float x) {
+__device__ __forceinline__ float gelu_tanh_both(float x, float& y) {
   const float x2 = x * x;
   float s, r;
   gelu_tanh_parts(x, x2, s, r);
+  y = x * s;
   const float du2 = fmaf(x2, 0.21406445f, 1.5957691f);
   return fmaf(x * du2 * r, s, s);
+}
+__device__ __forceinline__ float dgelu_tanh(float x) {
+  float y;
+  return gelu_tanh_both(x, y);
 }
 __device__ __forceinline__ float apply_act(int act, float v) {
   return act == TECM_ACT_GELU_ERF ? gelu_erf(v) : (act == TECM_ACT_GELU_TANH ? gelu_tanh(v) : v);
diff --git a/tec-mollm_amd/csrc/gemm.hip b/tec-mollm_amd/csrc/gemm.hip
--- a/tec-mollm_amd/csrc/gemm.hip
+++ b/tec-mollm_amd/csrc/gemm.hip
@@ -1,4 +1,5 @@
 #include "gemm_bf16_impl.h"
+#include <cstdlib>
 int tecm_gemm_x3_dispatch(const TecmGemm& g, int products, hipStream_t st);
 
 namespace {
@@ -63,6 +64,19 @@
     v >>= 1;
   }
   return v;
+}
+
+bool env_on(const char* name) {
+  const char* v = std::getenv(name);
+  return !(v && v[0] == '0');
+}
+
+bool a_win_segmented(const TecmGemm& g, int avec, int bvec, bool drop) {
+  const TecmWin& w = g.a_win;
+  if (!w.enabled || g.b_win.enabled || drop || avec != 4 || bvec != 4 || g.a_layout != TECM_A_MK) return false;
+  if (w.pad != 0 || (int64_t)(w.Lout - 1) * w.stride_t + w.taps > w.Lin) return false;
+  if (w.Cw % tecm_gemm::BK != 0 || g.M % ((int64_t)w.Lout * w.N) != 0) return false;
+  return env_on("TECM_GEMM_SEGK");
 }
 
 bool win_ok(const TecmWin& w) {
@@ -158,6 +172,10 @@
   }
   TecmGemm gk = g;
   gk.io_bf16 = io | (vec4 ? TECM_P0_VEC4 : 0);
+  if (mode == MODE_F32 && env_on("TECM_GEMM_EDGE")) gk.io_bf16 |= TECM_P0_EDGE;
+  if (g.act == TECM_ACT_GELU_TANH_D)
+    TECM_REQUIRE(mode == MODE_F32 && !p16, TECM_E_ARG,
+                 "tecm_gemm: TECM_ACT_GELU_TANH_D (stored GELU') is served by tecm_gemm_f32 with fp32 preact / dact_src only");
   const bool erf = g.act == TECM_ACT_GELU_ERF;
   if (erf) {
     TECM_REQUIRE(!g.residual && !g.accumulate && !g.c_win.enabled, TECM_E_ARG,
@@ -166,6 +184,7 @@
     gk.dact_src = nullptr;
     gk.out_drop.p = 0.f;
   }
+  const bool win32 = win && !a_win_segmented(g, avec, bvec, drop);
   int splits;
   if (mode == MODE_X3 || mode == MODE_X6) {
     splits = tecm_gemm_x3_dispatch(gk, mode == MODE_X6 ? 6 : 3, st);
@@ -177,11 +196,11 @@
     else
       splits = tecm_gemm16_dispatch_km_kn(gk, win, drop, st);
   } else if (g.a_layout == TECM_A_MK && g.b_layout == TECM_B_NK)
-    splits = tecm_gemm_dispatch_mk_nk(gk, avec, bvec, win, drop, st);
+    splits = tecm_gemm_dispatch_mk_nk(gk, avec, bvec, win32, drop, st);
   else if (g.a_layout == TECM_A_MK)
-    splits = tecm_gemm_dispatch_mk_kn(gk, avec, bvec, win, drop, st);
+    splits = tecm_gemm_dispatch_mk_kn(gk, avec, bvec, win32, drop, st);
   else
-    splits = tecm_gemm_dispatch_km_kn(gk, avec, bvec, win, drop, st);
+    splits = tecm_gemm_dispatch_km_kn(gk, avec, bvec, win32, drop, st);
   if (splits < 0) return splits;
   if (splits > 1) {
     const int64_t total = g.M * g.N;
diff --git a/tec-mollm_amd/csrc/gemm_impl.h b/tec-mollm_amd/csrc/gemm_impl.h
--- a/tec-mollm_amd/csrc/gemm_impl.h
+++ b/tec-mollm_amd/csrc/gemm_impl.h
@@ -15,6 +15,7 @@
 typedef float f32x4 __attribute__((ext_vector_type(4)));
 
 #define TECM_P0_VEC4 0x100
+#define TECM_P0_EDGE 0x200
 
 namespace tecm_gemm {
 
@@ -137,7 +138,19 @@
   int32_t rn[(WIN && ROWK) ? NV : 1], rt[(WIN && ROWK) ? NV : 1], rb[(WIN && ROWK) ? NV : 1];
   int32_t tap, c;
   int32_t kk;
-
+  int32_t seg_left, seg_len;
+  int64_t seg_jump;
+
+  template <bool SEG>
+  __device__ __forceinline__ int64_t seg_advance() {
+    if constexpr (!SEG) return BK;
+    const bool cross = seg_left <= BK;
+    const int64_t adv = BK + (cross ? seg_jump : (int64_t)0);
+    seg_left = cross ? seg_len : seg_left - BK;
+    return adv;
+  }
+
+  template <bool SEG = false>
   __device__ __forceinline__ void init(const float* __restrict__ P, const TecmWin& w, int64_t ld, int64_t row0,
                                        int64_t rows_total, int32_t kbeg, int64_t fixed0, int64_t fixed_lim,
                                        const DropCtx& dc) {
@@ -149,14 +162,34 @@
     c = 0;
     kk = kbeg + cv;
     const bool wen = WIN && w.enabled;
+    seg_left = 0x7fffffff;
+    seg_len = 0;
+    seg_jump = 0;
     if (!wen) {
       if constexpr (!ROWK) {
+        bool seg = false;
+        int32_t tap0 = 0, c0 = 0;
+        if constexpr (SEG && !WIN) {
+          if (w.enabled) {
+            seg = true;
+            tap0 = kbeg / w.Cw;
+            c0 = kbeg - tap0 * w.Cw;
+            seg_len = w.Cw;
+            seg_left = w.Cw - c0;
+            seg_jump = (int64_t)w.N * ld - w.Cw;
+          }
+        }
 #pragma unroll
         for (int i = 0; i < NV; ++i) {
           int64_t row = row0 + r0 + i * RSTEP;
           if (row < rows_total) rowok |= 1u << i;
           else row = rows_total - 1;
-          ptr[i] = P + row * ld + kbeg + cv;
+          if (seg) {
+            const WinRow wrow = win_row(w, row, rows_total);
+            ptr[i] = P + (wrow.srow + (int64_t)tap0 * w.N) * ld + c0 + cv;
+          } else {
+            ptr[i] = P + row * ld + kbeg + cv;
+          }
           if constexpr (DROP) didx[i] = row * dc.ld + kbeg + cv;
         }
       } else {
@@ -192,11 +225,12 @@
     }
   }
 
+  template <bool SEG = false>
   __device__ __forceinline__ void load(Tile& tl, const float* __restrict__ P, const TecmWin& w, int64_t ld, int32_t k0,
                                        int32_t klim, const DropCtx& dc) {
-    load_part<0, NV>(tl, P, w, ld, k0, klim, dc);
-  }
-  template <int IB, int IE>
+    load_part<0, NV, SEG>(tl, P, w, ld, k0, klim, dc);
+  }
+  template <int IB, int IE, bool SEG = false>
   __device__ __forceinline__ void load_part(Tile& tl, const float* __restrict__ P, const TecmWin& w, int64_t ld, int32_t k0,
                                             int32_t klim, const DropCtx& dc) {
     if constexpr (IB >= IE) return;
@@ -206,13 +240,15 @@
     if (!wen) {
       if constexpr (!ROWK) {
         const bool kok = kk < klim;
+        static_assert(!SEG || (IB == 0 && IE == NV), "the segment state advances once per whole tile");
+        const int64_t adv = seg_advance<SEG && !WIN>();
 #pragma unroll
         for (int i = IB; i < IE; ++i) {
           const bool ok = kok && ((rowok >> i) & 1u);
           gload<VEC>(ptr[i], P, ok, tl.regs[i]);
           tl.okbits = (tl.okbits & ~(1u << i)) | ((ok ? 1u : 0u) << i);
           if constexpr (DROP) { tl.dsave[i] = didx[i]; didx[i] += BK; }
-          ptr[i] += BK;
+          ptr[i] += adv;
         }
         if constexpr (LAST) kk += BK;
       } else {
@@ -262,14 +298,17 @@
     }
   }
 
+  template <bool SEG = false>
   __device__ __forceinline__ void load_steady(Tile& tl, int64_t ld, const DropCtx& dc) {
     tl.okbits = ~0u;
+    int64_t adv = BK;
+    if constexpr (!ROWK) adv = seg_advance<SEG && !WIN>();
 #pragma unroll
     for (int i = 0; i < NV; ++i) {
       gload<VEC>(ptr[i], ptr[i], true, tl.regs[i]);
       if constexpr (!ROWK) {
         if constexpr (DROP) { tl.dsave[i] = didx[i]; didx[i] += BK; }
-        ptr[i] += BK;
+        ptr[i] += adv;
       } else {
         if constexpr (DROP) { tl.dsave[i] = didx[i]; didx[i] += (int64_t)BK * dc.ld; }
         ptr[i] += (int64_t)BK * ld;
@@ -361,10 +400,17 @@
   const int32_t n = c.n;
   v = v * g.alpha + c.bias;
   if (r.rb) v += r.rb[n];
-  if (g.preact) g.preact[r.m * g.ldp + n] = v;
-  if (g.dact_src)
-    v *= dgelu_tanh(g.dact_src[r.m * g.ldd + n]);
-  else if (g.act)
+  const bool dstore = g.act == TECM_ACT_GELU_TANH_D;
+  if (g.preact && !dstore) g.preact[r.m * g.ldp + n] = v;
+  if (g.dact_src) {
+    const float t = g.dact_src[r.m * g.ldd + n];
+    v *= dstore ? t : dgelu_tanh(t);
+  } else if (dstore) {
+    float y;
+    const float d = gelu_tanh_both(v, y);
+    if (g.preact) g.preact[r.m * g.ldp + n] = d;
+    v = y;
+  } else if (g.act)
     v = gelu_tanh(v);
   int64_t off, didx;
   if (g.c_win.enabled) {
@@ -397,7 +443,8 @@
     o[0] += t.x; o[1] += t.y; o[2] += t.z; o[3] += t.w;
   }
   const bool p16 = (g.io_bf16 & TECM_IO_PRE_BF16) != 0;
-  if (g.preact) {
+  const bool dstore = g.act == TECM_ACT_GELU_TANH_D;
+  if (g.preact && !dstore) {
     if (p16) {
       tecm_bf16x4 h;
       h[0] = (__bf16)o[0]; h[1] = (__bf16)o[1]; h[2] = (__bf16)o[2]; h[3] = (__bf16)o[3];
@@ -415,8 +462,17 @@
     } else {
       t = *reinterpret_cast<const float4*>(g.dact_src + r.m * g.ldd + n);
     }
-    o[0] *= dgelu_tanh(t.x); o[1] *= dgelu_tanh(t.y);
-    o[2] *= dgelu_tanh(t.z); o[3] *= dgelu_tanh(t.w);
+    if (dstore) {
+      o[0] *= t.x; o[1] *= t.y; o[2] *= t.z; o[3] *= t.w;
+    } else {
+      o[0] *= dgelu_tanh(t.x); o[1] *= dgelu_tanh(t.y);
+      o[2] *= dgelu_tanh(t.z); o[3] *= dgelu_tanh(t.w);
+    }
+  } else if (dstore) {
+    float d[4];
+#pragma unroll
+    for (int e = 0; e < 4; ++e) d[e] = gelu_tanh_both(o[e], o[e]);
+    if (g.preact) *reinterpret_cast<float4*>(g.preact + r.m * g.ldp + n) = make_float4(d[0], d[1], d[2], d[3]);
   } else if (g.act) {
 #pragma unroll
     for (int e = 0; e < 4; ++e) o[e] = gelu_tanh(o[e]);
@@ -492,7 +548,7 @@
     }
   }
 }
-enum { EPI_F_PRE = 1, EPI_F_P16 = 2, EPI_F_ACT = 4, EPI_F_DROP = 8, EPI_F_C16 = 16 };
+enum { EPI_F_PRE = 1, EPI_F_P16 = 2, EPI_F_ACT = 4, EPI_F_DROP = 8, EPI_F_C16 = 16, EPI_F_DSTORE = 32 };
 template <int FEAT, int BIT>
 __device__ __forceinline__ bool epi_feat(bool dynamic) {
   if constexpr (FEAT < 0) return dynamic;
@@ -508,6 +564,7 @@
   const bool has_pre = epi_feat<FEAT, EPI_F_PRE>(g.preact != nullptr);
   const bool has_act = epi_feat<FEAT, EPI_F_ACT>(g.act != 0);
   const bool has_drop = epi_feat<FEAT, EPI_F_DROP>(odc.thresh != 0);
+  const bool dstore = epi_feat<FEAT, EPI_F_DSTORE>(g.act == TECM_ACT_GELU_TANH_D);
   constexpr int GRP = NIT < 4 ? NIT : 4;
   static_assert(NIT % GRP == 0, "row groups are read from the staging rows in whole batches");
   const int32_t mb = (int32_t)mrow0 + lrow;
@@ -542,7 +599,7 @@
         else *dst = hv;
       }
       o[0] = (float)hv[0]; o[1] = (float)hv[1]; o[2] = (float)hv[2]; o[3] = (float)hv[3];
-    } else if (has_pre && row_ok) {
+    } else if (has_pre && !dstore && row_ok) {
       if constexpr (NT) {
         f32x4 nv = {o[0], o[1], o[2], o[3]};
         __builtin_nontemporal_store(nv, reinterpret_cast<f32x4*>(g.preact + (offP0 + it * stepP)));
@@ -557,10 +614,19 @@
         t0 = __builtin_bit_cast(float, lo << 16); t1 = __builtin_bit_cast(float, lo & 0xffff0000u);
         t2 = __builtin_bit_cast(float, hi << 16); t3 = __builtin_bit_cast(float, hi & 0xffff0000u);
       }
-      o[0] *= dgelu_tanh(t0); o[1] *= dgelu_tanh(t1);
-      o[2] *= dgelu_tanh(t2); o[3] *= dgelu_tanh(t3);
+      if (dstore) {
+        o[0] *= t0; o[1] *= t1; o[2] *= t2; o[3] *= t3;
+      } else {
+        o[0] *= dgelu_tanh(t0); o[1] *= dgelu_tanh(t1);
+        o[2] *= dgelu_tanh(t2); o[3] *= dgelu_tanh(t3);
+      }
     } else {
-      if (has_act) {
+      if (MODE == 0 && dstore) {
+        float d[4];
+#pragma unroll
+        for (int e = 0; e < 4; ++e) d[e] = gelu_tanh_both(o[e], o[e]);
+        if (has_pre && row_ok) *reinterpret_cast<float4*>(g.preact + (offP0 + it * stepP)) = make_float4(d[0], d[1], d[2], d[3]);
+      } else if (has_act) {
 #pragma unroll
         for (int e = 0; e < 4; ++e) o[e] = gelu_tanh(o[e]);
       }
@@ -624,8 +690,9 @@
   const int streams = (g.residual ? 1 : 0) + (g.dact_src ? 1 : 0) + (g.accumulate ? 1 : 0);
   if (g.c_win.enabled)
     return (streams == 0 && !g.rowbias && !g.preact && !(g.io_bf16 & (TECM_IO_C_BF16 | TECM_IO_PRE_BF16))) ? 6 : -1;
-  if (g.rowbias) return streams == 0 ? 5 : -1;
-  if (streams > 1) return -1;
+  const bool dfwd = g.act == TECM_ACT_GELU_TANH_D && !g.dact_src;
+  if (g.rowbias) return (streams == 0 && !dfwd) ? 5 : -1;
+  if (streams > 1 || (dfwd && streams)) return -1;
   return g.residual ? 1 : (g.dact_src ? 2 : (g.accumulate ? 3 : 0));
 }
 template <int SLABS, int NIT, int RPI, int STG_LD, bool NT = false, bool SPECIAL = false, typename StageFn>
@@ -774,9 +841,21 @@
   BStager sb;
   typename AStager::Tile ta;
   typename BStager::Tile tb;
-  sa.init(g.A, g.a_win, g.lda, m0, g.M, kbeg, m0, g.M, adc);
+  constexpr bool SEGA = ALAY == TECM_A_MK && !WIN;
+  sa.template init<SEGA>(g.A, g.a_win, g.lda, m0, g.M, kbeg, m0, g.M, adc);
   sb.init(g.B, g.b_win, g.ldb, n0, g.N, kbeg, n0, g.N, bdc);
 
+  constexpr bool EDGE_OK = NWAVES == 8 && WN == 4 && NT == 1 && AVEC == 4 && BVEC == 4 && ALAY == TECM_A_MK && !WIN && !DROP &&
+                           TECM_ABLATE == 0;
+  int eL = WN;
+  if constexpr (EDGE_OK) {
+    const int64_t rem = g.N - n0;
+    if ((g.io_bf16 & TECM_P0_EDGE) && rem <= 2 * WTN) eL = rem > WTN ? 2 : 1;
+  }
+  const bool edge = EDGE_OK && eL < WN;
+  const int uwn = __builtin_amdgcn_readfirstlane(wn);
+  const int ecol = eL == 2 ? (uwn & 1) : 0, epart = eL == 2 ? (uwn >> 1) : uwn, emask = eL == 2 ? 1 : 3;
+
   f32x16 acc[MT][NT];
 #pragma unroll
   for (int i = 0; i < MT; ++i)
@@ -785,7 +864,7 @@
 #pragma unroll
       for (int e = 0; e < 16; ++e) acc[i][j][e] = 0.f;
 
-  auto read_frags = [&](const float* As, const float* Bs, auto qc, float (&af)[MT][4], float (&bf)[NT][4]) {
+  auto read_frags_at = [&](const float* As, const float* Bs, auto qc, int wcol, float (&af)[MT][4], float (&bf)[NT][4]) {
     constexpr int q = decltype(qc)::value;
 #pragma unroll
     for (int i = 0; i < MT; ++i) {
@@ -800,7 +879,7 @@
     }
 #pragma unroll
     for (int i = 0; i < NT; ++i) {
-      const int col = wn * WTN + i * 32 + r;
+      const int col = wcol * WTN + i * 32 + r;
       if constexpr (BLAY == TECM_B_NK) {
         const float4 v = *reinterpret_cast<const float4*>(&Bs[col * LDK + 8 * q + 4 * h]);
         bf[i][0] = v.x; bf[i][1] = v.y; bf[i][2] = v.z; bf[i][3] = v.w;
@@ -810,6 +889,9 @@
       }
     }
   };
+  auto read_frags = [&](const float* As, const float* Bs, auto qc, float (&af)[MT][4], float (&bf)[NT][4]) {
+    read_frags_at(As, Bs, qc, wn, af, bf);
+  };
   auto do_mfma = [&](const float (&af)[MT][4], const float (&bf)[NT][4]) {
 #pragma unroll
     for (int j = 0; j < 4; ++j)
@@ -823,10 +905,10 @@
   {
     typename AStager::Tile ta0;
     typename BStager::Tile tb0;
-    sa.load(ta0, g.A, g.a_win, g.lda, kbeg, kend, adc);
+    sa.template load<SEGA>(ta0, g.A, g.a_win, g.lda, kbeg, kend, adc);
     sb.load(tb0, g.B, g.b_win, g.ldb, kbeg, kend, bdc);
     if (kbeg + BK < kend) {
-      sa.load(ta, g.A, g.a_win, g.lda, kbeg + BK, kend, adc);
+      sa.template load<SEGA>(ta, g.A, g.a_win, g.lda, kbeg + BK, kend, adc);
       sb.load(tb, g.B, g.b_win, g.ldb, kbeg + BK, kend, bdc);
     }
     sa.store(ta0, smem, adc);
@@ -859,10 +941,10 @@
           }
         }
         if constexpr (FULL && !WIN && TECM_ABLATE != 4) {
-          sa.load_steady(ta, g.lda, adc);
+          sa.template load_steady<SEGA>(ta, g.lda, adc);
           sb.load_steady(tb, g.ldb, bdc);
         } else if ((FULL && TECM_ABLATE != 4) || (!FULL && k0 + 2 * BK < kend)) {
-          sa.load(ta, g.A, g.a_win, g.lda, k0 + 2 * BK, kend, adc);
+          sa.template load<SEGA>(ta, g.A, g.a_win, g.lda, k0 + 2 * BK, kend, adc);
           sb.load(tb, g.B, g.b_win, g.ldb, k0 + 2 * BK, kend, bdc);
         }
       }
@@ -886,8 +968,72 @@
     });
   };
 
+  auto tile_body_edge = [&](const float* Ac, const float* Bc, float* An, int32_t k0, auto fullc) {
+    constexpr bool FULL = decltype(fullc)::value;
+    static_for<4>([&](auto qc) {
+      constexpr int q = decltype(qc)::value;
+      if ((q & emask) == epart) {
+        read_frags_at(Ac, Bc, qc, ecol, fa[0], fb[0]);
+        do_mfma(fa[0], fb[0]);
+      }
+      if constexpr (q == TECM_STAGE_Q) {
+        if constexpr (FULL) {
+          sa.store_steady(ta, An, adc);
+          sb.store_steady(tb, An + A_FLOATS, bdc);
+          sa.template load_steady<SEGA>(ta, g.lda, adc);
+          sb.load_steady(tb, g.ldb, bdc);
+        } else {
+          if (k0 + BK < kend) {
+            sa.store(ta, An, adc);
+            sb.store(tb, An + A_FLOATS, bdc);
+          }
+          if (k0 + 2 * BK < kend) {
+            sa.template load<SEGA>(ta, g.A, g.a_win, g.lda, k0 + 2 * BK, kend, adc);
+            sb.load(tb, g.B, g.b_win, g.ldb, k0 + 2 * BK, kend, bdc);
+          }
+        }
+      }
+    });
+  };
+
   int cur = 0;
   int32_t k0 = kbeg;
+  if (EDGE_OK && edge) {
+    if constexpr (EDGE_OK) {
+      for (; k0 + 3 * BK <= kend; k0 += BK) {
+        tile_body_edge(smem + cur * TILE_FLOATS, smem + cur * TILE_FLOATS + A_FLOATS, smem + (cur ^ 1) * TILE_FLOATS, k0,
+                       std::true_type{});
+        __syncthreads();
+        cur ^= 1;
+      }
+      for (; k0 < kend; k0 += BK) {
+        tile_body_edge(smem + cur * TILE_FLOATS, smem + cur * TILE_FLOATS + A_FLOATS, smem + (cur ^ 1) * TILE_FLOATS, k0,
+                       std::false_type{});
+        __syncthreads();
+        cur ^= 1;
+      }
+      constexpr int WSTG = WTM * STG_LD;
+      static_assert(WSTG >= MT * 16 * 64, "a wave's staging rows hold its accumulators");
+      if (epart > 0) {
+        float* red = smem + wave * WSTG;
+#pragma unroll
+        for (int i = 0; i < MT; ++i)
+#pragma unroll
+          for (int e = 0; e < 16; ++e) red[(i * 16 + e) * 64 + lane] = acc[i][0][e];
+      }
+      __syncthreads();
+      if (epart == 0) {
+        for (int p = 1; p <= emask; ++p) {
+          const float* red = smem + (wm * WN + p * eL + ecol) * WSTG;
+#pragma unroll
+          for (int i = 0; i < MT; ++i)
+#pragma unroll
+            for (int e = 0; e < 16; ++e) acc[i][0][e] += red[(i * 16 + e) * 64 + lane];
+        }
+      }
+      __syncthreads();
+    }
+  } else {
   for (; k0 + 3 * BK <= kend; k0 += BK) {
     tile_body(smem + cur * TILE_FLOATS, smem + cur * TILE_FLOATS + A_FLOATS, smem + (cur ^ 1) * TILE_FLOATS, k0,
               std::true_type{});
@@ -899,6 +1045,7 @@
               std::false_type{});
     __syncthreads();
     cur ^= 1;
+  }
   }
 
 #ifdef TECM_ABLATE_NOEPI
diff --git a/tec-mollm_amd/tecmollm/functions.py b/tec-mollm_amd/tecmollm/functions.py
--- a/tec-mollm_amd/tecmollm/functions.py
+++ b/tec-mollm_amd/tecmollm/functions.py
@@ -598,13 +598,14 @@
         M = B * T * N
         h = h0.contiguous()
         level = plan.recompute if plan.keep else 0
+        dstore = int(plan.bf16) == ops.PREC_FP32 and ops.env_on("TECM_GELU_DSTORE")
         saved: List[torch.Tensor] = []
         ctx_lAT: List[Optional[torch.Tensor]] = []
         ctx_gen: List[int] = []
         ctx_wk: list = []
         for i in range(n_layers):
             lp = params[i * GPT2StackFn.PER_LAYER:(i + 1) * GPT2StackFn.PER_LAYER]
-            h3, acts, wk = GPT2StackFn._block_fwd(h, i, lp, plan, B, T, N, keep=plan.keep and level == 0)
+            h3, acts, wk = GPT2StackFn._block_fwd(h, i, lp, plan, B, T, N, keep=plan.keep and level == 0, dstore=dstore)
             ctx_lAT.append(wk[3])
             ctx_gen.append(wk[4])
             if acts is not None:
@@ -631,11 +632,13 @@
         ctx.kext_gen = ctx_gen
         ctx.wk = ctx_wk
         ctx.level = level
+        ctx.dstore = dstore
         ctx.meta = (B, T, N, D, n_layers, plan, len(saved))
         return out
 
     @staticmethod
-    def _block_fwd(h, i: int, lp, plan: DropPlan, B: int, T: int, N: int, wk=None, out: bool = True, keep: bool = True):
+    def _block_fwd(h, i: int, lp, plan: DropPlan, B: int, T: int, N: int, wk=None, out: bool = True, keep: bool = True,
+                   dstore: bool = False):
         (ln1w, ln1b, Wqkv, bqkv, lA, lB, Wo, bo, ln2w, ln2b, Wfc, bfc, Wpr, bpr) = lp
         D = h.shape[-1]
         M = B * T * N
@@ -695,8 +698,8 @@
         f16 = b16 and Wfc_f.dtype == torch.bfloat16 and Wpr_f.dtype == torch.bfloat16
         a = torch.empty(M, F4, device=h.device, dtype=torch.bfloat16 if f16 and PRE16 else torch.float32)
         f = torch.empty(M, F4, device=h.device, dtype=torch.bfloat16 if f16 else torch.float32)
-        gemm(M, F4, D, u2, D, Wfc_f, ldfc_f, f, F4, b_layout=lay_fc, bias=bfc, preact=(a, F4), act=ACT_GELU_TANH,
-             bf16=plan.bf16)
+        gemm(M, F4, D, u2, D, Wfc_f, ldfc_f, f, F4, b_layout=lay_fc, bias=bfc, preact=(a, F4),
+             act=ops.ACT_GELU_TANH_D if dstore else ACT_GELU_TANH, bf16=plan.bf16)
         if not keep:
             u2 = a = None
         h3 = None
@@ -753,14 +756,15 @@
                                 "forward's backward before the next forward of that layer")
             if ctx.level:
                 _, acts, _ = GPT2StackFn._block_fwd(h, i, params[i * GPT2StackFn.PER_LAYER:(i + 1) * GPT2StackFn.PER_LAYER],
-                                                    plan, B, T, N, wk=ctx.wk[i], out=False)
+                                                    plan, B, T, N, wk=ctx.wk[i], out=False, dstore=ctx.dstore)
                 u, ud, st1, qkv, h2, st2, a = acts
                 del acts
             F3, F4 = Wqkv.shape[1], Wfc.shape[1]
             Wpr_b, Wfc_b = _bwd_weight(Wpr, plan.bf16), _bwd_weight(Wfc, plan.bf16)
             da16 = Wpr_b.dtype == torch.bfloat16 and Wfc_b.dtype == torch.bfloat16
             da = torch.empty(M, F4, device=dh.device, dtype=torch.bfloat16 if da16 else torch.float32)
-            gemm(M, F4, D, dhm, D, Wpr_b, D, da, F4, act=ACT_GELU_TANH, dact_src=(a, F4), bf16=plan.bf16)
+            gemm(M, F4, D, dhm, D, Wpr_b, D, da, F4, act=ops.ACT_GELU_TANH_D if ctx.dstore else ACT_GELU_TANH,
+                 dact_src=(a, F4), bf16=plan.bf16)
             g16 = b16 and da16 and GRAD16
             du2 = torch.empty(M, D, device=dh.device, dtype=torch.bfloat16 if g16 else torch.float32)
             gemm(M, D, F4, da, F4, Wfc_b, F4, du2, D, bf16=plan.bf16)
diff --git a/tec-mollm_amd/tecmollm/ops.py b/tec-mollm_amd/tecmollm/ops.py
--- a/tec-mollm_amd/tecmollm/ops.py
+++ b/tec-mollm_amd/tecmollm/ops.py
@@ -12,6 +12,7 @@
 A_MK, A_KM = 0, 1
 B_NK, B_KN = 0, 1
 ACT_NONE, ACT_GELU_ERF, ACT_GELU_TANH = 0, 1, 2
+ACT_GELU_TANH_D = 3
 
 _MASK64 = (1 << 64) - 1
 
@@ -245,10 +246,27 @@
     if pair == (4, 4):
         win = bool(g.a_win.enabled or g.b_win.enabled)
         drp = bool(g.a_drop.p > 0 or g.b_drop.p > 0)
+        if win and a_win_segmented(g, drp):
+            win = False
     else:
         win = drp = True
     flags = f",{'true' if win else 'false'},{'true' if drp else 'false'}"
     return f"gemm_kernel<{g.a_layout},{g.b_layout},{pair[0]},{pair[1]},{bn}{flags}{m64}>"
+
+
+def env_on(name: str) -> bool:
+    return os.environ.get(name, "1")[:1] != "0"
+
+
+def a_win_segmented(g: TecmGemm, drop: bool) -> bool:
+    w = g.a_win
+    if not w.enabled or g.b_win.enabled or drop or g.a_layout != A_MK:
+        return False
+    if w.pad != 0 or (w.Lout - 1) * w.stride_t + w.taps > w.Lin:
+        return False
+    if w.Cw % 32 or g.M % (w.Lout * w.N):
+        return False
+    return env_on("TECM_GEMM_SEGK")
 
 
 def enable_gemm_timing(detail: bool = False) -> list:
```
